# nreHieW/Eagle

Measured on AMD Instinct MI355X. Metric: frames/sec end-to-end (detect+keypoint+homography) @1280x720, higher is better.
Workload: dtype f32 (split: hi/lo binary16 pairs, 3 x fp16 MFMA per product, fp32 accumulate); detector (1.4 % of the FLOP): f32, exact v_mfma_f32_16x16x4_f32 chains

## Files before the change

### eagle_amd/csrc/clip.hip

```cpp
#include "runtime.h"

namespace eagle {

struct ProfOff { EagleHandle* h; bool was; explicit ProfOff(EagleHandle* h_) : h(h_), was(h_->prof) { h->prof = false; } ~ProfOff() { h->prof = was; } };

static void clip_sync(EagleHandle* h)
{
    HIP_CHECK(hipStreamSynchronize(h->s_det));
    HIP_CHECK(hipStreamSynchronize(h->s_main));
    HIP_CHECK(hipStreamSynchronize(h->s_post));
}

void clip_close(EagleHandle* h)
{
    EagleHandle::Clip& c = h->clip;
    if (c.open) { (void)hipStreamSynchronize(h->s_det); (void)hipStreamSynchronize(h->s_main); (void)hipStreamSynchronize(h->s_post); }
    for (auto& p : c.g) { if (p) (void)hipFree(p); p = nullptr; }
    if (c.recs) (void)hipFree(c.recs);
    if (c.mem) (void)hipFree(c.mem);
    if (c.st) (void)hipFree(c.st);
    if (c.st_op) (void)hipFree(c.st_op);
    if (c.h_st) (void)hipHostFree(c.h_st);
    if (c.h_zero) (void)hipHostFree(c.h_zero);
    if (c.h_tail) (void)hipHostFree(c.h_tail);
    if (c.h_mem) (void)hipHostFree(c.h_mem);
    if (c.ecc_small) (void)hipFree(c.ecc_small);
    if (c.ecc_pairs) (void)hipFree(c.ecc_pairs);
    if (c.ecc_out) (void)hipFree(c.ecc_out);
    for (hipEvent_t e : {c.ev_gray, c.ev_det, c.ev_kp, c.ev_loop}) if (e) (void)hipEventDestroy(e);
    c = EagleHandle::Clip();
}

static void clip_open(EagleHandle* h, const uint8_t* d_bgr, int n)
{
    clip_close(h);
    const EagleConfig& cf = h->cfg;
    EagleHandle::Clip& c = h->clip;
    c.cv.bgr = d_bgr; c.cv.n = n; c.cv.h = cf.frame_h; c.cv.w = cf.frame_w;
    c.cv.lh[0] = cf.frame_h; c.cv.lw[0] = cf.frame_w; c.cv.levels = 0;
    for (int l = 1; l <= 2; ++l) {
        c.cv.lh[l] = (c.cv.lh[l - 1] + 1) / 2; c.cv.lw[l] = (c.cv.lw[l - 1] + 1) / 2;
        if (c.cv.lw[l] <= 15 || c.cv.lh[l] <= 15) break;
        c.cv.levels = l;
    }
    c.open = true;
    for (int l = 0; l < 3; ++l) {
        HIP_CHECK(hipMalloc((void**)&c.g[l], std::max<size_t>((size_t)n * c.cv.lh[l] * c.cv.lw[l], 16)));
        c.cv.g[l] = c.g[l];
    }
    const size_t nn = (size_t)std::max(n, 1);
    HIP_CHECK(hipMalloc((void**)&c.recs, sizeof(EagleFrameResult) * nn));
    HIP_CHECK(hipMalloc((void**)&c.mem, sizeof(MemList) * nn));
    HIP_CHECK(hipMalloc((void**)&c.st, sizeof(ChainState)));
    HIP_CHECK(hipMalloc((void**)&c.st_op, sizeof(ChainState)));
    HIP_CHECK(hipHostMalloc((void**)&c.h_st, sizeof(ChainState), hipHostMallocDefault));
    HIP_CHECK(hipHostMalloc((void**)&c.h_zero, sizeof(ChainState), hipHostMallocDefault));
    HIP_CHECK(hipHostMalloc((void**)&c.h_tail, sizeof(int) * 4, hipHostMallocDefault));
    HIP_CHECK(hipHostMalloc((void**)&c.h_mem, sizeof(MemList), hipHostMallocDefault));
    memset(c.h_zero, 0, sizeof(ChainState));
    c.h_zero->stalled = -1;
    c.h_tail[0] = -1; c.h_tail[1] = 0; c.h_tail[2] = -1;
    for (hipEvent_t* e : {&c.ev_gray, &c.ev_det, &c.ev_kp, &c.ev_loop}) HIP_CHECK(hipEventCreateWithFlags(e, hipEventDisableTiming));
    HIP_CHECK(hipMemsetAsync(c.mem, 0xFF, sizeof(MemList) * nn, h->s_main));
    HIP_CHECK(hipMemsetAsync(c.recs, 0, sizeof(EagleFrameResult) * nn, h->s_main));
    HIP_CHECK(hipMemsetAsync(h->clip_sat, 0, sat_pad_bytes(cf.batch), h->s_main));
    HIP_CHECK(hipMemcpyAsync(c.st, c.h_zero, sizeof(ChainState), hipMemcpyHostToDevice, h->s_main));
    if (n > 0) gray_pyramid_launch(d_bgr, n, c.cv.h, c.cv.w, c.g[0], c.g[1], c.g[2], h->s_main);
    HIP_CHECK(hipEventRecord(c.ev_gray, h->s_main));
    HIP_CHECK(hipStreamWaitEvent(h->s_det, c.ev_gray, 0));
    HIP_CHECK(hipEventRecord(c.ev_det, h->s_det));
    HIP_CHECK(hipEventRecord(c.ev_kp, h->s_main));
    HIP_CHECK(hipEventRecord(c.ev_loop, h->s_post));
}

static void clip_detect_objects(EagleHandle* h, int first, int count)
{
    const EagleConfig& cf = h->cfg;
    EagleHandle::Clip& c = h->clip;
    const int B = cf.batch;
    const size_t fb = (size_t)cf.frame_h * cf.frame_w * 3;
    size_t ev_i = 0;
    EagleHandle::StepBuf& sb = h->sb[0];
    ProfOff prof_off(h);
    h->cur_sat = h->clip_sat;
    for (int i = first; i < first + count; i += B) {
        const int na = std::min(B, first + count - i);
        HIP_CHECK(hipMemsetAsync(sb.d_out, 0, sizeof(EagleFrameResult) * B, h->s_det));
        preprocess_launch(h->det_prec, c.cv.bgr + (size_t)i * fb, na, cf.frame_h, cf.frame_w, h->kp_in, h->det_in, h->lb, h->s_det, 2);
        run_net(h, h->yo.get(), h->s_det, ev_i);
        yolo_decode_launch(h->levels, 3, B, 5, cf.detector_floor, h->ds, h->s_det);
        nms_launch(h->ds, B, h->pp, sb.d_out, h->s_det);
        HIP_CHECK(hipMemcpyAsync(c.recs + i, sb.d_out, sizeof(EagleFrameResult) * na, hipMemcpyDeviceToDevice, h->s_det));
    }
    HIP_CHECK(hipEventRecord(c.ev_det, h->s_det));
}

static void clip_detect_keypoints(EagleHandle* h, int first, int stride, int count)
{
    const EagleConfig& cf = h->cfg;
    EagleHandle::Clip& c = h->clip;
    const int B = cf.batch;
    const size_t fb = (size_t)cf.frame_h * cf.frame_w * 3;
    size_t ev_i = 0;
    EagleHandle::StepBuf& sb = h->sb[0];
    ProfOff prof_off(h);
    h->cur_sat = h->clip_sat;
    for (int k0 = 0; k0 < count; k0 += B) {
        const int na = std::min(B, count - k0);
        const uint8_t* src;
        if (stride == 1) src = c.cv.bgr + (size_t)(first + k0) * fb;
        else {
            for (int k = 0; k < na; ++k)
                HIP_CHECK(hipMemcpyAsync(sb.d_frames + (size_t)k * fb, c.cv.bgr + (size_t)(first + (k0 + k) * stride) * fb, fb, hipMemcpyDeviceToDevice, h->s_main));
            src = sb.d_frames;
        }
        preprocess_launch(h->prec, src, na, cf.frame_h, cf.frame_w, h->kp_in, h->det_in, h->lb, h->s_main, 1);
        h->cur_parts = sb.parts;
        run_net(h, h->hr.get(), h->s_main, ev_i);
        if (!h->fused_argmax) heat_argmax_launch(h->logits, sb.parts, h->hm_chunks, h->s_main);
        decode_mem_launch(sb.parts, na, h->pp, c.mem, first + k0 * stride, stride, h->s_main);
    }
    HIP_CHECK(hipEventRecord(c.ev_kp, h->s_main));
}

}

extern "C" {

int eagle_reproject(EagleHandle* h, EagleFrameResult* recs, int n, const double* Hs, const uint8_t* flags)
{
    API_BEGIN_H(h)
    if (!recs || !Hs || !flags || n < 0) fail(EAGLE_E_INVALID, "bad argument");
    if (n == 0) return EAGLE_OK;
    HIP_CHECK(hipSetDevice(h->cfg.device));
    Net scratch;
    EagleFrameResult* d_r = (EagleFrameResult*)scratch.get(sizeof(EagleFrameResult) * (size_t)n);
    double* d_H = (double*)scratch.get(sizeof(double) * 9 * (size_t)n);
    unsigned char* d_f = (unsigned char*)scratch.get((size_t)n);
    HIP_CHECK(hipMemcpyAsync(d_r, recs, sizeof(EagleFrameResult) * (size_t)n, hipMemcpyHostToDevice, h->s_main));
    HIP_CHECK(hipMemcpyAsync(d_H, Hs, sizeof(double) * 9 * (size_t)n, hipMemcpyHostToDevice, h->s_main));
    HIP_CHECK(hipMemcpyAsync(d_f, flags, (size_t)n, hipMemcpyHostToDevice, h->s_main));
    reproject_launch(d_r, d_H, d_f, n, h->cfg.frame_h, h->cfg.frame_w, h->s_main);
    HIP_CHECK(hipMemcpyAsync(recs, d_r, sizeof(EagleFrameResult) * (size_t)n, hipMemcpyDeviceToHost, h->s_main));
    HIP_CHECK(hipStreamSynchronize(h->s_main));
    API_END(h)
}

int eagle_team_colors(EagleHandle* h, const void* d_bgr, int n_frames, const EagleCrop* crops, int n_crops, int32_t* counts)
{
    API_BEGIN_H(h)
    if (!d_bgr || n_frames < 0 || n_crops < 0 || (n_crops > 0 && (!crops || !counts))) fail(EAGLE_E_INVALID, "bad argument");
    if (n_crops == 0) return EAGLE_OK;
    HIP_CHECK(hipSetDevice(h->cfg.device));
    Net scratch;
    EagleCrop* d_c = (EagleCrop*)scratch.get(sizeof(EagleCrop) * (size_t)n_crops);
    int* d_n = (int*)scratch.get(sizeof(int) * 12 * (size_t)n_crops);
    HIP_CHECK(hipMemcpyAsync(d_c, crops, sizeof(EagleCrop) * (size_t)n_crops, hipMemcpyHostToDevice, h->s_main));
    eagle::team_colors_launch((const uint8_t*)d_bgr, n_frames, h->cfg.frame_h, h->cfg.frame_w, d_c, n_crops, d_n, h->s_main);
    HIP_CHECK(hipMemcpyAsync(counts, d_n, sizeof(int) * 12 * (size_t)n_crops, hipMemcpyDeviceToHost, h->s_main));
    HIP_CHECK(hipStreamSynchronize(h->s_main));
    API_END(h)
}

int eagle_reid_features(EagleHandle* h, const void* d_bgr, int n_frames, const EagleCrop* crops, int n_crops, float* feats)
{
    API_BEGIN_H(h)
    if (!h->finalized || !h->reid) fail(EAGLE_E_STATE, "no appearance network: load the reid.* tensors (OSNet-x0.25, torchreid names) before eagle_finalize_weights");
    if (n_frames < 0 || n_crops < 0 || (n_crops > 0 && (!d_bgr || !crops || !feats))) fail(EAGLE_E_INVALID, "bad argument");
    if (n_crops == 0) return EAGLE_OK;
    HIP_CHECK(hipSetDevice(h->cfg.device));
    eagle::ProfOff prof_off(h);
    for (int i0 = 0; i0 < n_crops; i0 += eagle::REID_NB) {
        const int nb = std::min(eagle::REID_NB, n_crops - i0);
        for (int k = 0; k < eagle::REID_NB; ++k) {
            EagleCrop c = {-1, 0, 0, 0, 0};
            if (k < nb) c = crops[i0 + k];
            h->reid_crops_h[k] = c;
        }
        HIP_CHECK(hipMemcpyAsync(h->reid_crops, h->reid_crops_h, sizeof(EagleCrop) * eagle::REID_NB, hipMemcpyHostToDevice, h->s_main));
        eagle::reid_crop_launch((const uint8_t*)d_bgr, n_frames, h->cfg.frame_h, h->cfg.frame_w, h->reid_crops, eagle::REID_NB, h->reid_in, h->s_main);
        size_t ev_i = 0;
        eagle::run_net(h, h->reid.get(), h->s_main, ev_i);
        HIP_CHECK(hipMemcpyAsync(h->reid_feats_h, h->reid_feats, sizeof(float) * EAGLE_REID_DIM * (size_t)nb, hipMemcpyDeviceToHost, h->s_main));
        HIP_CHECK(hipStreamSynchronize(h->s_main));
        memcpy(feats + (size_t)i0 * EAGLE_REID_DIM, h->reid_feats_h, sizeof(float) * EAGLE_REID_DIM * (size_t)nb);
    }
    API_END(h)
}

int eagle_track_open(EagleHandle* h, const EagleTrackParams* params)
{
    API_BEGIN_H(h)
    if (h->tracker) eagle::tracker_destroy(h->tracker);
    h->tracker = eagle::tracker_create(params);
    h->ecc_has_prev = false;
    API_END(h)
}

int eagle_track_frames(EagleHandle* h, EagleFrameResult* recs, int n) { return eagle_track_frames_cmc(h, recs, n, nullptr); }

int eagle_track_frames_cmc(EagleHandle* h, EagleFrameResult* recs, int n, const double* warps) { return eagle_track_frames_reid(h, recs, n, warps, nullptr, nullptr, nullptr); }

int eagle_track_frames_reid(EagleHandle* h, EagleFrameResult* recs, int n, const double* warps, const float* feats, const int32_t* feat_det, const int32_t* feat_count)
{
    API_BEGIN_H(h)
    if (!recs || n < 0 || (feats && (!feat_det || !feat_count))) fail(EAGLE_E_INVALID, "bad argument");
    if (!h->tracker) fail(EAGLE_E_STATE, "eagle_track_open has not been called");
    if (n == 0) return EAGLE_OK;
    if (feats)
        for (int i = 0; i < n; ++i) {
            if (feat_count[i] < 0 || feat_count[i] > EAGLE_MAX_DET) fail(EAGLE_E_INVALID, "eagle_track_frames_reid: feat_count[%d] = %d", i, feat_count[i]);
            if (recs[i].n_det < 0 || recs[i].n_det > EAGLE_MAX_DET) fail(EAGLE_E_INVALID, "eagle_track_frames_reid: record %d has n_det = %d", i, recs[i].n_det);
        }
    if (feats) {
        size_t o = 0;
        for (int i = 0; i < n; ++i)
            for (int k = 0; k < feat_count[i]; ++k, ++o)
                if (feat_det[o] < 0 || feat_det[o] >= recs[i].n_det)
                    fail(EAGLE_E_INVALID, "eagle_track_frames_reid: feat_det[%zu] = %d is not a detection of record %d (n_det %d)", o, feat_det[o], i, recs[i].n_det);
    }
    std::vector<double> Hs((size_t)n * 9, 0.0);
    std::vector<uint8_t> flags((size_t)n, 0);
    bool any = false;
    size_t fo = 0;
    for (int i = 0; i < n; ++i) {
        const int nf = feats ? feat_count[i] : 0;
        const bool applied = eagle::tracker_apply(h->tracker, recs + i, h->cfg.frame_h, h->cfg.frame_w, h->cfg.detector_conf, warps ? warps + (size_t)i * 6 : nullptr,
                                                  feats ? feats + fo * EAGLE_REID_DIM : nullptr, feats ? feat_det + fo : nullptr, nf);
        fo += (size_t)nf;
        if (!applied) continue;
        any = true;
        flags[i] = recs[i].H_valid ? 1 : 2;
        memcpy(&Hs[(size_t)i * 9], recs[i].H, sizeof(double) * 9);
    }
    if (any) {
        const int rc = eagle_reproject(h, recs, n, Hs.data(), flags.data());
        if (rc) return rc;
    }
    API_END(h)
}

#define CLIP_CHECK(h, cond, msg) if (!(h) || !(h)->finalized) return EAGLE_E_STATE; if (!(cond)) { (h)->err = msg; return EAGLE_E_INVALID; }
int eagle_clip_open(EagleHandle* h, const void* d_bgr, int n)
{
    CLIP_CHECK(h, n >= 0 && (d_bgr || n == 0), "eagle_clip_open: bad arguments")
    API_BEGIN
    HIP_CHECK(hipSetDevice(h->cfg.device));
    eagle::clip_open(h, (const uint8_t*)d_bgr, n);
    API_END(h)
}

int eagle_clip_close(EagleHandle* h)
{
    API_BEGIN_H(h)
    HIP_CHECK(hipSetDevice(h->cfg.device));
    eagle::clip_close(h);
    API_END(h)
}

int eagle_clip_detect_objects(EagleHandle* h, int first, int count)
{
    CLIP_CHECK(h, h->clip.open && first >= 0 && count >= 0 && first + (int64_t)count <= h->clip.cv.n, "eagle_clip_detect_objects: no open clip or frames out of range")
    API_BEGIN
    HIP_CHECK(hipSetDevice(h->cfg.device));
    eagle::clip_detect_objects(h, first, count);
    API_END(h)
}

int eagle_clip_detect_keypoints(EagleHandle* h, int first, int stride, int count)
// ... 217 lines not shown
```

### eagle_amd/csrc/common.h

```cpp
#pragma once
#include <hip/hip_runtime.h>
#include <hip/hip_fp16.h>
#include <cstdint>
#include <cstdio>
#include <string>
#include <vector>

#include "../../include/eagle.h"

namespace eagle {

enum Act : int { ACT_NONE = 0, ACT_RELU = 1, ACT_SILU = 2 };

struct Err {
    int code;
    std::string msg;
};
[[noreturn]] void fail(int code, const char* fmt, ...);

#define HIP_CHECK(expr)                                                                                \
    do {                                                                                               \
        hipError_t _e = (expr);                                                                        \
        if (_e != hipSuccess) ::eagle::fail(EAGLE_E_HIP, "%s failed: %s (%s:%d)", #expr, hipGetErrorString(_e), \
                                            __FILE__, __LINE__);                                       \
    } while (0)

void ensure_max_dynamic_lds(const void* fn, int bytes);

struct TView {
    void* p = nullptr;
    int n = 0, h = 0, w = 0;
    int c = 0;
    int cs = 0;
    int off = 0;
    int f32 = 0;
    size_t esize() const { return f32 ? 4 : 2; }
    TView slice(int o, int cc) const { TView v = *this; v.off = off + o; v.c = cc; return v; }
};

struct ConvConfig {
    int ks = 3, stride = 1;
    int kc = 0;
    int nt = 0;
    int wx = 2;
    int cin = 0, cout_pad = 0;
    int variant = 0;
};
struct ArgmaxPart { float score; int idx; };
struct ConvLaunch {
    ConvConfig cfg;
    TView x, y, r1, r2;
    const void* w = nullptr;
    const float* bias = nullptr;
    int pre_act = 0, post_act = 0;
    int out_f32 = 0;
    double flop = 0;
    float descale = 1.0f;
    ArgmaxPart* const* am_slot = nullptr;
    unsigned* const* sat_slot = nullptr;
};
int conv_tiles_per_frame(int precision, const ConvConfig& cfg, int ho, int wo);
bool conv_supported(int precision, const ConvConfig& cfg);
void conv_launch(int precision, const ConvLaunch& L, hipStream_t s);
size_t conv_weight_elems(int precision, const ConvConfig& cfg);
size_t conv_lds_bytes(int precision, const ConvConfig& cfg);
void conv_tile_weights(int precision, const ConvConfig& cfg, const float* w_hwio, int cin_real, int cout_real, void* dst, float* descale = nullptr);
inline int prec_tensor_fmt(int precision) { return precision == EAGLE_PREC_F32 ? 1 : precision == EAGLE_PREC_F32S ? 2 : 0; }
inline bool prec_is_f16_kernels(int precision) { return precision == EAGLE_PREC_F16 || precision == EAGLE_PREC_F32S; }
ConvConfig conv_choose(int precision, int ks, int stride, int cin_pad, int cout_pad, int wo, bool plain_epilogue = false, bool second_residual = false);

struct BneckLaunch {
    TView x, res, y;
    const void *w1 = nullptr, *w2 = nullptr, *w3 = nullptr;
    const float *b1 = nullptr, *b2 = nullptr, *b3 = nullptr;
    float ds1 = 1.f, ds2 = 1.f, ds3 = 1.f;
    unsigned* const* sat_slot = nullptr;
    unsigned long long* dbg = nullptr;
    bool ds_fused = false;
};
bool bneck_supported(const TView& x, int cmid, int cout);
void bneck_tile_weights(const float* w, int taps, int cin, int cout, std::vector<_Float16>& out, float* descale);
void bneck_scale_bias(std::vector<float>& b, float descale);
void bneck_launch(const BneckLaunch& L, hipStream_t s);

struct LetterBox { int new_h, new_w, top, left, out_h, out_w; };
LetterBox letterbox_geometry(int h, int w, int imgsz, int square = 0);
void preprocess_launch(int precision, const uint8_t* d_bgr, int n, int h, int w, const TView& kp, const TView& det,
                       const LetterBox& lb, hipStream_t s, int which = 3, int det_precision = -1);
struct FuseUp { TView z; };
void fuse_sum_launch(const TView& base, const FuseUp* ups, int n_up, int relu, const TView& y, hipStream_t s, unsigned* sat = nullptr);
void maxpool5_launch(const TView& x, const TView& y, hipStream_t s);
void upsample2_launch(const TView& x, const TView& y, hipStream_t s);
void split_to_f32_launch(const TView& x, const TView& y, hipStream_t s);

void heat_argmax_launch(const TView& logits, ArgmaxPart* parts, int chunks, hipStream_t s);

struct DetLevel { TView box, cls; int gh, gw; float stride; int a0; };
struct DetScratch {
    int A = 0;
    float* boxes = nullptr;
    float* conf = nullptr;
    int* cls = nullptr;
    unsigned long long* keys = nullptr;
    int* count = nullptr;
};
void yolo_decode_launch(const DetLevel* lv, int n_lv, int n, int nc, float conf_floor, const DetScratch& sc, hipStream_t s);

struct PostParams {
    int frame_h, frame_w, in_h, in_w;
    int hm_h, hm_w, hm_chunks;
    double keypoint_conf, detector_conf, ransac_thresh;
    float nms_iou;
    int ransac_max_iters, lm_iters;
};
void nms_launch(const DetScratch& sc, int n, const PostParams& pp, EagleFrameResult* d_out, hipStream_t s);
void post_launch(const ArgmaxPart* parts, int n, const PostParams& pp, EagleFrameResult* d_out, hipStream_t s);
void reproject_launch(EagleFrameResult* d_recs, const double* d_Hs, const unsigned char* d_flags, int n, int frame_h, int frame_w, hipStream_t s);
void homography_only_launch(const float* d_img, const float* d_world, int npts, double thresh, int max_iters, int lm_iters,
                            double* d_H, uint8_t* d_mask, int* d_ok, hipStream_t s);


struct ClipView {
    const uint8_t* bgr = nullptr;
    const uint8_t* g[3] = {nullptr, nullptr, nullptr};
    int lh[3] = {0, 0, 0}, lw[3] = {0, 0, 0};
    int levels = 0;
    int n = 0, h = 0, w = 0;
};
struct MemList { int n; EagleFlowKp kp[EAGLE_N_LANDMARKS]; };
struct ChainState {
    int n_prev; EagleFlowKp prev[EAGLE_N_LANDMARKS];
    int has_H, compute_h; double H[9];
    int stalled;
    int error;
    int lk_valid, lk_n;
    float lk_prev[2 * EAGLE_N_LANDMARKS], lk_next[2 * EAGLE_N_LANDMARKS];
    unsigned char lk_status[EAGLE_N_LANDMARKS];
    int flow_n; EagleFlowKp flow[EAGLE_N_LANDMARKS];
};
void gray_pyramid_launch(const uint8_t* d_bgr, int n, int h, int w, uint8_t* g0, uint8_t* g1, uint8_t* g2, hipStream_t s);
void lk_launch(const ClipView& cv, int src_frame, int dst_frame, ChainState* st, const MemList* mem, int kint, hipStream_t s);
struct EccResult { int ok, iters; double rho; float M[6]; };
void ecc_small_launch(const uint8_t* gray, uint8_t* small, int n, int h, int w, int dh, int dw, double inv_scale , hipStream_t s);
void ecc_launch(const uint8_t* small, const uint8_t* carry, const int2* pairs, int n_pairs, EccResult* out, int h, int w, int max_iter, double eps, hipStream_t s);
struct YuvArgs {
    const uint8_t* src;
    uint8_t* dst;
    int h, w;
    int64_t frame_stride, y_pitch, c_offset, c_pitch, v_offset;
    int c_step;
    int vec;
};
void yuv_to_bgr_launch(const YuvArgs& a, int n, hipStream_t s);
void team_colors_launch(const uint8_t* d_bgr, int n_frames, int fh, int fw, const EagleCrop* d_crops, int n_crops, int* d_counts, hipStream_t s);

void reid_crop_launch(const uint8_t* d_bgr, int n_frames, int fh, int fw, const EagleCrop* d_crops, int n, const TView& out, hipStream_t s);
void reid_conv7_launch(const TView& x, const float* w, const float* b, const TView& y, int n, hipStream_t s);
void reid_maxpool3s2_launch(const TView& x, const TView& y, int n, hipStream_t s);
void reid_avgpool2_launch(const TView& x, const TView& y, int n, hipStream_t s);
void reid_dw3_launch(const TView& x, const float* w, const float* b, const TView& y, int n, hipStream_t s);
void reid_gate_launch(const TView* streams, const float* w1, const float* b1, const float* w2, const float* b2, int c_real, int r, float* g, const TView& y, int n, hipStream_t s);
void reid_head_launch(const TView& x, const float* w, const float* b, float* feats, int dim, int n, hipStream_t s);

struct Tracker;
Tracker* tracker_create(const EagleTrackParams* p);
void tracker_destroy(Tracker* t);
bool tracker_apply(Tracker* t, EagleFrameResult* rec, int frame_h, int frame_w, double detector_conf, const double* warp = nullptr,
                   const float* feats = nullptr, const int* feat_det = nullptr, int n_feat = 0);
void similarity_ransac(const double* p0, const double* p1, int n, double* W6);
int lk_debug(const char* key, long long value, void* out, long long out_bytes);
void decode_mem_launch(const ArgmaxPart* parts, int n, const PostParams& pp, MemList* mem, int first, int stride, hipStream_t s);
void chain_launch(const ClipView& cv, ChainState* st, const MemList* mem, EagleFrameResult* recs, const PostParams& pp, int frame,
                  int kint, int hint, int calib, hipStream_t s);
void flow_filter_launch(const ClipView& cv, ChainState* st, int hue_frame, hipStream_t s);

}
```

### eagle_amd/csrc/elementwise.hip

```cpp
#include <type_traits>
#include "common.h"
#include "dmath.h"

namespace eagle {

using half8 = __attribute__((ext_vector_type(8))) _Float16;

struct ResizeAxis { int s0, s1; int a0, a1; };

__device__ __forceinline__ ResizeAxis lin_coef(int d, int dsize, int ssize)
{
    const double scale = (double)ssize / (double)dsize;
    float f = (float)(((double)d + 0.5) * scale - 0.5);
    int s = (int)floorf(f);
    f -= (float)s;
    if (s < 0) { s = 0; f = 0.f; }
    if (s >= ssize - 1) { s = ssize - 1; f = 0.f; }
    ResizeAxis r;
    r.s0 = s; r.s1 = (s + 1 < ssize) ? s + 1 : s;
    r.a0 = (int)(short)lrintf((1.f - f) * 2048.f);
    r.a1 = (int)(short)lrintf(f * 2048.f);
    return r;
}

__device__ __forceinline__ void resize_px(const uint8_t* src, int sh, int sw, int dh, int dw, int dy, int dx, int rgb[3])
{
    const size_t rs = (size_t)sw * 3;
    if (sh == dh && sw == dw) {
        const uint8_t* p = src + dy * rs + dx * 3;
        rgb[0] = p[2]; rgb[1] = p[1]; rgb[2] = p[0];
    } else if (sh == 2 * dh && sw == 2 * dw) {
        const uint8_t* p = src + (size_t)(2 * dy) * rs + (size_t)(2 * dx) * 3;
#pragma unroll
        for (int c = 0; c < 3; ++c) rgb[2 - c] = (p[c] + p[3 + c] + p[rs + c] + p[rs + 3 + c] + 2) >> 2;
    } else {
        const ResizeAxis ax = lin_coef(dx, dw, sw), ay = lin_coef(dy, dh, sh);
        const uint8_t* r0 = src + ay.s0 * rs; const uint8_t* r1 = src + ay.s1 * rs;
#pragma unroll
        for (int c = 0; c < 3; ++c) {
            const int t0 = r0[ax.s0 * 3 + c] * ax.a0 + r0[ax.s1 * 3 + c] * ax.a1;
            const int t1 = r1[ax.s0 * 3 + c] * ax.a0 + r1[ax.s1 * 3 + c] * ax.a1;
            rgb[2 - c] = (((ay.a0 * (t0 >> 4)) >> 16) + ((ay.a1 * (t1 >> 4)) >> 16) + 2) >> 2;
        }
    }
}

struct SplitT { char b[4]; };
__device__ __forceinline__ void split8_store(void* dst, const float* v)
{
    half8 hi, lo;
#pragma unroll
    for (int i = 0; i < 8; ++i) { const float s = __builtin_amdgcn_fmed3f(v[i] * 16.0f, -65504.0f, 65504.0f); hi[i] = (_Float16)s; lo[i] = (_Float16)(s - (float)hi[i]); }
    *(half8*)dst = hi; *((half8*)dst + 1) = lo;
}

template <typename T>
__device__ __forceinline__ void store_px(const TView& v, size_t pix, float r, float g, float b)
{
    if constexpr (sizeof(T) == 4 && !__is_same(T, float)) {
        const float o[8] = {r, g, b, 0.f, 0.f, 0.f, 0.f, 0.f};
        split8_store((char*)v.p + (pix * v.cs + v.off) * 4, o);
    } else if constexpr (sizeof(T) == 2) {
        half8 o = {(_Float16)r, (_Float16)g, (_Float16)b, 0, 0, 0, 0, 0};
        *(half8*)((_Float16*)v.p + pix * v.cs + v.off) = o;
    } else {
        *(float4*)((float*)v.p + pix * v.cs + v.off) = make_float4(r, g, b, 0.f);
    }
}

template <typename T, typename TD = T>
__global__ __launch_bounds__(256) void preprocess_kernel(const uint8_t* bgr, int n, int h, int w, TView kp, TView det, LetterBox lb, int which)
{
    const size_t fsz = (size_t)h * w * 3;
    const int kp_px = kp.h * kp.w, det_px = det.h * det.w;
    const int lo = (which & 1) ? 0 : kp_px, hi = (which & 2) ? kp_px + det_px : kp_px;
    const int per = hi - lo;
    for (size_t i = (size_t)blockIdx.x * blockDim.x + threadIdx.x; i < (size_t)n * per; i += (size_t)gridDim.x * blockDim.x) {
        const int f = (int)(i / per);
        int r = lo + (int)(i - (size_t)f * per);
        const uint8_t* src = bgr + f * fsz;
        int rgb[3];
        if (r < kp_px) {
            const int dy = r / kp.w, dx = r - dy * kp.w;
            resize_px(src, h, w, kp.h, kp.w, dy, dx, rgb);
            const float m0 = 0x1.eeb334p+6f, m1 = 0x1.d11eb8p+6f, m2 = 0x1.9e1eb8p+6f;
            const float s0 = 0x1.18926cp-6f, s1 = 0x1.1ed5bp-6f, s2 = 0x1.1d8f56p-6f;
            store_px<T>(kp, (size_t)f * kp_px + r, ((float)rgb[0] - m0) * s0, ((float)rgb[1] - m1) * s1, ((float)rgb[2] - m2) * s2);
        } else {
            r -= kp_px;
            const int dy = r / det.w, dx = r - dy * det.w;
            const int yy = dy - lb.top, xx = dx - lb.left;
            if (yy >= 0 && yy < lb.new_h && xx >= 0 && xx < lb.new_w) resize_px(src, h, w, lb.new_h, lb.new_w, yy, xx, rgb);
            else rgb[0] = rgb[1] = rgb[2] = 114;
            store_px<TD>(det, (size_t)f * det_px + r, (float)rgb[0] / 255.0f, (float)rgb[1] / 255.0f, (float)rgb[2] / 255.0f);
        }
    }
}

LetterBox letterbox_geometry(int h, int w, int imgsz, int square)
{
    const double r = std::min((double)imgsz / h, (double)imgsz / w);
    LetterBox lb;
    lb.new_w = (int)nearbyint(w * r); lb.new_h = (int)nearbyint(h * r);
    double dw = square ? (imgsz - lb.new_w) : (imgsz - lb.new_w) % 32, dh = square ? (imgsz - lb.new_h) : (imgsz - lb.new_h) % 32;
    dw /= 2; dh /= 2;
    lb.top = (int)nearbyint(dh - 0.1); lb.left = (int)nearbyint(dw - 0.1);
    const int bottom = (int)nearbyint(dh + 0.1), right = (int)nearbyint(dw + 0.1);
    lb.out_h = lb.new_h + lb.top + bottom; lb.out_w = lb.new_w + lb.left + right;
    return lb;
}

template <typename T>
static void preprocess_launch_det(int det_precision, dim3 grid, hipStream_t s, const uint8_t* d_bgr, int n, int h, int w, const TView& kp, const TView& det, const LetterBox& lb, int which)
{
    if (det_precision == EAGLE_PREC_F16) hipLaunchKernelGGL((preprocess_kernel<T, _Float16>), grid, dim3(256), 0, s, d_bgr, n, h, w, kp, det, lb, which);
    else if (det_precision == EAGLE_PREC_F32S) hipLaunchKernelGGL((preprocess_kernel<T, SplitT>), grid, dim3(256), 0, s, d_bgr, n, h, w, kp, det, lb, which);
    else hipLaunchKernelGGL((preprocess_kernel<T, float>), grid, dim3(256), 0, s, d_bgr, n, h, w, kp, det, lb, which);
}

void preprocess_launch(int precision, const uint8_t* d_bgr, int n, int h, int w, const TView& kp, const TView& det,
                       const LetterBox& lb, hipStream_t s, int which, int det_precision)
{
    const size_t total = (size_t)n * (((which & 1) ? kp.h * kp.w : 0) + ((which & 2) ? det.h * det.w : 0));
    if (total == 0) return;
    const int blocks = (int)std::min<size_t>((total + 255) / 256, 256 * 16);
    if (det_precision >= 0 && det_precision != precision) {
        if (precision == EAGLE_PREC_F16) preprocess_launch_det<_Float16>(det_precision, dim3(blocks), s, d_bgr, n, h, w, kp, det, lb, which);
        else if (precision == EAGLE_PREC_F32S) preprocess_launch_det<SplitT>(det_precision, dim3(blocks), s, d_bgr, n, h, w, kp, det, lb, which);
        else preprocess_launch_det<float>(det_precision, dim3(blocks), s, d_bgr, n, h, w, kp, det, lb, which);
        HIP_CHECK(hipGetLastError());
        return;
    }
    if (precision == EAGLE_PREC_F16) hipLaunchKernelGGL(preprocess_kernel<_Float16>, dim3(blocks), dim3(256), 0, s, d_bgr, n, h, w, kp, det, lb, which);
    else if (precision == EAGLE_PREC_F32S) hipLaunchKernelGGL(preprocess_kernel<SplitT>, dim3(blocks), dim3(256), 0, s, d_bgr, n, h, w, kp, det, lb, which);
    else hipLaunchKernelGGL(preprocess_kernel<float>, dim3(blocks), dim3(256), 0, s, d_bgr, n, h, w, kp, det, lb, which);
    HIP_CHECK(hipGetLastError());
}

#ifndef EAGLE_FUSE_NT
#define EAGLE_FUSE_NT 0
#endif
template <typename T> struct Vec;
template <> struct Vec<_Float16> {
    static constexpr int N = 8;
    float v[8];
    __device__ __forceinline__ void load(const void* p, size_t e) { half8 h = *(const half8*)((const _Float16*)p + e); for (int i = 0; i < 8; ++i) v[i] = (float)h[i]; }
    __device__ __forceinline__ void store(void* p, size_t e) const { half8 h; for (int i = 0; i < 8; ++i) h[i] = (_Float16)v[i]; *(half8*)((_Float16*)p + e) = h; }
};
template <> struct Vec<SplitT> {
    static constexpr int N = 8;
    float v[8];
    __device__ __forceinline__ void load(const void* p, size_t e)
    {
        const half8 hi = *(const half8*)((const char*)p + e * 4), lo = *(const half8*)((const char*)p + e * 4 + 16);
        for (int i = 0; i < 8; ++i) v[i] = (float)hi[i] + (float)lo[i];
    }
    __device__ __forceinline__ void store(void* p, size_t e) const
    {
        half8 hi, lo;
#pragma unroll
        for (int i = 0; i < 8; ++i) { const float s = __builtin_amdgcn_fmed3f(v[i], -65504.0f, 65504.0f); hi[i] = (_Float16)s; lo[i] = (_Float16)(s - (float)hi[i]); }
        *(half8*)((char*)p + e * 4) = hi; *((half8*)((char*)p + e * 4) + 1) = lo;
    }
    __device__ __forceinline__ void store_nt(void* p, size_t e) const
    {
        half8 hi, lo;
#pragma unroll
        for (int i = 0; i < 8; ++i) { const float s = __builtin_amdgcn_fmed3f(v[i], -65504.0f, 65504.0f); hi[i] = (_Float16)s; lo[i] = (_Float16)(s - (float)hi[i]); }
        __builtin_nontemporal_store(hi, (half8*)((char*)p + e * 4)); __builtin_nontemporal_store(lo, (half8*)((char*)p + e * 4) + 1);
    }
};
template <> struct Vec<float> {
    static constexpr int N = 4;
    float v[4];
    __device__ __forceinline__ void load(const void* p, size_t e) { float4 f = *(const float4*)((const float*)p + e); v[0] = f.x; v[1] = f.y; v[2] = f.z; v[3] = f.w; }
    __device__ __forceinline__ void store(void* p, size_t e) const { *(float4*)((float*)p + e) = make_float4(v[0], v[1], v[2], v[3]); }
};

struct FuseArgs { TView base, y; TView z[3]; float sh[3], sw[3]; int n_up; int relu; unsigned* sat; };

constexpr int FUSE_ROWS = 8;
template <typename T, int NUP>
__global__ __launch_bounds__(256) void fuse_sum_kernel(FuseArgs a)
{
    constexpr int VN = Vec<T>::N;
    const int H = a.y.h, W = a.y.w, groups = a.y.c / VN;
    const unsigned col = blockIdx.y * 256u + threadIdx.x;
    if (col >= (unsigned)(W * groups)) return;
    const int hb = (H + FUSE_ROWS - 1) / FUSE_ROWS;
    const int band = gridDim.x >> 3, rb = (int)(blockIdx.x & 7) * band + (int)(blockIdx.x >> 3);
    if (rb >= a.y.n * hb) return;
    const int n = rb / hb, oy0 = (rb - n * hb) * FUSE_ROWS;
    const int ox = (int)(col / (unsigned)groups), g = (int)(col - (unsigned)ox * (unsigned)groups);
    constexpr int NU = NUP > 0 ? NUP : 1;
    Vec<T> p00[NU], p01[NU], p10[NU], p11[NU];
    float lx1[NU];
    int cy0[NU], cy1[NU];
    unsigned zc0[NU], zc1[NU];
#pragma unroll
    for (int j = 0; j < NUP; ++j) {
        const TView& z = a.z[j];
        const float fx = a.sw[j] * (float)ox;
        const int x0 = (int)fx, x1 = x0 + (x0 < z.w - 1 ? 1 : 0);
        lx1[j] = fx - (float)x0;
        const unsigned co = (unsigned)(z.off + g * VN);
        zc0[j] = (unsigned)x0 * (unsigned)z.cs + co; zc1[j] = (unsigned)x1 * (unsigned)z.cs + co;
        cy0[j] = -1; cy1[j] = -1;
    }
    for (int r = 0; r < FUSE_ROWS; ++r) {
        const int oy = oy0 + r;
        if (oy >= H) break;
        const unsigned pix = ((unsigned)n * H + (unsigned)oy) * (unsigned)W + (unsigned)ox;
        Vec<T> acc; acc.load(a.base.p, (size_t)pix * a.base.cs + a.base.off + g * VN);
        float ly1[NU];
#pragma unroll
        for (int j = 0; j < NUP; ++j) {
            const TView& z = a.z[j];
            const float fy = a.sh[j] * (float)oy;
            const int y0 = __builtin_amdgcn_readfirstlane((int)fy);
            const int y1 = y0 + (y0 < z.h - 1 ? 1 : 0);
            ly1[j] = fy - (float)y0;
            const unsigned b = (unsigned)n * z.h;
            if (y0 != cy0[j]) {
                if (y0 == cy1[j]) { p00[j] = p10[j]; p01[j] = p11[j]; }
                else {
                    const unsigned ro = (b + (unsigned)y0) * (unsigned)z.w * (unsigned)z.cs;
                    p00[j].load(z.p, (size_t)(ro + zc0[j])); p01[j].load(z.p, (size_t)(ro + zc1[j]));
                }
                cy0[j] = y0;
            }
            if (y1 != cy1[j]) {
                if (y1 == y0) { p10[j] = p00[j]; p11[j] = p01[j]; }
                else {
                    const unsigned ro = (b + (unsigned)y1) * (unsigned)z.w * (unsigned)z.cs;
                    p10[j].load(z.p, (size_t)(ro + zc0[j])); p11[j].load(z.p, (size_t)(ro + zc1[j]));
                }
                cy1[j] = y1;
            }
        }
#pragma unroll
        for (int j = 0; j < NUP; ++j) {
            const float ly0 = 1.0f - ly1[j], lx0 = 1.0f - lx1[j];
#pragma unroll
            for (int k = 0; k < VN; ++k) {
                const float top = fmaf(lx1[j], p01[j].v[k], lx0 * p00[j].v[k]);
// ... 163 lines not shown
```

### eagle_amd/csrc/nets.hip

```cpp
#include "runtime.h"

namespace eagle {

struct Builder {
    EagleHandle* H;
    Net* net;
    int prec;
    double bn_eps;
    int N;
    const char* label_suffix = "";
    int cur_stream = 0;
    void set_stream(int k) { cur_stream = k; net->pool = k; }
    void fork_join(Op::Kind kind, int nbranch) { Op op; op.kind = kind; op.nbranch = nbranch; op.tag = kind == Op::FORK ? "fork" : "join"; net->ops.push_back(op); }

    int gran() const { return prec == EAGLE_PREC_F32 ? 4 : 8; }

    TView act(int h, int w, int c, bool f32 = false)
    {
        TView v; v.n = N; v.h = h; v.w = w; v.c = c; v.cs = c; v.off = 0;
        v.f32 = (f32 || prec == EAGLE_PREC_F32) ? 1 : prec_tensor_fmt(prec);
        v.p = net->get((size_t)N * h * w * c * v.esize());
        return v;
    }
    void release(const TView& v) { net->put(v.p); }

    const HostTensor& W(const std::string& name)
    {
        auto it = H->weights.find(name);
        if (it == H->weights.end()) fail(EAGLE_E_MISSING, "weight tensor '%s' was not loaded", name.c_str());
        return it->second;
    }

    TView conv(const TView& x, const std::string& cname, const std::string& bn, int stride, int pre, const TView* r1,
               const TView* r2, int post, const TView* out = nullptr, bool out_f32 = false, ArgmaxPart* const* am_slot = nullptr)
    {
        std::vector<float> hwio, bias; int cin, cout, ks;
        fold(cname, bn, hwio, bias, cin, cout, ks);
        if (cin > x.c) fail(EAGLE_E_INVALID, "%s: input has %d channels, weight expects %d", cname.c_str(), x.c, cin);
        const int cout_pad = (cout + 15) / 16 * 16;
        bias.resize(cout_pad, 0.f);
        const int ho = (x.h + 2 * (ks / 2) - ks) / stride + 1, wo = (x.w + 2 * (ks / 2) - ks) / stride + 1;
        if (const char* dump = getenv("EAGLE_DUMP_LAYERS")) {
            if (FILE* f = fopen(dump, "a")) { fprintf(f, "%d,%d,%d,%d,%d,%d,%d\n", ks, stride, x.c, cout_pad, x.h, x.w, N); fclose(f); }
        }
        ConvLaunch L;
        L.cfg = conv_choose(prec, ks, stride, x.c, cout_pad, wo, pre == ACT_NONE && post <= ACT_RELU && !out_f32, r1 && r2);
        if (!conv_supported(prec, L.cfg))
            fail(EAGLE_E_NOKERNEL, "%s: no kernel instance (ks=%d s=%d kc=%d nt=%d)", cname.c_str(), ks, stride, L.cfg.kc, L.cfg.nt);
        const size_t ne = conv_weight_elems(prec, L.cfg);
        std::vector<char> tiled(ne * (prec == EAGLE_PREC_F32 ? 4 : 2));
        conv_tile_weights(prec, L.cfg, hwio.data(), cin, cout, tiled.data(), &L.descale);
        L.w = net->upload(tiled.data(), tiled.size());
        L.bias = (const float*)net->upload(bias.data(), bias.size() * 4);
        L.x = x;
        if (out) {
            L.y = *out;
            if (out->c != cout_pad || out->h != ho || out->w != wo) fail(EAGLE_E_INVALID, "%s: output slice mismatch", cname.c_str());
        } else {
            L.y = act(ho, wo, cout_pad, out_f32);
        }
        if (r1) L.r1 = *r1;
        if (r2) L.r2 = *r2;
        L.pre_act = pre; L.post_act = post; L.out_f32 = out_f32 ? 1 : 0;
        refuse_2gib(cname, "layer", {&L.x, &L.y, r1 ? &L.r1 : nullptr, r2 ? &L.r2 : nullptr});
        L.am_slot = am_slot;
        if (prec == EAGLE_PREC_F32S && !out_f32 && !am_slot) L.sat_slot = &H->cur_sat;
        if (am_slot) { H->hm_chunks = conv_tiles_per_frame(prec, L.cfg, ho, wo); H->fused_argmax = true; }
        L.flop = 2.0 * N * ho * wo * (double)cout * cin * ks * ks;
        const int pr = prec;
        char label[64];
        snprintf(label, sizeof(label), "conv %dx%d/%d %d->%d @%dx%d v%d%s", ks, ks, stride, cin, cout, ho, wo, L.cfg.variant, label_suffix);
        const double es = prec == EAGLE_PREC_F16 ? 2 : 4;
        emit_conv(label, L.flop, (double)N * x.h * x.w * cin * es + (double)N * ho * wo * cout * ((out_f32 || prec != EAGLE_PREC_F16) ? 4 : 2) * (am_slot ? 0 : 1) +
                                 (r1 ? (double)N * ho * wo * cout * es : 0) + (r2 ? (double)N * ho * wo * cout * es : 0) + (double)ks * ks * cin * cout * es,
                  [L, pr](hipStream_t s) { conv_launch(pr, L, s); });
        return L.y;
    }
    void fold(const std::string& cname, const std::string& bn, std::vector<float>& hwio, std::vector<float>& bias, int& cin, int& cout, int& ks)
    {
        const HostTensor& w = W(cname + ".weight");
        if (w.shape.size() != 4) fail(EAGLE_E_INVALID, "%s.weight: expected 4-d", cname.c_str());
        cout = (int)w.shape[0]; cin = (int)w.shape[1]; ks = (int)w.shape[2];
        hwio.assign((size_t)ks * ks * cin * cout, 0.f); bias.assign(cout, 0.f);
        std::vector<double> scale(cout, 1.0);
        if (!bn.empty()) {
            const HostTensor &g = W(bn + ".weight"), &b = W(bn + ".bias"), &m = W(bn + ".running_mean"), &v = W(bn + ".running_var");
            for (int o = 0; o < cout; ++o) {
                scale[o] = (double)g.data[o] / std::sqrt((double)v.data[o] + bn_eps);
                bias[o] = (float)((double)b.data[o] - (double)m.data[o] * scale[o]);
            }
        } else if (H->weights.count(cname + ".bias")) {
            const HostTensor& b = W(cname + ".bias");
            for (int o = 0; o < cout; ++o) bias[o] = b.data[o];
        }
        for (int o = 0; o < cout; ++o)
            for (int i = 0; i < cin; ++i)
                for (int t = 0; t < ks * ks; ++t) {
                    const float wv = w.data[((size_t)o * cin + i) * ks * ks + t];
                    hwio[((size_t)t * cin + i) * cout + o] = bn.empty() ? wv : (float)((double)wv * scale[o]);
                }
    }
    void refuse_2gib(const std::string& name, const char* what, std::initializer_list<const TView*> ts)
    {
        for (const TView* t : ts)
            if (t && (size_t)t->n * t->h * t->w * t->cs * t->esize() >= ((size_t)1 << 31))
                fail(EAGLE_E_INVALID, "%s: a %d x %d x %d x %d-channel tensor of this %s reaches 2 GiB at a device batch of %d frames (32-bit tensor offsets); use a smaller EagleConfig.batch",
                     name.c_str(), t->n, t->h, t->w, t->cs, what, N);
    }
    void emit_conv(const char* label, double flop, double bytes, std::function<void(hipStream_t)> run)
    {
        net->names.emplace_back(new std::string(label));
        Op op; op.kind = Op::CONV; op.flop = flop; op.bytes = bytes; op.tag = net->names.back()->c_str(); op.stream = cur_stream; op.run = std::move(run);
        net->ops.push_back(op);
    }
    TView bottleneck(const TView& x, const std::string& q, const TView& res, const std::string& ds_conv = "", const std::string& ds_bn = "")
    {
        BneckLaunch L;
        const bool dsf = !ds_conv.empty();
        std::vector<float> hw, bs; int ci, co, ks;
        std::vector<_Float16> img;
        double flop = 0;
        const char* cn[3] = {"conv1", "conv2", "conv3"}; const char* bnn[3] = {"bn1", "bn2", "bn3"};
        const int want_ks[3] = {1, 3, 1}, want_ci[3] = {x.c, 64, 64}, want_co[3] = {64, 64, 256};
        for (int k = 0; k < 3; ++k) {
            fold(q + cn[k], q + bnn[k], hw, bs, ci, co, ks);
            if (ks != want_ks[k] || ci != want_ci[k] || co != want_co[k]) fail(EAGLE_E_INVALID, "%s%s: not the Bottleneck shape of the fused kernel", q.c_str(), cn[k]);
            if (k == 2 && dsf) {
                std::vector<float> hwd, bd; int cid, cod, ksd;
                fold(ds_conv, ds_bn, hwd, bd, cid, cod, ksd);
                if (ksd != 1 || cid != 64 || cod != 256 || x.c != 64) fail(EAGLE_E_INVALID, "%s: not the 1x1 64->256 downsample of the fused kernel", ds_conv.c_str());
                hw.insert(hw.end(), hwd.begin(), hwd.end());
                for (int o = 0; o < 256; ++o) bs[o] = bs[o] + bd[o];
                ci = 128;
                flop += 2.0 * N * x.h * x.w * 256.0 * 64;
            }
            float ds = 1.f;
            bneck_tile_weights(hw.data(), ks * ks, ci, co, img, &ds);
            bneck_scale_bias(bs, ds);
            const void* dw = net->upload(img.data(), img.size() * 2);
            const float* db = (const float*)net->upload(bs.data(), bs.size() * 4);
            if (k == 0) { L.w1 = dw; L.b1 = db; L.ds1 = ds; } else if (k == 1) { L.w2 = dw; L.b2 = db; L.ds2 = ds; } else { L.w3 = dw; L.b3 = db; L.ds3 = ds; }
            flop += 2.0 * N * x.h * x.w * (double)co * (k == 2 ? 64 : ci) * ks * ks;
        }
        L.x = x; L.y = act(x.h, x.w, 256); L.res = dsf ? L.y : res; L.ds_fused = dsf;
        L.sat_slot = &H->cur_sat;
        refuse_2gib(q, "block", {&L.x, &L.y, &L.res});
        char label[64];
        snprintf(label, sizeof(label), "bneck %d->64->256%s @%dx%d%s", x.c, dsf ? "+ds" : "", x.h, x.w, label_suffix);
        emit_conv(label, flop, (double)N * x.h * x.w * 4.0 * (x.c + 256 + ((dsf || res.p == x.p) ? 0 : 256)) + 4.0 * (x.c * 64 + 9 * 64 * 64 + 64 * 256 + (dsf ? 64 * 256 : 0)),
                  [L](hipStream_t s) { bneck_launch(L, s); });
        return L.y;
    }
    static double vbytes(const TView& v) { return (double)v.n * v.h * v.w * v.c * (v.f32 ? 4 : 2); }
    void other(std::function<void(hipStream_t)> fn, const char* tag, double bytes = 0)
    {
        Op op; op.kind = Op::OTHER; op.run = std::move(fn); op.tag = tag; op.stream = cur_stream; op.bytes = bytes;
        net->ops.push_back(op);
    }
};

static const char* HRP = "unnormalized_model.0.";

static std::vector<TView> hr_stage(Builder& B, std::vector<TView> xs, int stage_idx, int n_modules, int nb, bool last_single)
{
    const int R = ACT_RELU;
    for (int m = 0; m < n_modules; ++m) {
        const std::string q = std::string(HRP) + "stage" + std::to_string(stage_idx) + "." + std::to_string(m) + ".";
        B.fork_join(Op::FORK, nb - 1);
        const bool interleave = !(getenv("EAGLE_HR_INTERLEAVE") && atoi(getenv("EAGLE_HR_INTERLEAVE")) == 0);
        for (int step = 0; step < 4 * nb; ++step) {
            const int k = interleave ? step / nb : step % 4, b = interleave ? nb - 1 - step % nb : step / 4;
            B.set_stream(b);
            TView x = xs[b];
            const std::string r = q + "branches." + std::to_string(b) + "." + std::to_string(k) + ".";
            TView o = B.conv(x, r + "conv1", r + "bn1", 1, 0, nullptr, nullptr, R);
            TView y = B.conv(o, r + "conv2", r + "bn2", 1, 0, &x, nullptr, R);
            B.release(o);
            B.release(x);
            xs[b] = y;
        }
        B.set_stream(0);
        B.fork_join(Op::JOIN, nb - 1);
        const int n_out = (last_single && m == n_modules - 1) ? 1 : nb;
        std::vector<TView> out;
        if (n_out > 1) B.fork_join(Op::FORK, n_out - 1);
        for (int i = 0; i < n_out; ++i) {
            B.set_stream(n_out > 1 ? i : 0);
            TView y; bool have_y = false;
            for (int j = 0; j < i; ++j) {
                TView t = xs[j];
                for (int k = 0; k < i - j; ++k) {
                    const std::string r = q + "fuse_layers." + std::to_string(i) + "." + std::to_string(j) + "." + std::to_string(k) + ".";
                    const bool last = k == i - j - 1;
                    TView nt;
                    if (!last) {
                        nt = B.conv(t, r + "0", r + "1", 2, 0, nullptr, nullptr, R);
                    } else {
                        const TView* ident = (j == i - 1) ? &xs[i] : nullptr;
                        const bool relu_now = ident && i == nb - 1;
                        nt = B.conv(t, r + "0", r + "1", 2, 0, have_y ? &y : nullptr, ident, relu_now ? R : 0);
                    }
                    if (k > 0) B.release(t);
                    t = nt;
                }
                if (have_y) B.release(y);
                y = t; have_y = true;
            }
            if (i == 0) y = xs[0];
            FuseUp ups[3]; int nu = 0;
            for (int j = i + 1; j < nb; ++j) {
                const std::string r = q + "fuse_layers." + std::to_string(i) + "." + std::to_string(j) + ".";
                ups[nu++].z = B.conv(xs[j], r + "0", r + "1", 1, 0, nullptr, nullptr, 0);
            }
            if (nu) {
                TView o = B.act(y.h, y.w, y.c);
                const TView base = y; FuseUp u0 = ups[0], u1 = ups[1], u2 = ups[2]; const int n_up = nu;
                EagleHandle* const Hh = B.H;
                B.other([base, u0, u1, u2, n_up, o, Hh](hipStream_t s) { FuseUp u[3] = {u0, u1, u2}; fuse_sum_launch(base, u, n_up, 1, o, s, Hh->cur_sat); }, "fuse_sum",
                        Builder::vbytes(base) + Builder::vbytes(o) + (nu > 0 ? Builder::vbytes(ups[0].z) : 0) + (nu > 1 ? Builder::vbytes(ups[1].z) : 0) + (nu > 2 ? Builder::vbytes(ups[2].z) : 0));
                for (int k = 0; k < nu; ++k) B.release(ups[k].z);
                if (i != 0) B.release(y);
                y = o;
            }
            out.push_back(y);
        }
        B.set_stream(0);
        if (n_out > 1) B.fork_join(Op::JOIN, n_out - 1);
        for (int b = 0; b < nb; ++b) B.release(xs[b]);
        xs = out;
    }
    return xs;
}

static TView build_hrnet(Builder& B, const TView& x_in)
{
    const int R = ACT_RELU;
    const std::string P = HRP;
    TView x = B.conv(x_in, P + "conv1", P + "bn1", 2, 0, nullptr, nullptr, R);
    TView x2 = B.conv(x, P + "conv2", P + "bn2", 2, 0, nullptr, nullptr, R);
    B.release(x); x = x2;
    for (int b = 0; b < 4; ++b) {
        const std::string q = P + "layer1." + std::to_string(b) + ".";
        const char* fe = getenv("EAGLE_BNECK_FUSED");
        const char* de = getenv("EAGLE_BNECK_DS");
        const bool fused = B.prec == EAGLE_PREC_F32S && !(fe && atoi(fe) == 0) && bneck_supported(x, 64, 256);
        const bool dsf = fused && b == 0 && x.c == 64 && !(de && atoi(de) == 0);
        TView res = x;
        if (b == 0 && !dsf) res = B.conv(x, q + "downsample.0", q + "downsample.1", 1, 0, nullptr, nullptr, 0);
        if (fused) {
            TView y = dsf ? B.bottleneck(x, q, x, q + "downsample.0", q + "downsample.1") : B.bottleneck(x, q, res);
            if (b == 0 && !dsf) B.release(res);
            B.release(x);
            x = y;
            continue;
        }
        TView o1 = B.conv(x, q + "conv1", q + "bn1", 1, 0, nullptr, nullptr, R);
        TView o2 = B.conv(o1, q + "conv2", q + "bn2", 1, 0, nullptr, nullptr, R);
        TView y = B.conv(o2, q + "conv3", q + "bn3", 1, 0, &res, nullptr, R);
        B.release(o1); B.release(o2);
        if (b == 0) B.release(res);
        B.release(x);
        x = y;
    }
    std::vector<TView> ys(2);
    B.fork_join(Op::FORK, 1);
    B.set_stream(1);
    ys[1] = B.conv(x, P + "transition1.1.0.0", P + "transition1.1.0.1", 2, 0, nullptr, nullptr, R);
    B.set_stream(0);
    ys[0] = B.conv(x, P + "transition1.0.0", P + "transition1.0.1", 1, 0, nullptr, nullptr, R);
    B.fork_join(Op::JOIN, 1);
    B.release(x);
    ys = hr_stage(B, ys, 2, 1, 2, false);
    ys.push_back(B.conv(ys.back(), P + "transition2.2.0.0", P + "transition2.2.0.1", 2, 0, nullptr, nullptr, R));
    ys = hr_stage(B, ys, 3, 4, 3, false);
    ys.push_back(B.conv(ys.back(), P + "transition3.3.0.0", P + "transition3.3.0.1", 2, 0, nullptr, nullptr, R));
    ys = hr_stage(B, ys, 4, 3, 4, true);
    ArgmaxPart* const* am = (prec_is_f16_kernels(B.prec) && !getenv("EAGLE_NO_FUSED_ARGMAX")) ? &B.H->cur_parts : nullptr;
    TView logits = B.conv(ys[0], "unnormalized_model.1", "", 1, 0, nullptr, nullptr, 0, nullptr, true, am);
    B.release(ys[0]);
    return logits;
}

struct YoloDims { int c[5]; int n[4]; };
static YoloDims yolo_dims(int variant)
{
    static const double D[5] = {0.33, 0.33, 0.67, 1.0, 1.0}, Wd[5] = {0.25, 0.5, 0.75, 1.0, 1.25};
    static const int MC[5] = {1024, 1024, 768, 512, 512};
    YoloDims y;
    const int base[5] = {64, 128, 256, 512, 1024};
    for (int i = 0; i < 5; ++i) y.c[i] = (int)std::ceil(std::min(base[i], MC[variant]) * Wd[variant] / 8.0) * 8;
    const int rep[4] = {3, 6, 6, 3};
    for (int i = 0; i < 4; ++i) y.n[i] = std::max((int)std::nearbyint(rep[i] * D[variant]), 1);
    return y;
}

struct YoloBuilder {
    Builder& B;
    int S = ACT_SILU;
    TView cv(const TView& x, const std::string& name, int stride = 1, const TView* r1 = nullptr, const TView* out = nullptr)
    {
        return B.conv(x, name + ".conv", name + ".bn", stride, S, r1, nullptr, 0, out);
    }
    TView c2f(const TView& x, int idx, int cout, int n, bool shortcut, const TView* out = nullptr)
    {
        const std::string p = "model." + std::to_string(idx);
        const int c = cout / 2;
        TView cat = B.act(x.h, x.w, (2 + n) * c);
        TView first = cat.slice(0, 2 * c);
        cv(x, p + ".cv1", 1, nullptr, &first);
        for (int k = 0; k < n; ++k) {
            TView in = cat.slice((1 + k) * c, c);
            TView t = cv(in, p + ".m." + std::to_string(k) + ".cv1");
            TView o = cat.slice((2 + k) * c, c);
            cv(t, p + ".m." + std::to_string(k) + ".cv2", 1, shortcut ? &in : nullptr, &o);
            B.release(t);
        }
        TView y = cv(cat, p + ".cv2", 1, nullptr, out);
        B.release(cat);
        return y;
    }
};

static void build_yolo(Builder& B, const TView& x_in, int variant, DetLevel lv[3], int nc, bool mixed = false)
{
    YoloBuilder Y{B};
    const YoloDims d = yolo_dims(variant);
    const int c1 = d.c[0], c2 = d.c[1], c3 = d.c[2], c4 = d.c[3], c5 = d.c[4];
    TView x0 = Y.cv(x_in, "model.0", 2);
    TView x1 = Y.cv(x0, "model.1", 2); B.release(x0);
    TView x2 = Y.c2f(x1, 2, c2, d.n[0], true); B.release(x1);
    TView x3 = Y.cv(x2, "model.3", 2); B.release(x2);
    const int h3 = x3.h, w3 = x3.w;
    const int h4 = (h3 - 1) / 2 + 1, w4 = (w3 - 1) / 2 + 1, h5 = (h4 - 1) / 2 + 1, w5 = (w4 - 1) / 2 + 1;
    TView cat15 = B.act(h3, w3, c4 + c3);
    TView cat12 = B.act(h4, w4, c5 + c4);
    TView cat18 = B.act(h4, w4, c3 + c4);
    TView cat21 = B.act(h5, w5, c4 + c5);
    TView p3 = cat15.slice(c4, c3), p4 = cat12.slice(c5, c4), p5 = cat21.slice(c4, c5), h12 = cat18.slice(c3, c4);
    Y.c2f(x3, 4, c3, d.n[1], true, &p3); B.release(x3);
    TView x5 = Y.cv(p3, "model.5", 2);
    Y.c2f(x5, 6, c4, d.n[2], true, &p4); B.release(x5);
    TView x7 = Y.cv(p4, "model.7", 2);
    TView x8 = Y.c2f(x7, 8, c5, d.n[3], true); B.release(x7);
    {
        const int ch = c5 / 2;
        TView cat = B.act(h5, w5, 4 * ch);
        TView s0 = cat.slice(0, ch), s1 = cat.slice(ch, ch), s2 = cat.slice(2 * ch, ch), s3 = cat.slice(3 * ch, ch);
        Y.cv(x8, "model.9.cv1", 1, nullptr, &s0); B.release(x8);
        B.other([s0, s1](hipStream_t s) { maxpool5_launch(s0, s1, s); }, "maxpool5", 2 * Builder::vbytes(s0));
        B.other([s1, s2](hipStream_t s) { maxpool5_launch(s1, s2, s); }, "maxpool5", 2 * Builder::vbytes(s0));
        B.other([s2, s3](hipStream_t s) { maxpool5_launch(s2, s3, s); }, "maxpool5", 2 * Builder::vbytes(s0));
        Y.cv(cat, "model.9.cv2", 1, nullptr, &p5);
        B.release(cat);
    }
    {
        TView u = cat12.slice(0, c5);
        B.other([p5, u](hipStream_t s) { upsample2_launch(p5, u, s); }, "upsample2", Builder::vbytes(p5) + Builder::vbytes(u));
        Y.c2f(cat12, 12, c4, d.n[0], false, &h12);
    }
    TView h15, h18, h21;
    {
        TView u = cat15.slice(0, c4);
        B.other([h12, u](hipStream_t s) { upsample2_launch(h12, u, s); }, "upsample2", Builder::vbytes(h12) + Builder::vbytes(u));
    }
    if (!mixed) {
        h15 = Y.c2f(cat15, 15, c3, d.n[0], false);
        {
            TView o = cat18.slice(0, c3);
            Y.cv(h15, "model.16", 2, nullptr, &o);
        }
        h18 = Y.c2f(cat18, 18, c4, d.n[0], false);
        {
            TView o = cat21.slice(0, c4);
            Y.cv(h18, "model.19", 2, nullptr, &o);
        }
        h21 = Y.c2f(cat21, 21, c5, d.n[0], false);
    } else {
        B.prec = EAGLE_PREC_F32;
        auto to_f32 = [&B](const TView& x, const TView& y) {
            B.other([x, y](hipStream_t s) { split_to_f32_launch(x, y, s); }, "split_to_f32", Builder::vbytes(x) + Builder::vbytes(y));
        };
        TView cat15f = B.act(h3, w3, c4 + c3), cat18f = B.act(h4, w4, c3 + c4), cat21f = B.act(h5, w5, c4 + c5);
        to_f32(cat15, cat15f);
        h15 = Y.c2f(cat15f, 15, c3, d.n[0], false);
        {
            TView o = cat18f.slice(0, c3);
            Y.cv(h15, "model.16", 2, nullptr, &o);
            to_f32(h12, cat18f.slice(c3, c4));
        }
        h18 = Y.c2f(cat18f, 18, c4, d.n[0], false);
        {
// ... 9 lines not shown
    for (int l = 0; l < 3; ++l) {
        const std::string pb = "model.22.cv2." + std::to_string(l), pc = "model.22.cv3." + std::to_string(l);
        TView b0 = Y.cv(feats[l], pb + ".0");
        TView b1 = Y.cv(b0, pb + ".1"); B.release(b0);
        TView box = B.conv(b1, pb + ".2", "", 1, 0, nullptr, nullptr, 0, nullptr, true); B.release(b1);
        TView k0 = Y.cv(feats[l], pc + ".0");
        TView k1 = Y.cv(k0, pc + ".1"); B.release(k0);
        TView cls = B.conv(k1, pc + ".2", "", 1, 0, nullptr, nullptr, 0, nullptr, true); B.release(k1);
        lv[l].box = box; lv[l].cls = cls; lv[l].gh = box.h; lv[l].gw = box.w; lv[l].stride = strides[l]; lv[l].a0 = a0;
        a0 += box.h * box.w;
    }
    (void)c1; (void)nc;
}

static const char* RP = "reid.";

struct ReidFold { std::vector<float> scale, shift; };
static ReidFold reid_bn(Builder& B, const std::string& bn, int c)
{
    const HostTensor &g = B.W(bn + ".weight"), &b = B.W(bn + ".bias"), &m = B.W(bn + ".running_mean"), &v = B.W(bn + ".running_var");
    ReidFold f; f.scale.resize(c); f.shift.resize(c);
    for (int o = 0; o < c; ++o) {
        const double sc = (double)g.data[o] / std::sqrt((double)v.data[o] + 1e-5);
        f.scale[o] = (float)sc; f.shift[o] = (float)((double)b.data[o] - (double)m.data[o] * sc);
    }
    return f;
}

static TView reid_light(Builder& B, const TView& x, const std::string& lc, int mid)
{
    TView t = B.conv(x, lc + ".conv1", "", 1, 0, nullptr, nullptr, 0);
    const HostTensor& w = B.W(lc + ".conv2.weight");
    const ReidFold f = reid_bn(B, lc + ".bn", mid);
    const int C = t.c;
    std::vector<float> wk((size_t)9 * C, 0.f), bk(C, 0.f);
    for (int c = 0; c < mid; ++c) {
        for (int k = 0; k < 9; ++k) wk[(size_t)k * C + c] = (float)((double)w.data[(size_t)c * 9 + k] * (double)f.scale[c]);
        bk[c] = f.shift[c];
    }
    const float* dw = (const float*)B.net->upload(wk.data(), wk.size() * 4);
    const float* db = (const float*)B.net->upload(bk.data(), bk.size() * 4);
    TView y = B.act(t.h, t.w, C);
    const int n = B.N;
    B.other([t, dw, db, y, n](hipStream_t s) { reid_dw3_launch(t, dw, db, y, n, s); }, "reid dw3x3", 2 * Builder::vbytes(y));
    B.release(t);
    return y;
}

static TView reid_osblock(Builder& B, const TView& x, const std::string& b, int cin, int cout)
{
    const int mid = cout / 4, R = ACT_RELU;
    TView x1 = B.conv(x, b + ".conv1.conv", b + ".conv1.bn", 1, 0, nullptr, nullptr, R);
    TView st[4];
    st[0] = reid_light(B, x1, b + ".conv2a", mid);
    const char* names[3] = {"b", "c", "d"};
    for (int k = 0; k < 3; ++k) {
        TView y = x1;
        for (int d = 0; d < k + 2; ++d) {
            TView nx = reid_light(B, y, b + ".conv2" + names[k] + "." + std::to_string(d), mid);
            if (d > 0) B.release(y);
            y = nx;
        }
        st[k + 1] = y;
    }
    B.release(x1);
    const HostTensor &w1 = B.W(b + ".gate.fc1.weight"), &b1 = B.W(b + ".gate.fc1.bias"), &w2 = B.W(b + ".gate.fc2.weight"), &b2 = B.W(b + ".gate.fc2.bias");
    const int r = (int)w1.shape[0];
    const float* d1 = (const float*)B.net->upload(w1.data.data(), w1.data.size() * 4);
    const float* e1 = (const float*)B.net->upload(b1.data.data(), b1.data.size() * 4);
    const float* d2 = (const float*)B.net->upload(w2.data.data(), w2.data.size() * 4);
    const float* e2 = (const float*)B.net->upload(b2.data.data(), b2.data.size() * 4);
    const int C = st[0].c, n = B.N;
    float* g = (float*)B.net->get((size_t)n * 4 * C * 4);
    TView x2 = B.act(st[0].h, st[0].w, C);
    const TView s0 = st[0], s1 = st[1], s2 = st[2], s3 = st[3];
    B.other([s0, s1, s2, s3, d1, e1, d2, e2, mid, r, g, x2, n](hipStream_t s) { const TView ss[4] = {s0, s1, s2, s3}; reid_gate_launch(ss, d1, e1, d2, e2, mid, r, g, x2, n, s); },
            "reid gate", 5 * Builder::vbytes(x2));
    for (auto& t : st) B.release(t);
    TView ident = x;
    if (cin != cout) ident = B.conv(x, b + ".downsample.conv", b + ".downsample.bn", 1, 0, nullptr, nullptr, 0);
    TView y = B.conv(x2, b + ".conv3.conv", b + ".conv3.bn", 1, 0, &ident, nullptr, R);
    B.release(x2);
    if (cin != cout) B.release(ident);
    return y;
}

static void build_reid(Builder& B, EagleHandle* h)
{
    const std::string P = RP;
    const int n = B.N;
    h->reid_in = B.act(256, 128, 4);
    const HostTensor& w1 = B.W(P + "conv1.conv.weight");
    const ReidFold f1 = reid_bn(B, P + "conv1.bn", 16);
    std::vector<float> wk(7 * 7 * 3 * 16), bk(16);
    for (int o = 0; o < 16; ++o) {
        for (int c = 0; c < 3; ++c)
            for (int k = 0; k < 49; ++k) wk[(size_t)(k * 3 + c) * 16 + o] = (float)((double)w1.data[((size_t)o * 3 + c) * 49 + k] * (double)f1.scale[o]);
        bk[o] = f1.shift[o];
    }
    const float* dw = (const float*)B.net->upload(wk.data(), wk.size() * 4);
    const float* db = (const float*)B.net->upload(bk.data(), bk.size() * 4);
    TView c1 = B.act(128, 64, 16);
    const TView in = h->reid_in;
    B.other([in, dw, db, c1, n](hipStream_t s) { reid_conv7_launch(in, dw, db, c1, n, s); }, "reid conv7x7", Builder::vbytes(in) + Builder::vbytes(c1));
    TView x = B.act(64, 32, 16);
    B.other([c1, x, n](hipStream_t s) { reid_maxpool3s2_launch(c1, x, n, s); }, "reid maxpool", Builder::vbytes(c1) + Builder::vbytes(x));
    B.release(c1);
    static const int CH[4] = {16, 64, 96, 128};
    const char* stage[3] = {"conv2", "conv3", "conv4"};
    for (int sI = 0; sI < 3; ++sI) {
        const int cin = CH[sI], cout = CH[sI + 1];
        const std::string sp = P + stage[sI];
        TView y = reid_osblock(B, x, sp + ".0", cin, cout); B.release(x); x = y;
        y = reid_osblock(B, x, sp + ".1", cout, cout); B.release(x); x = y;
        if (sI < 2) {
            TView t = B.conv(x, sp + ".2.0.conv", sp + ".2.0.bn", 1, 0, nullptr, nullptr, ACT_RELU); B.release(x);
            TView p = B.act(t.h / 2, t.w / 2, t.c);
            B.other([t, p, n](hipStream_t s) { reid_avgpool2_launch(t, p, n, s); }, "reid avgpool", Builder::vbytes(t) + Builder::vbytes(p));
            B.release(t);
            x = p;
        }
    }
    TView c5 = B.conv(x, P + "conv5.conv", P + "conv5.bn", 1, 0, nullptr, nullptr, ACT_RELU); B.release(x);
    const HostTensor &fw = B.W(P + "fc.0.weight"), &fb = B.W(P + "fc.0.bias");
    const ReidFold ff = reid_bn(B, P + "fc.1", EAGLE_REID_DIM);
    std::vector<float> hw((size_t)EAGLE_REID_DIM * c5.c, 0.f), hb(EAGLE_REID_DIM);
    for (int o = 0; o < EAGLE_REID_DIM; ++o) {
        for (int c = 0; c < 128; ++c) hw[(size_t)o * c5.c + c] = (float)((double)fw.data[(size_t)o * 128 + c] * (double)ff.scale[o]);
        hb[o] = (float)((double)fb.data[o] * (double)ff.scale[o] + (double)ff.shift[o]);
    }
    const float* dhw = (const float*)B.net->upload(hw.data(), hw.size() * 4);
    const float* dhb = (const float*)B.net->upload(hb.data(), hb.size() * 4);
    h->reid_feats = (float*)B.net->get((size_t)n * EAGLE_REID_DIM * 4);
    float* feats = h->reid_feats;
    B.other([c5, dhw, dhb, feats, n](hipStream_t s) { reid_head_launch(c5, dhw, dhb, feats, EAGLE_REID_DIM, n, s); }, "reid head", Builder::vbytes(c5));
    h->reid_crops = (EagleCrop*)B.net->get(sizeof(EagleCrop) * (size_t)n);
    HIP_CHECK(hipHostMalloc((void**)&h->reid_crops_h, sizeof(EagleCrop) * (size_t)n, hipHostMallocDefault));
    HIP_CHECK(hipHostMalloc((void**)&h->reid_feats_h, sizeof(float) * EAGLE_REID_DIM * (size_t)n, hipHostMallocDefault));
}

void finalize(EagleHandle* h)
{
    const EagleConfig& c = h->cfg;
    const int B = c.batch;
    h->prec = c.precision;
    const bool det_mixed = c.det_precision == EAGLE_DET_PREC_MIXED;
    h->det_prec = det_mixed ? EAGLE_PREC_F32S : c.det_precision ? c.det_precision - 1 : c.precision;
    h->hr.reset(new Net); h->yo.reset(new Net); h->misc.reset(new Net);
    const int cin_pad = h->prec == EAGLE_PREC_F32 ? 4 : 8, det_cin_pad = h->det_prec == EAGLE_PREC_F32 ? 4 : 8;
    h->lb = letterbox_geometry(c.frame_h, c.frame_w, c.det_imgsz, c.letterbox);
    Builder Bh{h, h->hr.get(), h->prec, 1e-5, B};
    Builder By{h, h->yo.get(), h->det_prec, 1e-3, B};
    By.label_suffix = " d";
    h->kp_in = Bh.act(540, 960, cin_pad);
    h->det_in = By.act(h->lb.out_h, h->lb.out_w, det_cin_pad);
    h->logits = build_hrnet(Bh, h->kp_in);
    build_yolo(By, h->det_in, c.det_variant, h->levels, 5, det_mixed);
    if (h->weights.count(std::string(RP) + "conv1.conv.weight")) {
        h->reid.reset(new Net);
        Builder Br{h, h->reid.get(), EAGLE_PREC_F32, 1e-5, REID_NB};
        build_reid(Br, h);
    }
    Net* m = h->misc.get();
    for (auto& sb : h->sb) {
        sb.d_frames = (uint8_t*)m->get((size_t)B * c.frame_h * c.frame_w * 3);
        sb.parts = (ArgmaxPart*)m->get(sizeof(ArgmaxPart) * (size_t)B * h->hm_chunks * 64);
        const size_t sat_pad = sat_pad_bytes(B);
        sb.d_sat = (unsigned*)m->get(sat_pad + sizeof(EagleFrameResult) * (size_t)B);
        sb.d_out = (EagleFrameResult*)((char*)sb.d_sat + sat_pad);
        HIP_CHECK(hipHostMalloc((void**)&sb.h_sat, sat_pad + sizeof(EagleFrameResult) * (size_t)B, hipHostMallocDefault));
        sb.h_out = (EagleFrameResult*)((char*)sb.h_sat + sat_pad);
        HIP_CHECK(hipEventCreateWithFlags(&sb.ev_compute, hipEventDisableTiming));
        HIP_CHECK(hipEventCreateWithFlags(&sb.ev_done, hipEventDisableTiming));
        HIP_CHECK(hipEventCreateWithFlags(&sb.ev_copy, hipEventDisableTiming));
    }
    h->clip_sat = (unsigned*)m->get(sat_pad_bytes(B));
    HIP_CHECK(hipHostMalloc((void**)&h->clip_sat_h, sat_pad_bytes(B), hipHostMallocDefault));
    int A = 0;
    for (int l = 0; l < 3; ++l) A += h->levels[l].gh * h->levels[l].gw;
    h->ds.A = A;
    h->ds.boxes = (float*)m->get(sizeof(float) * 4 * (size_t)B * A);
    h->ds.conf = (float*)m->get(sizeof(float) * (size_t)B * A);
    h->ds.cls = (int*)m->get(sizeof(int) * (size_t)B * A);
    h->ds.keys = (unsigned long long*)m->get(sizeof(unsigned long long) * (size_t)B * A);
    h->ds.count = (int*)m->get(sizeof(int) * (size_t)B);
    PostParams& pp = h->pp;
    pp.frame_h = c.frame_h; pp.frame_w = c.frame_w; pp.in_h = h->lb.out_h; pp.in_w = h->lb.out_w;
    pp.hm_h = h->logits.h; pp.hm_w = h->logits.w; pp.hm_chunks = h->hm_chunks;
    pp.keypoint_conf = c.keypoint_conf; pp.detector_conf = c.detector_conf; pp.nms_iou = c.nms_iou;
    pp.ransac_thresh = c.ransac_thresh; pp.ransac_max_iters = c.ransac_max_iters; pp.lm_iters = c.lm_iters;
    h->n_conv = 0; h->conv_flop_step = 0; h->n_launch = 6;
    for (Net* n : {h->hr.get(), h->yo.get()})
        for (Op& op : n->ops) { ++h->n_launch; if (op.kind == Op::CONV) { ++h->n_conv; h->conv_flop_step += op.flop; } }
    h->conv_ev.resize((size_t)h->n_conv * 2);
    for (auto& e : h->conv_ev) HIP_CHECK(hipEventCreate(&e));
    h->weights.clear();
    h->finalized = true;
}

}
```

### eagle_amd/csrc/ops_api.hip

```cpp
#include "runtime.h"

extern "C" {

static void to_dev(Net& net, int prec, const float* src, int n, int h, int w, int c, int cpad, TView& v)
{
    v.n = n; v.h = h; v.w = w; v.c = cpad; v.cs = cpad; v.off = 0; v.f32 = prec_tensor_fmt(prec);
    const size_t px = (size_t)n * h * w;
    if (v.f32 == 2) {
        std::vector<_Float16> t(px * cpad * 2, (_Float16)0.f);
        for (size_t p = 0; p < px; ++p)
            for (int k = 0; k < c; ++k) {
                const float sv = src[p * c + k] * 16.0f;
                const _Float16 hi = (_Float16)sv;
                t[p * cpad * 2 + (k / 8) * 16 + (k % 8)] = hi;
                t[p * cpad * 2 + (k / 8) * 16 + 8 + (k % 8)] = (_Float16)(sv - (float)hi);
            }
        v.p = net.upload(t.data(), t.size() * 2);
    } else if (v.f32) {
        std::vector<float> t(px * cpad, 0.f);
        for (size_t p = 0; p < px; ++p) for (int k = 0; k < c; ++k) t[p * cpad + k] = src[p * c + k];
        v.p = net.upload(t.data(), t.size() * 4);
    } else {
        std::vector<_Float16> t(px * cpad, (_Float16)0.f);
        for (size_t p = 0; p < px; ++p) for (int k = 0; k < c; ++k) t[p * cpad + k] = (_Float16)src[p * c + k];
        v.p = net.upload(t.data(), t.size() * 2);
    }
}
static void from_dev(const TView& v, int c, float* dst)
{
    const size_t px = (size_t)v.n * v.h * v.w;
    if (v.f32 == 2) {
        std::vector<_Float16> t(px * v.cs * 2);
        HIP_CHECK(hipMemcpy(t.data(), v.p, t.size() * 2, hipMemcpyDeviceToHost));
        for (size_t p = 0; p < px; ++p)
            for (int k = 0; k < c; ++k) {
                const size_t e = p * v.cs * 2 + (size_t)((v.off + k) / 8) * 16 + (v.off + k) % 8;
                dst[p * c + k] = ((float)t[e] + (float)t[e + 8]) * 0.0625f;
            }
    } else if (v.f32) {
        std::vector<float> t(px * v.cs);
        HIP_CHECK(hipMemcpy(t.data(), v.p, t.size() * 4, hipMemcpyDeviceToHost));
        for (size_t p = 0; p < px; ++p) for (int k = 0; k < c; ++k) dst[p * c + k] = t[p * v.cs + v.off + k];
    } else {
        std::vector<_Float16> t(px * v.cs);
        HIP_CHECK(hipMemcpy(t.data(), v.p, t.size() * 2, hipMemcpyDeviceToHost));
        for (size_t p = 0; p < px; ++p) for (int k = 0; k < c; ++k) dst[p * c + k] = (float)t[p * v.cs + v.off + k];
    }
}

int eagle_op_conv2d(int device, int precision, const float* x, int n, int h, int w, int cin, const float* w_hwio,
                    const float* bias, int cout, int ks, int stride, int pre_act, const float* r1, const float* r2,
                    int post_act, float* y)
{
    EagleHandle* hh = nullptr;
    API_BEGIN
    HIP_CHECK(hipSetDevice(device));
    Net net;
    const int g = precision == EAGLE_PREC_F32 ? 4 : 8;
    const int cin_pad = cin <= g ? g : (cin + 15) / 16 * 16, cout_pad = (cout + 15) / 16 * 16;
    const int ho = (h + 2 * (ks / 2) - ks) / stride + 1, wo = (w + 2 * (ks / 2) - ks) / stride + 1;
    ConvLaunch L;
    to_dev(net, precision, x, n, h, w, cin, cin_pad, L.x);
    L.cfg = conv_choose(precision, ks, stride, cin_pad, cout_pad, wo, pre_act == ACT_NONE && post_act <= ACT_RELU, r1 && r2);
    if (!conv_supported(precision, L.cfg)) fail(EAGLE_E_NOKERNEL, "no kernel instance ks=%d s=%d kc=%d nt=%d", ks, stride, L.cfg.kc, L.cfg.nt);
    std::vector<char> tiled(conv_weight_elems(precision, L.cfg) * (precision == EAGLE_PREC_F32 ? 4 : 2));
    conv_tile_weights(precision, L.cfg, w_hwio, cin, cout, tiled.data(), &L.descale);
    L.w = net.upload(tiled.data(), tiled.size());
    std::vector<float> b(cout_pad, 0.f);
    for (int i = 0; i < cout; ++i) b[i] = bias[i];
    L.bias = (const float*)net.upload(b.data(), b.size() * 4);
    L.y.n = n; L.y.h = ho; L.y.w = wo; L.y.c = cout_pad; L.y.cs = cout_pad; L.y.f32 = prec_tensor_fmt(precision);
    L.y.p = net.get((size_t)n * ho * wo * cout_pad * L.y.esize());
    if (r1) to_dev(net, precision, r1, n, ho, wo, cout, cout_pad, L.r1);
    if (r2) to_dev(net, precision, r2, n, ho, wo, cout, cout_pad, L.r2);
    L.pre_act = pre_act; L.post_act = post_act;
    conv_launch(precision, L, nullptr);
    HIP_CHECK(hipDeviceSynchronize());
    from_dev(L.y, cout, y);
    API_END(hh)
}

int eagle_op_bottleneck(int device, const float* x, int n, int h, int w, int cin, const float* w1, const float* b1, const float* w2, const float* b2,
                        const float* w3, const float* b3, const float* res, float* y, int reps, float* ms, const float* wd, const float* bd)
{
    EagleHandle* hh = nullptr;
    API_BEGIN
    HIP_CHECK(hipSetDevice(device));
    if (!x || !w1 || !b1 || !w2 || !b2 || !w3 || !b3 || !y || n < 1 || h < 1 || w < 1 || cin % 16 || cin < 16) fail(EAGLE_E_INVALID, "eagle_op_bottleneck: bad argument (Cin must be a multiple of 16)");
    if ((wd != nullptr) != (bd != nullptr) || (wd && (res || cin != 64))) fail(EAGLE_E_INVALID, "eagle_op_bottleneck: the in-kernel downsample branch takes (wd, bd) together, Cin = 64 and no residual tensor");
    if (!res && !wd && cin != 256) fail(EAGLE_E_INVALID, "eagle_op_bottleneck: an identity shortcut needs Cin = 256");
    Net net;
    BneckLaunch L;
    to_dev(net, EAGLE_PREC_F32S, x, n, h, w, cin, cin, L.x);
    if (res) to_dev(net, EAGLE_PREC_F32S, res, n, h, w, 256, 256, L.res); else L.res = L.x;
    L.y = L.x; L.y.c = L.y.cs = 256; L.y.off = 0; L.y.p = net.get((size_t)n * h * w * 256 * 4);
    if (wd) L.res = L.y;
    std::vector<_Float16> img;
    bneck_tile_weights(w1, 1, cin, 64, img, &L.ds1); L.w1 = net.upload(img.data(), img.size() * 2);
    bneck_tile_weights(w2, 9, 64, 64, img, &L.ds2); L.w2 = net.upload(img.data(), img.size() * 2);
    std::vector<float> w3x(w3, w3 + 64 * 256), sb3(b3, b3 + 256);
    if (wd) {
        w3x.insert(w3x.end(), wd, wd + 64 * 256);
        for (int o = 0; o < 256; ++o) sb3[o] = sb3[o] + bd[o];
        L.ds_fused = true;
    }
    bneck_tile_weights(w3x.data(), 1, wd ? 128 : 64, 256, img, &L.ds3); L.w3 = net.upload(img.data(), img.size() * 2);
    std::vector<float> sb1(b1, b1 + 64), sb2(b2, b2 + 64);
    bneck_scale_bias(sb1, L.ds1); bneck_scale_bias(sb2, L.ds2); bneck_scale_bias(sb3, L.ds3);
    L.b1 = (const float*)net.upload(sb1.data(), 64 * 4); L.b2 = (const float*)net.upload(sb2.data(), 64 * 4); L.b3 = (const float*)net.upload(sb3.data(), 256 * 4);
    if (getenv("EAGLE_BNECK_TIMING")) L.dbg = (unsigned long long*)net.get(8192 * 8 * 8);
    unsigned* op_sat = nullptr; unsigned* const* op_sat_slot = &op_sat;
    if (getenv("EAGLE_BNECK_OPSAT")) { op_sat = (unsigned*)net.get(sizeof(unsigned) * (size_t)n); L.sat_slot = op_sat_slot; }
    bneck_launch(L, nullptr);
    HIP_CHECK(hipDeviceSynchronize());
    if (L.dbg) {
        std::vector<unsigned long long> t(8192 * 8);
        HIP_CHECK(hipMemcpy(t.data(), L.dbg, t.size() * 8, hipMemcpyDeviceToHost));
        double sum[8] = {0}; int nw = 0;
        for (int b = 0; b < 8192; ++b) { bool any = false; for (int k = 0; k < 8; ++k) { sum[k] += (double)t[b * 8 + k]; any |= t[b * 8 + k] != 0; } nw += any; }
        if (nw) fprintf(stderr, "[bneck timing] %d workgroups, mean us per workgroup: phase1 %.1f  wait %.1f  epi1 %.1f  phase2 %.1f  epi2 %.1f  phase3 %.1f\n", nw,
                        sum[0] / nw / 100, sum[1] / nw / 100, sum[2] / nw / 100, sum[3] / nw / 100, sum[4] / nw / 100, sum[5] / nw / 100);
    }
    if (reps > 0 && ms) {
        hipEvent_t e0, e1;
        HIP_CHECK(hipEventCreate(&e0)); HIP_CHECK(hipEventCreate(&e1));
        HIP_CHECK(hipEventRecord(e0, nullptr));
        for (int i = 0; i < reps; ++i) bneck_launch(L, nullptr);
        HIP_CHECK(hipEventRecord(e1, nullptr));
        HIP_CHECK(hipEventSynchronize(e1));
        HIP_CHECK(hipEventElapsedTime(ms, e0, e1));
        *ms /= (float)reps;
        (void)hipEventDestroy(e0); (void)hipEventDestroy(e1);
    }
    from_dev(L.y, 256, y);
    API_END(hh)
}

int eagle_op_fuse_sum(int device, int precision, const float* base, int n, int H, int W, int c, int n_up,
                      const float* const* ups, const int* up_h, const int* up_w, int relu, float* y)
{
    EagleHandle* hh = nullptr;
    API_BEGIN
    HIP_CHECK(hipSetDevice(device));
    if (n_up > 3 || c % 8) fail(EAGLE_E_INVALID, "fuse_sum: n_up <= 3 and c %% 8 == 0 required");
    Net net;
    TView b, o;
    to_dev(net, precision, base, n, H, W, c, c, b);
    FuseUp u[3];
    for (int i = 0; i < n_up; ++i) to_dev(net, precision, ups[i], n, up_h[i], up_w[i], c, c, u[i].z);
    o = b; o.p = net.get((size_t)n * H * W * c * b.esize());
    fuse_sum_launch(b, u, n_up, relu, o, nullptr);
    HIP_CHECK(hipDeviceSynchronize());
    from_dev(o, c, y);
    API_END(hh)
}

int eagle_op_preprocess(int device, int precision, const uint8_t* bgr, int n, int h, int w, int det_imgsz,
                        float* kp_out, float* det_out, int* det_hw)
{
    return eagle_op_preprocess_lb(device, precision, bgr, n, h, w, det_imgsz, EAGLE_LETTERBOX_RECT, kp_out, det_out, det_hw);
}

int eagle_op_preprocess_lb(int device, int precision, const uint8_t* bgr, int n, int h, int w, int det_imgsz, int letterbox,
                           float* kp_out, float* det_out, int* det_hw)
{
    EagleHandle* hh = nullptr;
    API_BEGIN
    HIP_CHECK(hipSetDevice(device));
    Net net;
    const int cp = precision == EAGLE_PREC_F32 ? 4 : 8;
    const LetterBox lb = letterbox_geometry(h, w, det_imgsz, letterbox);
    det_hw[0] = lb.out_h; det_hw[1] = lb.out_w;
    if (!kp_out || !det_out) return EAGLE_OK;
    uint8_t* d = (uint8_t*)net.upload(bgr, (size_t)n * h * w * 3);
    TView kp, det;
    kp.n = n; kp.h = 540; kp.w = 960; kp.c = kp.cs = cp; kp.f32 = prec_tensor_fmt(precision);
    det = kp; det.h = lb.out_h; det.w = lb.out_w;
    kp.p = net.get((size_t)n * 540 * 960 * cp * kp.esize());
    det.p = net.get((size_t)n * lb.out_h * lb.out_w * cp * det.esize());
    preprocess_launch(precision, d, n, h, w, kp, det, lb, nullptr);
    HIP_CHECK(hipDeviceSynchronize());
    from_dev(kp, 3, kp_out);
    from_dev(det, 3, det_out);
    API_END(hh)
}

int eagle_op_find_homography(int device, const float* img_pts, const float* world_pts, int n, double thresh,
                             int max_iters, int lm_iters, double* H9, uint8_t* mask, int* ok)
{
    EagleHandle* hh = nullptr;
    API_BEGIN
    HIP_CHECK(hipSetDevice(device));
    if (n < 0 || n > EAGLE_MAX_KP) fail(EAGLE_E_INVALID, "0 <= n <= %d required", EAGLE_MAX_KP);
    Net net;
    float* di = (float*)net.upload(img_pts, sizeof(float) * 2 * std::max(n, 1));
    float* dw = (float*)net.upload(world_pts, sizeof(float) * 2 * std::max(n, 1));
    double* dH = (double*)net.get(72);
    uint8_t* dm = (uint8_t*)net.get(256);
    int* dok = (int*)net.get(16);
    homography_only_launch(di, dw, n, thresh, max_iters, lm_iters, dH, dm, dok, nullptr);
    HIP_CHECK(hipDeviceSynchronize());
    HIP_CHECK(hipMemcpy(H9, dH, 72, hipMemcpyDeviceToHost));
    if (n > 0) HIP_CHECK(hipMemcpy(mask, dm, n, hipMemcpyDeviceToHost));
    HIP_CHECK(hipMemcpy(ok, dok, sizeof(int), hipMemcpyDeviceToHost));
    API_END(hh)
}

}
```

### eagle_amd/csrc/resize.h

```cpp
#pragma once
#include <hip/hip_runtime.h>
#include <cstdint>

namespace eagle {

struct ResizeTap { int s0, s1; int a0, a1; };

__device__ __forceinline__ ResizeTap resize_tap_scaled(int d, double scale, int ssize)
{
    float f = (float)(((double)d + 0.5) * scale - 0.5);
    int s = (int)floorf(f);
    f -= (float)s;
    if (s < 0) { s = 0; f = 0.f; }
    if (s >= ssize - 1) { s = ssize - 1; f = 0.f; }
    ResizeTap r;
    r.s0 = s; r.s1 = (s + 1 < ssize) ? s + 1 : s;
    r.a0 = (int)(short)lrintf((1.f - f) * 2048.f);
    r.a1 = (int)(short)lrintf(f * 2048.f);
    return r;
}
__device__ __forceinline__ ResizeTap resize_tap(int d, int dsize, int ssize) { return resize_tap_scaled(d, (double)ssize / (double)dsize, ssize); }

__device__ __forceinline__ void resize_px_strided(const uint8_t* src, size_t rs, int sh, int sw, int dh, int dw, int dy, int dx, int rgb[3])
{
    if (sh == dh && sw == dw) {
        const uint8_t* p = src + dy * rs + dx * 3;
        rgb[0] = p[2]; rgb[1] = p[1]; rgb[2] = p[0];
    } else if (sh == 2 * dh && sw == 2 * dw) {
        const uint8_t* p = src + (size_t)(2 * dy) * rs + (size_t)(2 * dx) * 3;
#pragma unroll
        for (int c = 0; c < 3; ++c) rgb[2 - c] = (p[c] + p[3 + c] + p[rs + c] + p[rs + 3 + c] + 2) >> 2;
    } else {
        const ResizeTap ax = resize_tap(dx, dw, sw), ay = resize_tap(dy, dh, sh);
        const uint8_t* r0 = src + ay.s0 * rs; const uint8_t* r1 = src + ay.s1 * rs;
#pragma unroll
        for (int c = 0; c < 3; ++c) {
            const int t0 = r0[ax.s0 * 3 + c] * ax.a0 + r0[ax.s1 * 3 + c] * ax.a1;
            const int t1 = r1[ax.s0 * 3 + c] * ax.a0 + r1[ax.s1 * 3 + c] * ax.a1;
            rgb[2 - c] = (((ay.a0 * (t0 >> 4)) >> 16) + ((ay.a1 * (t1 >> 4)) >> 16) + 2) >> 2;
        }
    }
}

}
```

### eagle_amd/csrc/runtime.h

```cpp
#pragma once
#include <algorithm>
#include <atomic>
#include <chrono>
#include <cmath>
#include <condition_variable>
#include <mutex>
#include <shared_mutex>
#include <thread>
#include <cstdarg>
#include <cstring>
#include <functional>
#include <map>
#include <memory>
#include <string>
#include <vector>
#include <cstddef>
#include "common.h"

namespace eagle {

extern thread_local std::string g_create_error;
extern std::shared_timed_mutex g_capture_mutex;
extern std::mutex g_gate_m;
extern std::condition_variable g_gate_cv;
// ... 2 lines not shown
extern thread_local std::shared_lock<std::shared_timed_mutex>* t_api_lock;
struct ApiGuard {
    std::shared_lock<std::shared_timed_mutex> lk;
    bool outer;
    ApiGuard() : lk(g_capture_mutex, std::defer_lock), outer(t_api_lock == nullptr)
    {
        if (!outer) return;
        {
            std::unique_lock<std::mutex> g(g_gate_m);
            g_gate_cv.wait_for(g, std::chrono::milliseconds(GATE_WAIT_MS), [] { return g_capture_waiting == 0; });
        }
        lk.lock(); t_api_lock = &lk;
    }
    ~ApiGuard() { if (outer) t_api_lock = nullptr; }
};
struct CaptureExclusive {
    std::shared_lock<std::shared_timed_mutex>* al;
    std::unique_lock<std::shared_timed_mutex> ex;
    bool ok = false;
    CaptureExclusive() : al(t_api_lock), ex(g_capture_mutex, std::defer_lock)
    {
        if (al && al->owns_lock()) al->unlock();
        { std::lock_guard<std::mutex> g(g_gate_m); ++g_capture_waiting; }
        ok = ex.try_lock_for(std::chrono::milliseconds(CAPTURE_TRY_MS));
        { std::lock_guard<std::mutex> g(g_gate_m); --g_capture_waiting; }
        g_gate_cv.notify_all();
        if (!ok && al) al->lock();
    }
    ~CaptureExclusive() { if (ok) { ex.unlock(); if (al) al->lock(); } }
};
extern int g_dbg_skip;

struct HostTensor { std::vector<int64_t> shape; std::vector<float> data; };

class CopyPool {
public:
    explicit CopyPool(int n) { for (int i = 0; i < n; ++i) th_.emplace_back([this] { work(); }); }
    ~CopyPool()
    {
        { std::lock_guard<std::mutex> g(m_); quit_ = true; }
        cv_.notify_all();
        for (auto& t : th_) t.join();
    }
    void run(int n, const std::function<void(int)>& fn)
    {
        if (n <= 0) return;
        std::unique_lock<std::mutex> g(m_);
        fn_ = &fn; next_ = 0; n_ = n; left_ = n;
        cv_.notify_all();
        done_.wait(g, [this] { return left_ == 0; });
        fn_ = nullptr;
    }
private:
    void work()
    {
        std::unique_lock<std::mutex> g(m_);
        for (;;) {
            cv_.wait(g, [this] { return quit_ || (fn_ && next_ < n_); });
            if (quit_) return;
            const int k = next_++;
            const std::function<void(int)>* f = fn_;
            g.unlock();
            (*f)(k);
            g.lock();
            if (--left_ == 0) done_.notify_all();
        }
    }
    std::vector<std::thread> th_;
    std::mutex m_;
    std::condition_variable cv_, done_;
    const std::function<void(int)>* fn_ = nullptr;
    int next_ = 0, n_ = 0, left_ = 0;
    bool quit_ = false;
};

struct Op {
    enum Kind { CONV, OTHER, FORK, JOIN } kind = OTHER;
    std::function<void(hipStream_t)> run;
    double flop = 0;
    double bytes = 0;
    const char* tag = "";
    int stream = 0;
    int nbranch = 0;
};

struct Net {
    std::vector<Op> ops;
    std::vector<std::unique_ptr<std::string>> names;
    std::vector<void*> owned;
    std::multimap<size_t, void*> free_list[4];
    int pool = 0;
    std::map<void*, size_t> sizes;
    size_t bytes = 0;
    ~Net() { for (void* p : owned) (void)hipFree(p); }
    void* get(size_t b)
    {
        b = (b + 255) & ~(size_t)255;
        auto it = free_list[pool].find(b);
        if (it != free_list[pool].end()) { void* p = it->second; free_list[pool].erase(it); return p; }
        void* p = nullptr;
        HIP_CHECK(hipMalloc(&p, b));
        HIP_CHECK(hipMemset(p, 0, b));
        owned.push_back(p); sizes[p] = b; bytes += b;
        return p;
    }
    void put(void* p) { if (p) free_list[pool].insert({sizes.at(p), p}); }
    void* upload(const void* src, size_t b)
    {
        void* p = nullptr;
        HIP_CHECK(hipMalloc(&p, std::max<size_t>(b, 16)));
        HIP_CHECK(hipMemcpy(p, src, b, hipMemcpyHostToDevice));
        owned.push_back(p); bytes += b;
        return p;
    }
};

}

using namespace eagle;

struct EagleHandle {
    EagleConfig cfg;
    std::string err;
    std::map<std::string, HostTensor> weights;
    bool finalized = false;
    int prec = 0, det_prec = 0;
    hipStream_t s_main = nullptr, s_det = nullptr, s_post = nullptr, s_copy = nullptr;
    hipStream_t s_br[3] = {nullptr, nullptr, nullptr};
    hipEvent_t ev_fork = nullptr, ev_join[3] = {nullptr, nullptr, nullptr};
    bool multi_stream = true;
    hipEvent_t ev_pre = nullptr, ev_det = nullptr, ev_t0 = nullptr, ev_t1 = nullptr;
    struct StepBuf {
        ArgmaxPart* parts = nullptr;
        EagleFrameResult* d_out = nullptr;
        EagleFrameResult* h_out = nullptr;
        unsigned* d_sat = nullptr;
        unsigned* h_sat = nullptr;
        uint8_t* d_frames = nullptr;
        uint8_t* h_frames = nullptr;
        uint8_t* d_yuv = nullptr;
        uint8_t* h_yuv = nullptr;
        bool copy_pending = false;
        hipEvent_t ev_compute = nullptr, ev_done = nullptr, ev_copy = nullptr;
        std::map<int, hipGraphExec_t> graphs;
        int capture_backoff = 0, capture_skip = 0;
    } sb[2];
    bool graph_broken = false;
    int graph_captures = 0, graph_skipped = 0;
    std::unique_ptr<Net> hr, yo, misc, reid;
    TView reid_in; float* reid_feats = nullptr; EagleCrop* reid_crops = nullptr; EagleCrop* reid_crops_h = nullptr; float* reid_feats_h = nullptr;
    eagle::Tracker* tracker = nullptr;
    std::unique_ptr<CopyPool> pool;
    TView kp_in, det_in, logits;
    LetterBox lb;
    int hm_chunks = 64;
    ArgmaxPart* cur_parts = nullptr;
    unsigned* cur_sat = nullptr;
    unsigned* clip_sat = nullptr;
    unsigned* clip_sat_h = nullptr;
    long long sat_events = 0; int sat_frames = 0;
    bool fused_argmax = false;
    DetScratch ds;
    DetLevel levels[3];
    PostParams pp;
    bool warmed = false;
    int call_steps = 0;
    bool prof = false;
    std::vector<hipEvent_t> conv_ev;
    struct Span { int k; double bytes; hipEvent_t a, b; };
    std::vector<hipEvent_t> span_pool; size_t span_used = 0;
    std::vector<Span> spans;
    std::vector<EagleKernelTime> ktab;
    std::vector<const Op*> conv_ops;
    EagleTimings timings{};
    double conv_flop_step = 0; int n_conv = 0, n_launch = 0;
    struct Clip {
        bool open = false;
        ClipView cv;
        uint8_t* g[3] = {nullptr, nullptr, nullptr};
        EagleFrameResult* recs = nullptr;
        MemList* mem = nullptr;
        ChainState* st = nullptr;
        ChainState* st_op = nullptr;
        ChainState* h_st = nullptr;
        ChainState* h_zero = nullptr;
        int* h_tail = nullptr;
        MemList* h_mem = nullptr;
        hipEvent_t ev_gray = nullptr, ev_det = nullptr, ev_kp = nullptr, ev_loop = nullptr;
        uint8_t* ecc_small = nullptr;
        int ecc_h = 0, ecc_w = 0;
        int2* ecc_pairs = nullptr; eagle::EccResult* ecc_out = nullptr;
        int ecc_next = -1, ecc_tmpl = -2;
    } clip;
    uint8_t* ecc_prev = nullptr; int ecc_prev_h = 0, ecc_prev_w = 0; bool ecc_has_prev = false;
    void* rccl = nullptr; void* comm = nullptr; int rank = 0, world = 1;
    void* gather_buf = nullptr; size_t gather_cap = 0;
};

namespace eagle {
constexpr int REID_NB = 64;
void finalize(EagleHandle* h);
size_t sat_pad_bytes(int B);
void run_net(EagleHandle* h, Net* net, hipStream_t s, size_t& ev_i);
void check_saturation(EagleHandle* h, const char* what);
void clip_close(EagleHandle* h);
}

#define API_BEGIN try { eagle::ApiGuard api_guard_;
#define API_BEGIN_H(h) if (!(h)) return EAGLE_E_INVALID; API_BEGIN
#define API_END(h)                                                       \
    }                                                                    \
    catch (const eagle::Err& e) { if (h) (h)->err = e.msg; else eagle::g_create_error = e.msg; return e.code; } \
    catch (const std::exception& e) { if (h) (h)->err = e.what(); else eagle::g_create_error = e.what(); return EAGLE_E_INVALID; } \
    return EAGLE_OK;
```

### eagle_amd/csrc/step.hip

```cpp
#include "runtime.h"

namespace eagle {

static int ktab_index(EagleHandle* h, const char* name)
{
    for (size_t i = 0; i < h->ktab.size(); ++i) if (!strcmp(h->ktab[i].name, name)) return (int)i;
    EagleKernelTime e; memset(&e, 0, sizeof(e)); strncpy(e.name, name, sizeof(e.name) - 1);
    h->ktab.push_back(e);
    return (int)h->ktab.size() - 1;
}
template <class F>
static void timed(EagleHandle* h, const char* name, double bytes, hipStream_t st, F&& fn)
{
    if (!h->prof) { fn(); return; }
    while (h->span_pool.size() < h->span_used + 2) { hipEvent_t e; HIP_CHECK(hipEventCreate(&e)); h->span_pool.push_back(e); }
    EagleHandle::Span sp{ktab_index(h, name), bytes, h->span_pool[h->span_used], h->span_pool[h->span_used + 1]};
    h->span_used += 2;
    HIP_CHECK(hipEventRecord(sp.a, st));
    fn();
    HIP_CHECK(hipEventRecord(sp.b, st));
    h->spans.push_back(sp);
}

size_t sat_pad_bytes(int B) { return ((size_t)B * sizeof(unsigned) + 255) & ~(size_t)255; }

void run_net(EagleHandle* h, Net* net, hipStream_t s, size_t& ev_i)
{
    const bool multi = h->multi_stream && !h->prof;
    for (Op& op : net->ops) {
        if (op.kind == Op::FORK) {
            if (multi) {
                HIP_CHECK(hipEventRecord(h->ev_fork, s));
                for (int k = 0; k < op.nbranch; ++k) HIP_CHECK(hipStreamWaitEvent(h->s_br[k], h->ev_fork, 0));
            }
            continue;
        }
        if (op.kind == Op::JOIN) {
            if (multi)
                for (int k = 0; k < op.nbranch; ++k) {
                    HIP_CHECK(hipEventRecord(h->ev_join[k], h->s_br[k]));
                    HIP_CHECK(hipStreamWaitEvent(s, h->ev_join[k], 0));
                }
            continue;
        }
        hipStream_t st = (multi && op.stream > 0) ? h->s_br[op.stream - 1] : s;
        if ((g_dbg_skip & 64) && op.kind == Op::OTHER) continue;
        if ((g_dbg_skip & 128) && op.kind == Op::CONV) continue;
        if (h->prof && op.kind == Op::CONV) {
            HIP_CHECK(hipEventRecord(h->conv_ev[ev_i++], st));
            op.run(st);
            HIP_CHECK(hipEventRecord(h->conv_ev[ev_i++], st));
            h->conv_ops.push_back(&op);
        } else {
            timed(h, op.tag, op.bytes, st, [&] { op.run(st); });
        }
    }
}

static void enqueue_compute(EagleHandle* h, int p, const uint8_t* d_src, int n_active)
{
    const EagleConfig& c = h->cfg;
    const int B = c.batch;
    EagleHandle::StepBuf& sb = h->sb[p];
    size_t ev_i = 0;
    HIP_CHECK(hipMemsetAsync(sb.d_sat, 0, sat_pad_bytes(B) + sizeof(EagleFrameResult) * B, h->s_main));
    h->cur_sat = sb.d_sat;
    const double esz = h->prec == EAGLE_PREC_F16 ? 2 : 4;
    if (!(g_dbg_skip & 16))
        timed(h, "preprocess", (double)n_active * ((double)c.frame_h * c.frame_w * 3 + (540.0 * 960 + (double)h->lb.out_h * h->lb.out_w) * h->kp_in.c * esz), h->s_main,
              [&] {
                  preprocess_launch(h->prec, d_src, n_active, c.frame_h, c.frame_w, h->kp_in, h->det_in, h->lb, h->s_main, 3, h->det_prec);
              });
    const bool two = !h->prof;
    hipStream_t sd = two ? h->s_det : h->s_main;
    if (two) {
        HIP_CHECK(hipEventRecord(h->ev_pre, h->s_main));
        HIP_CHECK(hipStreamWaitEvent(sd, h->ev_pre, 0));
    }
    if (!(g_dbg_skip & 2)) run_net(h, h->yo.get(), sd, ev_i);
    if (!(g_dbg_skip & 4)) {
        timed(h, "yolo_decode", (double)B * h->ds.A * ((64 + 16) * 4.0 + 4 * 4 + 4 + 4 + 8), sd, [&] { yolo_decode_launch(h->levels, 3, B, 5, c.detector_floor, h->ds, sd); });
        timed(h, "nms", (double)B * h->ds.A * 8.0, sd, [&] { nms_launch(h->ds, B, h->pp, sb.d_out, sd); });
    }
    if (two) HIP_CHECK(hipEventRecord(h->ev_det, sd));
    h->cur_parts = sb.parts;
    if (!(g_dbg_skip & 1)) run_net(h, h->hr.get(), h->s_main, ev_i);
    if (!(g_dbg_skip & 32) && !h->fused_argmax)
        timed(h, "heat_argmax", (double)h->logits.n * h->logits.h * h->logits.w * h->logits.cs * 4.0, h->s_main, [&] { heat_argmax_launch(h->logits, sb.parts, h->hm_chunks, h->s_main); });
    if (two) HIP_CHECK(hipStreamWaitEvent(h->s_main, h->ev_det, 0));
}

static bool graph_on(const EagleHandle* h) { return !h->graph_broken && (h->cfg.use_graph == 1 || (h->cfg.use_graph == 2 && h->call_steps >= 3)); }

static void launch_step(EagleHandle* h, int p, const uint8_t* d_src, int n_active)
{
    const EagleConfig& c = h->cfg;
    EagleHandle::StepBuf& sb = h->sb[p];
    bool replayed = false;
    if (graph_on(h) && !h->prof) {
        if (!h->warmed) {
            enqueue_compute(h, p, d_src, n_active);
            HIP_CHECK(hipStreamSynchronize(h->s_main));
            h->warmed = true;
        }
        if (d_src != sb.d_frames) fail(EAGLE_E_STATE, "graph replay needs the slot's staging buffer as the source");
        auto it = sb.graphs.find(n_active);
        if (it == sb.graphs.end() && sb.capture_skip > 0) --sb.capture_skip;
        else if (it == sb.graphs.end()) {
            CaptureExclusive only_this_thread_talks_to_hip;
            if (only_this_thread_talks_to_hip.ok) {
                struct CaptureScope {
                    EagleHandle* h; bool open = false; hipGraph_t g = nullptr;
                    ~CaptureScope()
                    {
                        if (open) { (void)hipStreamEndCapture(h->s_main, &g); (void)hipGetLastError(); h->graph_broken = true; }
                        if (g) (void)hipGraphDestroy(g);
                    }
                } cs{h};
                HIP_CHECK(hipStreamBeginCapture(h->s_main, hipStreamCaptureModeThreadLocal));
                cs.open = true;
                enqueue_compute(h, p, d_src, n_active);
                cs.open = false;
                HIP_CHECK(hipStreamEndCapture(h->s_main, &cs.g));
                hipGraphExec_t ge = nullptr;
                if (hipGraphInstantiate(&ge, cs.g, nullptr, nullptr, 0) != hipSuccess) { (void)hipGetLastError(); h->graph_broken = true; fail(EAGLE_E_HIP, "hipGraphInstantiate failed"); }
                if (sb.graphs.size() >= 16) { (void)hipGraphExecDestroy(sb.graphs.begin()->second); sb.graphs.erase(sb.graphs.begin()); }
                it = sb.graphs.emplace(n_active, ge).first;
                sb.capture_backoff = 0;
                ++h->graph_captures;
            } else {
                sb.capture_backoff = std::min(64, std::max(1, sb.capture_backoff * 2));
                sb.capture_skip = sb.capture_backoff;
                ++h->graph_skipped;
            }
        }
        if (it != sb.graphs.end()) { HIP_CHECK(hipGraphLaunch(it->second, h->s_main)); replayed = true; }
    }
    if (!replayed) enqueue_compute(h, p, d_src, n_active);
    hipStream_t sp = h->prof ? h->s_main : h->s_post;
    if (!h->prof) {
        HIP_CHECK(hipEventRecord(sb.ev_compute, h->s_main));
        HIP_CHECK(hipStreamWaitEvent(sp, sb.ev_compute, 0));
    }
    if (!(g_dbg_skip & 8)) timed(h, "post (geometry)", 0, sp, [&] { post_launch(sb.parts, c.batch, h->pp, sb.d_out, sp); });
    HIP_CHECK(hipMemcpyAsync(sb.h_sat, sb.d_sat, sat_pad_bytes(c.batch) + sizeof(EagleFrameResult) * n_active, hipMemcpyDeviceToHost, sp));
    HIP_CHECK(hipEventRecord(sb.ev_done, sp));
}

static void collect_step(EagleHandle* h, int p, int n_active, EagleFrameResult* out)
{
    HIP_CHECK(hipEventSynchronize(h->sb[p].ev_done));
    memcpy(out, h->sb[p].h_out, sizeof(EagleFrameResult) * n_active);
    for (int i = 0; i < n_active; ++i)
        if (h->sb[p].h_sat[i]) { out[i].pad[1] = 1; h->sat_events += h->sb[p].h_sat[i]; ++h->sat_frames; }
    h->timings.n_launches += h->n_launch;
    h->timings.n_conv_launches += h->n_conv;
    h->timings.conv_flop += h->conv_flop_step;
    if (h->prof) {
        for (size_t i = 0; i + 1 < h->conv_ev.size(); i += 2) {
            float t = 0.f;
            HIP_CHECK(hipEventElapsedTime(&t, h->conv_ev[i], h->conv_ev[i + 1]));
            h->timings.conv_ms += t;
            if (i / 2 < h->conv_ops.size()) {
                const Op* op = h->conv_ops[i / 2];
                EagleKernelTime& e = h->ktab[ktab_index(h, op->tag)];
                e.ms += t; e.launches += 1; e.bytes += op->bytes; e.flop += op->flop;
            }
        }
        h->conv_ops.clear();
        for (const EagleHandle::Span& sp : h->spans) {
            float t = 0.f;
            HIP_CHECK(hipEventElapsedTime(&t, sp.a, sp.b));
            EagleKernelTime& e = h->ktab[sp.k];
            e.ms += t; e.launches += 1; e.bytes += sp.bytes;
        }
        h->spans.clear(); h->span_used = 0;
    }
}

template <class Stage>
static void run_pipeline(EagleHandle* h, const char* what, int n, EagleFrameResult* out, Stage stage)
{
    const int B = h->cfg.batch;
    memset(&h->timings, 0, sizeof(h->timings));
    h->sat_events = 0; h->sat_frames = 0;
    if (n == 0) return;
    h->call_steps = (n + B - 1) / B;
    HIP_CHECK(hipEventRecord(h->ev_t0, h->s_main));
    int prev_n = 0, prev_i = 0, k = 0;
    for (int i = 0; i < n; i += B, ++k) {
        const int p = k & 1, na = std::min(B, n - i);
        const uint8_t* src = stage(p, i, na);
        launch_step(h, p, src, na);
        if (k > 0) collect_step(h, p ^ 1, prev_n, out + prev_i);
        prev_n = na; prev_i = i;
        if (h->prof) { collect_step(h, p, na, out + i); prev_n = 0; }
    }
    if (prev_n > 0) collect_step(h, (k - 1) & 1, prev_n, out + prev_i);
    hipStream_t sp = h->prof ? h->s_main : h->s_post;
    HIP_CHECK(hipEventRecord(h->ev_t1, sp));
    HIP_CHECK(hipEventSynchronize(h->ev_t1));
    HIP_CHECK(hipEventSynchronize(h->ev_t0));
    float ms = 0.f;
    HIP_CHECK(hipEventElapsedTime(&ms, h->ev_t0, h->ev_t1));
    h->timings.total_ms = ms;
    h->timings.sat_events = (int32_t)std::min<long long>(h->sat_events, 0x7fffffff);
    h->timings.sat_frames = h->sat_frames;
    check_saturation(h, what);
}

void check_saturation(EagleHandle* h, const char* what)
{
    if (h->sat_events > 0 && !h->cfg.allow_saturation)
        fail(EAGLE_E_RANGE, "%s: %lld activation stores in %d frame(s) left the range of the f32s tensor format (|v| > 4094) and were clipped; the records are "
             "written (EagleFrameResult.pad[1] marks the frames) but are not fp32-grade.  Use EAGLE_PREC_F32 for these weights, or set EagleConfig.allow_saturation",
             what, h->sat_events, h->sat_frames);
}

struct HostPlane { int64_t off, pitch, rows, row_bytes, dense_off; };

struct YuvGeom {
    int fmt, h, w, nplanes;
    int64_t frame_stride, y_pitch, c_offset, c_pitch, v_offset;
    int64_t extent;
// ... 230 lines not shown
```

### eagle_amd/lib.py

```python
import ctypes as C
import os

import numpy as np

_HERE = os.path.dirname(os.path.abspath(__file__))
LIB_PATH = os.environ.get("EAGLE_HIP_LIB") or os.path.join(_HERE, "libeagle_hip.so")

MAX_DET, N_LANDMARKS, MAX_KP = 300, 57, 87
PREC_F16, PREC_F32, PREC_F32S = 0, 1, 2
PRECISIONS = {"f16": PREC_F16, "f32": PREC_F32, "f32s": PREC_F32S}
DET_VARIANTS = {"n": 0, "s": 1, "m": 2, "l": 3, "x": 4}
AUTO, SMALL_BATCH = -1, 32
LETTERBOX = {"rect": 0, "square": 1}
DET_PREC_AUTO = -1
DET_PREC_MIXED = 4


class EagleError(RuntimeError):
    pass


class EagleRangeError(EagleError):
    records = None


class EagleConfig(C.Structure):
    _fields_ = [("device", C.c_int32), ("frame_h", C.c_int32), ("frame_w", C.c_int32), ("det_variant", C.c_int32),
                ("det_imgsz", C.c_int32), ("batch", C.c_int32), ("precision", C.c_int32),
                ("keypoint_conf", C.c_double), ("detector_conf", C.c_double), ("ransac_thresh", C.c_double),
                ("detector_floor", C.c_float), ("nms_iou", C.c_float),
                ("ransac_max_iters", C.c_int32), ("lm_iters", C.c_int32), ("use_graph", C.c_int32), ("det_precision", C.c_int32),
                ("allow_saturation", C.c_int32), ("multi_stream", C.c_int32), ("letterbox", C.c_int32), ("reserved", C.c_int32 * 3)]


class EagleTimings(C.Structure):
    _fields_ = [("total_ms", C.c_float), ("conv_ms", C.c_float), ("n_launches", C.c_int32),
                ("n_conv_launches", C.c_int32), ("conv_flop", C.c_double), ("sat_events", C.c_int32), ("sat_frames", C.c_int32),
                ("graph_captures", C.c_int32), ("graph_skipped", C.c_int32), ("reserved", C.c_int32 * 4)]


class EagleTrackParams(C.Structure):
    _fields_ = [("track_high_thresh", C.c_float), ("track_low_thresh", C.c_float), ("new_track_thresh", C.c_float), ("match_thresh", C.c_float),
                ("track_buffer", C.c_int32), ("frame_rate", C.c_int32)]


class EagleYuvLayout(C.Structure):
    _fields_ = [("frame_stride", C.c_int64), ("y_pitch", C.c_int64), ("c_offset", C.c_int64), ("c_pitch", C.c_int64), ("v_offset", C.c_int64)]


PIX_FORMATS = {"nv12": 1, "i420": 2}


class EagleKernelTime(C.Structure):
    _fields_ = [("name", C.c_char * 40), ("ms", C.c_float), ("launches", C.c_int32), ("bytes", C.c_double), ("flop", C.c_double)]


DET_DTYPE = np.dtype([("x1", "<f4"), ("y1", "<f4"), ("x2", "<f4"), ("y2", "<f4"), ("conf", "<f4"), ("cls", "<i4"),
                      ("id", "<i4"), ("bx1", "<i4"), ("by1", "<i4"), ("bx2", "<i4"), ("by2", "<i4"),
                      ("foot_x", "<i4"), ("foot_y", "<i4"), ("pitch_xf", "<f4"), ("pitch_yf", "<f4"),
                      ("pitch_x", "<i4"), ("pitch_y", "<i4"), ("reported", "u1"), ("in_bounds", "u1"), ("pad", "u1", 2)],
                     align=True)
KP_DTYPE = np.dtype([("label", "<i4"), ("x", "<i4"), ("y", "<i4"), ("score", "<f4"), ("synthesized", "u1"),
                     ("on_plane", "u1"), ("inlier", "u1"), ("pad", "u1")], align=True)
RESULT_DTYPE = np.dtype([("n_det", "<i4"), ("n_kp", "<i4"), ("n_candidates", "<i4"), ("H_valid", "u1"),
                         ("bounds_valid", "u1"), ("pad", "u1", 2), ("H", "<f8", 9), ("bounds", "<f8", 4),
                         ("hm_idx", "<i4", N_LANDMARKS), ("hm_score", "<f4", N_LANDMARKS),
                         ("kp", KP_DTYPE, MAX_KP), ("det", DET_DTYPE, MAX_DET)], align=True)

_lib = None


def require_torch_first():
    import sys
    if "torch" not in sys.modules and _lib is not None:
        raise EagleError("torch must be imported before eagle_amd.lib loads libeagle_hip.so in a process that uses both "
                         "(two ROCm runtimes would be mapped: torch's bundled one and /opt/rocm's); import torch first, or keep the process torch-free")


def load():
    global _lib
    if _lib is not None:
        return _lib
    if not os.path.exists(LIB_PATH):
        raise EagleError(f"{LIB_PATH} not found: run `python -c 'import __graft_entry__ as g; g.build()'` "
                         "(there is no CPU fallback for the product path)")
    L = C.CDLL(LIB_PATH)
    vp, i32, i64 = C.c_void_p, C.c_int, C.c_int64
    fp, dp, u8p = C.POINTER(C.c_float), C.POINTER(C.c_double), C.POINTER(C.c_uint8)
    L.eagle_abi_sizes.argtypes = [C.POINTER(C.c_int32)]
    L.eagle_default_config.argtypes = [C.POINTER(EagleConfig)]
    L.eagle_create.argtypes = [C.POINTER(EagleConfig), C.POINTER(vp)]
    L.eagle_destroy.argtypes = [vp]
    L.eagle_destroy.restype = None
    L.eagle_last_error.argtypes = [vp]
    L.eagle_last_error.restype = C.c_char_p
    L.eagle_get_config.argtypes = [vp, C.POINTER(EagleConfig)]
    L.eagle_resolve_config.argtypes = [C.POINTER(EagleConfig)]
    L.eagle_load_weights.argtypes = [vp, C.c_char_p, fp, C.POINTER(i64), i32]
    L.eagle_finalize_weights.argtypes = [vp]
    L.eagle_process_frames.argtypes = [vp, u8p, i32, i64, i64, vp]
    L.eagle_process_device_frames.argtypes = [vp, vp, i32, vp]
    L.eagle_host_alloc.argtypes = [vp, i64, C.POINTER(vp)]
    L.eagle_host_free.argtypes = [vp, vp]
    L.eagle_device_alloc.argtypes = [vp, i64, C.POINTER(vp)]
    L.eagle_device_free.argtypes = [vp, vp]
    L.eagle_device_upload.argtypes = [vp, vp, vp, i64]
    L.eagle_reproject.argtypes = [vp, vp, i32, dp, u8p]
    L.eagle_clip_open.argtypes = [vp, vp, i32]
    L.eagle_clip_close.argtypes = [vp]
    L.eagle_clip_detect_keypoints.argtypes = [vp, i32, i32, i32]
    L.eagle_clip_get_keypoints.argtypes = [vp, i32, vp, C.POINTER(i32)]
    L.eagle_clip_set_keypoints.argtypes = [vp, i32, vp, i32]
    L.eagle_clip_flow.argtypes = [vp, i32, i32, i32, vp, i32, vp, C.POINTER(i32), fp, u8p]
    L.eagle_clip_run.argtypes = [vp, i32, i32, i32, i32, i32, i32, C.POINTER(i32)]
    L.eagle_clip_detect_objects.argtypes = [vp, i32, i32]
    L.eagle_clip_fetch.argtypes = [vp, vp]
    L.eagle_comm_id.argtypes = [vp]
    L.eagle_comm_init.argtypes = [vp, i32, i32, vp]
    L.eagle_gather.argtypes = [vp, vp, i32, vp]
    L.eagle_set_profiling.argtypes = [vp, i32]
    L.eagle_get_timings.argtypes = [vp, C.POINTER(EagleTimings)]
    L.eagle_get_kernel_times.argtypes = [vp, C.POINTER(EagleKernelTime), i32, C.POINTER(i32)]
    L.eagle_op_conv2d.argtypes = [i32, i32, fp, i32, i32, i32, i32, fp, fp, i32, i32, i32, i32, fp, fp, i32, fp]
    L.eagle_op_bottleneck.argtypes = [i32, fp, i32, i32, i32, i32, fp, fp, fp, fp, fp, fp, fp, fp, i32, fp, fp, fp]
    L.eagle_op_fuse_sum.argtypes = [i32, i32, fp, i32, i32, i32, i32, i32, C.POINTER(fp), C.POINTER(i32), C.POINTER(i32), i32, fp]
    L.eagle_op_preprocess.argtypes = [i32, i32, u8p, i32, i32, i32, i32, fp, fp, C.POINTER(i32)]
    L.eagle_op_preprocess_lb.argtypes = [i32, i32, u8p, i32, i32, i32, i32, i32, fp, fp, C.POINTER(i32)]
    L.eagle_op_find_homography.argtypes = [i32, fp, fp, i32, C.c_double, i32, i32, dp, u8p, C.POINTER(i32)]
    L.eagle_debug.argtypes = [C.c_char_p, i64, vp, i64]
    L.eagle_team_colors.argtypes = [vp, vp, i32, vp, i32, vp]
    L.eagle_track_open.argtypes = [vp, C.POINTER(EagleTrackParams)]
    L.eagle_track_frames.argtypes = [vp, vp, i32]
    L.eagle_track_frames_cmc.argtypes = [vp, vp, i32, C.POINTER(C.c_double)]
    L.eagle_clip_motion.argtypes = [vp, i32, i32, C.POINTER(C.c_double)]
    L.eagle_clip_motion_ecc.argtypes = [vp, i32, i32, i32, C.POINTER(C.c_double), C.POINTER(i32)]
    L.eagle_reid_features.argtypes = [vp, vp, i32, vp, i32, fp]
    yl = C.POINTER(EagleYuvLayout)
    L.eagle_process_frames_yuv.argtypes = [vp, i32, u8p, i32, yl, vp]
    L.eagle_process_device_frames_yuv.argtypes = [vp, i32, vp, i32, yl, vp]
    L.eagle_yuv_to_bgr.argtypes = [vp, i32, vp, i32, yl, vp]
    L.eagle_op_yuv_to_bgr.argtypes = [i32, i32, u8p, i32, i32, i32, yl, u8p]
    L.eagle_track_frames_reid.argtypes = [vp, vp, i32, C.POINTER(C.c_double), fp, C.POINTER(i32), C.POINTER(i32)]
    _lib = L
    return L


EXPORTS = ["eagle_abi_sizes", "eagle_default_config", "eagle_create", "eagle_destroy", "eagle_last_error", "eagle_get_config", "eagle_resolve_config", "eagle_load_weights",
           "eagle_finalize_weights", "eagle_process_frames", "eagle_process_device_frames", "eagle_device_alloc",
           "eagle_device_free", "eagle_device_upload", "eagle_host_alloc", "eagle_host_free", "eagle_reproject", "eagle_comm_id", "eagle_comm_init", "eagle_gather",
           "eagle_set_profiling", "eagle_get_timings", "eagle_get_kernel_times", "eagle_op_conv2d", "eagle_op_bottleneck", "eagle_op_fuse_sum", "eagle_op_preprocess", "eagle_op_preprocess_lb",
           "eagle_op_find_homography", "eagle_clip_open", "eagle_clip_close", "eagle_clip_detect_objects", "eagle_clip_detect_keypoints", "eagle_clip_get_keypoints",
           "eagle_clip_set_keypoints", "eagle_clip_flow", "eagle_clip_run", "eagle_clip_fetch", "eagle_debug", "eagle_track_open", "eagle_track_frames", "eagle_track_frames_cmc", "eagle_clip_motion_ecc", "eagle_clip_motion", "eagle_team_colors",
           "eagle_reid_features", "eagle_track_frames_reid", "eagle_process_frames_yuv", "eagle_process_device_frames_yuv", "eagle_yuv_to_bgr",
           "eagle_op_yuv_to_bgr"]

FLOWKP_DTYPE = np.dtype([("label", "<i4"), ("x", "<i4"), ("y", "<i4"), ("score", "<f4")], align=True)
E_REFERENCE_RAISES = -7
E_RANGE = -8


def debug(key, value=0, out=None):
    rc = load().eagle_debug(key.encode(), int(value), None if out is None else out.ctypes.data_as(C.c_void_p), 0 if out is None else out.nbytes)
    if rc:
        raise EagleError(f"eagle_debug({key}) failed ({rc})")
    return out


def resolve_config(cfg):
    out = EagleConfig.from_buffer_copy(cfg)
    if load().eagle_resolve_config(C.byref(out)):
        raise EagleError("eagle_resolve_config failed")
    return out


def abi_sizes():
    o = (C.c_int32 * 4)()
    load().eagle_abi_sizes(o)
    return list(o)


def _fp(a):
    return a.ctypes.data_as(C.POINTER(C.c_float)) if a is not None else None


def default_config(**kw):
    cfg = EagleConfig()
    load().eagle_default_config(C.byref(cfg))
    for k, v in kw.items():
        if k == "det_variant" and isinstance(v, str):
            v = DET_VARIANTS[v]
        if k == "letterbox" and isinstance(v, str):
            v = LETTERBOX[v]
        if not hasattr(cfg, k):
            raise TypeError(f"unknown config field {k}")
        setattr(cfg, k, v)
    return cfg


class Handle:

    def __init__(self, cfg=None, **kw):
        self.L = load()
        self.cfg = cfg or default_config(**kw)
        self._h = C.c_void_p()
        rc = self.L.eagle_create(C.byref(self.cfg), C.byref(self._h))
        if rc:
            raise EagleError(f"eagle_create failed ({rc}): {self.L.eagle_last_error(None).decode()}")
        resolved = EagleConfig()
        self._check(self.L.eagle_get_config(self._h, C.byref(resolved)), "get_config")
        self.cfg = resolved

    def _check(self, rc, what):
        if rc == E_RANGE:
            raise EagleRangeError(f"{what}: {self.L.eagle_last_error(self._h).decode()}")
        if rc:
            raise EagleError(f"{what} failed ({rc}): {self.L.eagle_last_error(self._h).decode()}")

    def _check_records(self, rc, what, out):
        try:
            self._check(rc, what)
        except EagleRangeError as e:
            e.records = out
            raise

    def close(self):
        if self._h:
            self.L.eagle_destroy(self._h)
            self._h = C.c_void_p()

    def __del__(self):
        try:
            self.close()
        except Exception:
            pass

    def load_weight(self, name, arr):
        arr = np.ascontiguousarray(arr, np.float32)
        shape = (C.c_int64 * max(arr.ndim, 1))(*arr.shape)
        self._check(self.L.eagle_load_weights(self._h, name.encode(), _fp(arr), shape, arr.ndim), f"load_weights({name})")

    def finalize_weights(self):
        self._check(self.L.eagle_finalize_weights(self._h), "finalize_weights")

    def process(self, frames, out=None, strides=None):
        frames = np.asarray(frames)
        if frames.dtype != np.uint8:
            frames = frames.astype(np.uint8)
        if frames.ndim == 3:
            frames = frames[None]
        n, h, w, c = frames.shape
        if (h, w, c) != (self.cfg.frame_h, self.cfg.frame_w, 3):
            raise EagleError(f"frame shape {(h, w, c)} does not match the handle ({self.cfg.frame_h}, {self.cfg.frame_w}, 3)")
        fs, rs, ps, cs = frames.strides
        if n == 1:
            fs = max(fs, rs * (h - 1) + 3 * w)
        if not (cs == 1 and ps == 3 and rs >= 3 * w and fs >= rs * (h - 1) + 3 * w):
            frames = np.ascontiguousarray(frames)
            fs, rs = h * w * 3, w * 3
        if strides is not None:
            fs, rs = strides
        if out is None:
            out = np.zeros(n, RESULT_DTYPE)
        assert out.dtype == RESULT_DTYPE and len(out) >= n and out.flags.c_contiguous
        self._check_records(self.L.eagle_process_frames(self._h, C.cast(frames.ctypes.data, C.POINTER(C.c_uint8)), n, int(fs), int(rs),
                                                        out.ctypes.data_as(C.c_void_p)), "process_frames", out)
        return out

    def host_frames(self, n):
        shape = (n, self.cfg.frame_h, self.cfg.frame_w, 3)
        nbytes = int(np.prod(shape))
        p = C.c_void_p()
        self._check(self.L.eagle_host_alloc(self._h, nbytes, C.byref(p)), "host_alloc")
        buf = (C.c_uint8 * max(nbytes, 1)).from_address(p.value)
        a = np.frombuffer(buf, np.uint8, nbytes).reshape(shape)
        self._pinned = getattr(self, "_pinned", {})
        self._pinned[a.ctypes.data] = p
        return a

    def host_buffer(self, nbytes):
        p = C.c_void_p()
        self._check(self.L.eagle_host_alloc(self._h, int(nbytes), C.byref(p)), "host_alloc")
        a = np.frombuffer((C.c_uint8 * max(int(nbytes), 1)).from_address(p.value), np.uint8, int(nbytes))
        self._pinned = getattr(self, "_pinned", {})
        self._pinned[a.ctypes.data] = p
        return a

    def host_free(self, a):
        p = self._pinned.pop(a.ctypes.data)
        self._check(self.L.eagle_host_free(self._h, p), "host_free")

    def upload(self, frames):
        frames = np.ascontiguousarray(frames, np.uint8)
        d = C.c_void_p()
        self._check(self.L.eagle_device_alloc(self._h, frames.nbytes, C.byref(d)), "device_alloc")
        self._check(self.L.eagle_device_upload(self._h, d, frames.ctypes.data_as(C.c_void_p), frames.nbytes), "device_upload")
        return d

    def free(self, d):
        self._check(self.L.eagle_device_free(self._h, d), "device_free")

    def process_device(self, dptr, n, out=None):
        if out is None:
            out = np.zeros(n, RESULT_DTYPE)
# ... 82 lines not shown

    def clip_detect_keypoints(self, first, stride=1, count=1):
        self._check(self.L.eagle_clip_detect_keypoints(self._h, first, stride, count), "clip_detect_keypoints")

    def clip_get_keypoints(self, frame):
        buf = np.zeros(N_LANDMARKS, FLOWKP_DTYPE); n = C.c_int(0)
        self._check(self.L.eagle_clip_get_keypoints(self._h, frame, buf.ctypes.data_as(C.c_void_p), C.byref(n)), "clip_get_keypoints")
        return None if n.value < 0 else buf[: n.value].copy()

    def clip_set_keypoints(self, frame, kps):
        kps = np.ascontiguousarray(kps, FLOWKP_DTYPE)
        self._check(self.L.eagle_clip_set_keypoints(self._h, frame, kps.ctypes.data_as(C.c_void_p), len(kps)), "clip_set_keypoints")

    def clip_flow(self, src_frame, dst_frame, hue_frame, kps, raw=False):
        kps = np.ascontiguousarray(kps, FLOWKP_DTYPE)
        out = np.zeros(N_LANDMARKS, FLOWKP_DTYPE); n = C.c_int(0)
        nxt = np.zeros((max(len(kps), 1), 2), np.float32); st = np.zeros(max(len(kps), 1), np.uint8)
        self._check(self.L.eagle_clip_flow(self._h, src_frame, dst_frame, hue_frame, kps.ctypes.data_as(C.c_void_p), len(kps),
                                           out.ctypes.data_as(C.c_void_p), C.byref(n), _fp(nxt), st.ctypes.data_as(C.POINTER(C.c_uint8))), "clip_flow")
        return (out[: n.value].copy(), nxt[: len(kps)], st[: len(kps)]) if raw else out[: n.value].copy()

    def clip_run(self, first, last, keypoint_interval, homography_interval, calibration=False, wait=True):
        stalled = C.c_int(-1)
        rc = self.L.eagle_clip_run(self._h, first, last, keypoint_interval, homography_interval, int(calibration), int(wait), C.byref(stalled))
        if rc == E_REFERENCE_RAISES:
            raise IndexError(self.L.eagle_last_error(self._h).decode())
        self._check(rc, "clip_run")
        return stalled.value

    def clip_fetch(self, n):
        out = np.zeros(n, RESULT_DTYPE)
        self._check(self.L.eagle_clip_fetch(self._h, out.ctypes.data_as(C.c_void_p)), "clip_fetch")
        return out

    def team_colors(self, dptr, n_frames, crops):
        crops = np.ascontiguousarray(crops, np.int32).reshape(-1, 5)
        out = np.zeros((len(crops), 12), np.int32)
        self._check(self.L.eagle_team_colors(self._h, dptr, n_frames, crops.ctypes.data_as(C.c_void_p), len(crops), out.ctypes.data_as(C.c_void_p)), "team_colors")
        return out

    def track_open(self, **params):
        p = None
        if params:
            d = dict(track_high_thresh=0.5, track_low_thresh=0.1, new_track_thresh=0.6, match_thresh=0.8, track_buffer=30, frame_rate=30)
            d.update(params)
            p = C.byref(EagleTrackParams(**d))
        self._check(self.L.eagle_track_open(self._h, p), "track_open")

    def reid_features(self, dptr, n_frames, crops):
        crops = np.ascontiguousarray(crops, np.int32).reshape(-1, 5)
        out = np.zeros((len(crops), 512), np.float32)
        self._check(self.L.eagle_reid_features(self._h, dptr, n_frames, crops.ctypes.data_as(C.c_void_p), len(crops), out.ctypes.data_as(C.POINTER(C.c_float))), "reid_features")
        return out

    def track_frames_reid(self, recs, feats, feat_det, feat_count, warps=None):
        assert recs.dtype == RESULT_DTYPE and recs.flags.c_contiguous
        feats = np.ascontiguousarray(feats, np.float32).reshape(-1, 512)
        feat_det = np.ascontiguousarray(feat_det, np.int32); feat_count = np.ascontiguousarray(feat_count, np.int32)
        assert len(feat_count) == len(recs) and int(feat_count.sum()) == len(feats) == len(feat_det)
        w = None if warps is None else np.ascontiguousarray(warps, np.float64).reshape(len(recs), 6)
        self._check(self.L.eagle_track_frames_reid(self._h, recs.ctypes.data_as(C.c_void_p), len(recs), None if w is None else w.ctypes.data_as(C.POINTER(C.c_double)),
                                                   feats.ctypes.data_as(C.POINTER(C.c_float)), feat_det.ctypes.data_as(C.POINTER(C.c_int32)),
                                                   feat_count.ctypes.data_as(C.POINTER(C.c_int32))), "track_frames_reid")
        return recs

    def track_frames(self, recs, warps=None):
        assert recs.dtype == RESULT_DTYPE and recs.flags.c_contiguous
        w = None
        if warps is not None:
            w = np.ascontiguousarray(warps, np.float64).reshape(len(recs), 6)
        self._check(self.L.eagle_track_frames_cmc(self._h, recs.ctypes.data_as(C.c_void_p), len(recs),
                                                  w.ctypes.data_as(C.POINTER(C.c_double)) if w is not None else None), "track_frames")
        return recs

    def clip_motion(self, first, count):
        w = np.zeros((max(count, 0), 6), np.float64)
        self._check(self.L.eagle_clip_motion(self._h, first, count, w.ctypes.data_as(C.POINTER(C.c_double))), "clip_motion")
        return w

    def clip_motion_ecc(self, first, count, carry=False, return_ok=False):
        w = np.zeros((max(count, 0), 6), np.float64)
        ok = np.zeros(max(count, 0), np.int32)
        self._check(self.L.eagle_clip_motion_ecc(self._h, first, count, int(bool(carry)), w.ctypes.data_as(C.POINTER(C.c_double)),
                                                 ok.ctypes.data_as(C.POINTER(C.c_int32))), "clip_motion_ecc")
        return (w, ok) if return_ok else w

    def set_profiling(self, on):
        self._check(self.L.eagle_set_profiling(self._h, int(on)), "set_profiling")

    def timings(self):
        t = EagleTimings()
        self._check(self.L.eagle_get_timings(self._h, C.byref(t)), "get_timings")
        return t

    def kernel_times(self):
        buf = (EagleKernelTime * 256)(); n = C.c_int(0)
        self._check(self.L.eagle_get_kernel_times(self._h, buf, 256, C.byref(n)), "get_kernel_times")
        return [(buf[i].name.decode(), float(buf[i].ms), int(buf[i].launches), float(buf[i].bytes), float(buf[i].flop)) for i in range(min(n.value, 256))]

    def comm_init(self, rank, world, uid_bytes):
        buf = C.create_string_buffer(bytes(uid_bytes), 128)
        self._check(self.L.eagle_comm_init(self._h, rank, world, buf), "comm_init")

    def gather(self, local, world, out=None):
        local = np.ascontiguousarray(local)
        if out is None:
            out = np.zeros(len(local) * world, RESULT_DTYPE)
        assert out.dtype == RESULT_DTYPE and len(out) == len(local) * world and out.flags.c_contiguous
        self._check(self.L.eagle_gather(self._h, local.ctypes.data_as(C.c_void_p), len(local), out.ctypes.data_as(C.c_void_p)), "gather")
        return out


def comm_unique_id():
    buf = C.create_string_buffer(128)
    rc = load().eagle_comm_id(buf)
    if rc:
        raise EagleError(f"eagle_comm_id failed ({rc}): {load().eagle_last_error(None).decode()}")
    return buf.raw


def op_conv2d(x, w_hwio, bias, stride=1, pre=0, r1=None, r2=None, post=0, precision=PREC_F32, device=0):
    L = load()
    x = np.ascontiguousarray(x, np.float32); w = np.ascontiguousarray(w_hwio, np.float32); b = np.ascontiguousarray(bias, np.float32)
    n, h, wd, cin = x.shape
    ks, _, _, cout = w.shape
    ho = (h + 2 * (ks // 2) - ks) // stride + 1
    wo = (wd + 2 * (ks // 2) - ks) // stride + 1
    y = np.empty((n, ho, wo, cout), np.float32)
    r1 = None if r1 is None else np.ascontiguousarray(r1, np.float32)
    r2 = None if r2 is None else np.ascontiguousarray(r2, np.float32)
    rc = L.eagle_op_conv2d(device, precision, _fp(x), n, h, wd, cin, _fp(w), _fp(b), cout, ks, stride, pre, _fp(r1), _fp(r2), post, _fp(y))
    if rc:
        raise EagleError(f"eagle_op_conv2d failed ({rc}): {L.eagle_last_error(None).decode()}")
    return y


def op_bottleneck(x, w1, b1, w2, b2, w3, b3, res=None, reps=0, device=0, wd=None, bd=None):
    L = load()
    x = np.ascontiguousarray(x, np.float32)
    n, h, w, cin = x.shape
    arrs = [np.ascontiguousarray(a, np.float32) for a in (w1, b1, w2, b2, w3, b3)]
    assert arrs[0].shape == (1, 1, cin, 64) and arrs[2].shape == (3, 3, 64, 64) and arrs[4].shape == (1, 1, 64, 256), "HWIO weights of a 64-wide Bottleneck"
    res = None if res is None else np.ascontiguousarray(res, np.float32)
    y = np.empty((n, h, w, 256), np.float32)
    ms = C.c_float(0)
    wd = None if wd is None else np.ascontiguousarray(wd, np.float32)
    bd = None if bd is None else np.ascontiguousarray(bd, np.float32)
    rc = L.eagle_op_bottleneck(device, _fp(x), n, h, w, cin, *[_fp(a) for a in arrs], _fp(res), _fp(y), int(reps), C.byref(ms), _fp(wd), _fp(bd))
    if rc:
        raise EagleError(f"eagle_op_bottleneck failed ({rc}): {L.eagle_last_error(None).decode()}")
    return (y, ms.value) if reps > 0 else y


def op_fuse_sum(base, ups, relu=True, precision=PREC_F32, device=0):
    L = load()
    base = np.ascontiguousarray(base, np.float32)
    n, H, W, c = base.shape
    ups = [np.ascontiguousarray(u, np.float32) for u in ups]
    arr = (C.POINTER(C.c_float) * max(len(ups), 1))(*[_fp(u) for u in ups])
    uh = (C.c_int * max(len(ups), 1))(*[u.shape[1] for u in ups])
    uw = (C.c_int * max(len(ups), 1))(*[u.shape[2] for u in ups])
    y = np.empty_like(base)
    rc = L.eagle_op_fuse_sum(device, precision, _fp(base), n, H, W, c, len(ups), arr, uh, uw, int(relu), _fp(y))
    if rc:
        raise EagleError(f"eagle_op_fuse_sum failed ({rc}): {L.eagle_last_error(None).decode()}")
    return y


def op_preprocess(frames, det_imgsz=640, precision=PREC_F32, device=0, letterbox=0):
    L = load()
    frames = np.ascontiguousarray(frames, np.uint8)
    n, h, w, _ = frames.shape
    hw = (C.c_int * 2)()
    rc = L.eagle_op_preprocess_lb(device, precision, frames.ctypes.data_as(C.POINTER(C.c_uint8)), n, h, w, det_imgsz, int(letterbox), None, None, hw)
    if rc:
        raise EagleError(f"eagle_op_preprocess failed ({rc}): {L.eagle_last_error(None).decode()}")
    kp = np.empty((n, 540, 960, 3), np.float32)
    det = np.empty((n, hw[0], hw[1], 3), np.float32)
    rc = L.eagle_op_preprocess_lb(device, precision, frames.ctypes.data_as(C.POINTER(C.c_uint8)), n, h, w, det_imgsz, int(letterbox), _fp(kp), _fp(det), hw)
    if rc:
        raise EagleError(f"eagle_op_preprocess failed ({rc}): {L.eagle_last_error(None).decode()}")
    return kp, det


def op_find_homography(img_pts, world_pts, thresh=5.0, max_iters=2000, lm_iters=10, device=0):
    L = load()
    a = np.ascontiguousarray(img_pts, np.float32).reshape(-1, 2)
    b = np.ascontiguousarray(world_pts, np.float32).reshape(-1, 2)
    n = len(a)
    H = np.zeros(9, np.float64); mask = np.zeros(max(n, 1), np.uint8); ok = C.c_int(0)
    rc = L.eagle_op_find_homography(device, _fp(a), _fp(b), n, thresh, max_iters, lm_iters,
                                    H.ctypes.data_as(C.POINTER(C.c_double)), mask.ctypes.data_as(C.POINTER(C.c_uint8)), C.byref(ok))
    if rc:
        raise EagleError(f"eagle_op_find_homography failed ({rc}): {L.eagle_last_error(None).decode()}")
    return (H.reshape(3, 3), mask[:n]) if ok.value else (None, None)


def _pix(fmt):
    if isinstance(fmt, str):
        if fmt.lower() not in PIX_FORMATS:
            raise EagleError(f"unknown pixel format {fmt!r} (nv12 or i420)")
        return PIX_FORMATS[fmt.lower()]
    return int(fmt)


def _yuv_layout(layout):
    if layout is None or isinstance(layout, EagleYuvLayout):
        return layout
    lay = EagleYuvLayout()
    for k, v in dict(layout).items():
        if k not in dict(EagleYuvLayout._fields_):
            raise TypeError(f"unknown layout field {k}")
        setattr(lay, k, int(v))
    return lay


def yuv_span(fmt, h, w, layout, n):
    lay = _yuv_layout(layout) or EagleYuvLayout()
    nv12 = _pix(fmt) == PIX_FORMATS["nv12"]
    c_row = w if nv12 else w // 2
    yp = lay.y_pitch or w
    co = lay.c_offset or yp * h
    cp = lay.c_pitch or c_row
    planes = [(0, yp, h, w), (co, cp, h // 2, c_row)]
    if not nv12:
        planes.append((lay.v_offset or co + cp * (h // 2), cp, h // 2, c_row))
    extent = max(o + p * (r - 1) + b for o, p, r, b in planes)
    stride = lay.frame_stride or max(o + p * r for o, p, r, _ in planes)
    return 0 if n <= 0 else (n - 1) * stride + extent


def op_yuv_to_bgr(frames, fmt="nv12", layout=None, h=None, w=None, n=None, device=0):
    L = load()
    a = np.asarray(frames)
    if a.ndim in (2, 3):
        if a.ndim == 2:
            a = a[None]
        n, h, w = a.shape[0], a.shape[1] * 2 // 3, a.shape[2]
    elif h is None or w is None or n is None:
        raise EagleError("a flat 4:2:0 buffer needs h, w and n")
    a = np.ascontiguousarray(a, np.uint8)
    lay = _yuv_layout(layout)
    if a.ndim == 1 and a.nbytes < yuv_span(fmt, h, w, lay, n):
        raise EagleError(f"the buffer holds {a.nbytes} bytes, {n} frames of this layout span {yuv_span(fmt, h, w, lay, n)}")
    out = np.empty((n, h, w, 3), np.uint8)
    rc = L.eagle_op_yuv_to_bgr(device, _pix(fmt), a.ctypes.data_as(C.POINTER(C.c_uint8)), n, h, w, None if lay is None else C.byref(lay),
                               out.ctypes.data_as(C.POINTER(C.c_uint8)))
    if rc:
        raise EagleError(f"eagle_op_yuv_to_bgr failed ({rc}): {L.eagle_last_error(None).decode()}")
    return out
```

### include/eagle.h

```cpp
#ifndef EAGLE_H
#define EAGLE_H
#include <stdint.h>

#ifdef __cplusplus
extern "C" {
#endif

#define EAGLE_OK 0
#define EAGLE_E_INVALID (-1)
#define EAGLE_E_HIP (-2)
#define EAGLE_E_STATE (-3)
#define EAGLE_E_MISSING (-4)
#define EAGLE_E_NOKERNEL (-5)
#define EAGLE_E_COMM (-6)
#define EAGLE_E_RANGE (-8)

#define EAGLE_MAX_DET 300
#define EAGLE_N_LANDMARKS 57
#define EAGLE_MAX_KP 87

#define EAGLE_PREC_F16 0
#define EAGLE_PREC_F32 1
#define EAGLE_PREC_F32S 2

// ... 19 lines not shown
    int32_t det_variant;
    int32_t det_imgsz;
    int32_t batch;
    int32_t precision;
    double keypoint_conf;
    double detector_conf;
    double ransac_thresh;
    float detector_floor;
    float nms_iou;
    int32_t ransac_max_iters;
    int32_t lm_iters;
    int32_t use_graph;
    int32_t det_precision;
    int32_t allow_saturation;
    int32_t multi_stream;
    int32_t letterbox;
    int32_t reserved[3];
} EagleConfig;

typedef struct EagleDet {
    float x1, y1, x2, y2;
    float conf;
    int32_t cls;
    int32_t id;
    int32_t bx1, by1, bx2, by2;
    int32_t foot_x, foot_y;
    float pitch_xf, pitch_yf;
    int32_t pitch_x, pitch_y;
    uint8_t reported;
    uint8_t in_bounds;
    uint8_t pad[2];
} EagleDet;

typedef struct EagleKeypoint {
    int32_t label;
    int32_t x, y;
    float score;
    uint8_t synthesized;
    uint8_t on_plane;
    uint8_t inlier;
    uint8_t pad;
} EagleKeypoint;

typedef struct EagleFrameResult {
    int32_t n_det;
    int32_t n_kp;
    int32_t n_candidates;
    uint8_t H_valid;
    uint8_t bounds_valid;
    uint8_t pad[2];
    double H[9];
    double bounds[4];
    int32_t hm_idx[EAGLE_N_LANDMARKS];
    float hm_score[EAGLE_N_LANDMARKS];
    EagleKeypoint kp[EAGLE_MAX_KP];
    EagleDet det[EAGLE_MAX_DET];
} EagleFrameResult;

int eagle_abi_sizes(int32_t* out4);
int eagle_default_config(EagleConfig* cfg);
int eagle_create(const EagleConfig* cfg, EagleHandle** out);
void eagle_destroy(EagleHandle* h);
const char* eagle_last_error(EagleHandle* h);
int eagle_resolve_config(EagleConfig* cfg);
int eagle_get_config(EagleHandle* h, EagleConfig* cfg);

int eagle_load_weights(EagleHandle* h, const char* name, const float* data, const int64_t* shape, int ndim);
int eagle_finalize_weights(EagleHandle* h);

int eagle_process_frames(EagleHandle* h, const uint8_t* bgr, int n, int64_t frame_stride, int64_t row_stride,
                         EagleFrameResult* out);
int eagle_host_alloc(EagleHandle* h, int64_t bytes, void** ptr);
int eagle_host_free(EagleHandle* h, void* ptr);

int eagle_process_device_frames(EagleHandle* h, const void* d_bgr, int n, EagleFrameResult* out);
int eagle_device_alloc(EagleHandle* h, int64_t bytes, void** dptr);
int eagle_device_free(EagleHandle* h, void* dptr);
int eagle_device_upload(EagleHandle* h, void* dptr, const void* src, int64_t bytes);

#define EAGLE_PIX_NV12 1
#define EAGLE_PIX_I420 2
typedef struct EagleYuvLayout {
    int64_t frame_stride;
    int64_t y_pitch;
    int64_t c_offset;
    int64_t c_pitch;
    int64_t v_offset;
} EagleYuvLayout;
int eagle_process_frames_yuv(EagleHandle* h, int format, const uint8_t* src, int n, const EagleYuvLayout* layout, EagleFrameResult* out);
int eagle_process_device_frames_yuv(EagleHandle* h, int format, const void* d_src, int n, const EagleYuvLayout* layout, EagleFrameResult* out);
int eagle_yuv_to_bgr(EagleHandle* h, int format, const void* d_src, int n, const EagleYuvLayout* layout, void* d_bgr);
int eagle_op_yuv_to_bgr(int device, int format, const uint8_t* src, int n, int h, int w, const EagleYuvLayout* layout, uint8_t* bgr);

int eagle_reproject(EagleHandle* h, EagleFrameResult* recs, int n, const double* Hs, const uint8_t* flags);

typedef struct EagleFlowKp { int32_t label; int32_t x, y; float score; } EagleFlowKp;
int eagle_clip_open(EagleHandle* h, const void* d_bgr, int n);
int eagle_clip_detect_objects(EagleHandle* h, int first, int count);
int eagle_clip_detect_keypoints(EagleHandle* h, int first, int stride, int count);
int eagle_clip_get_keypoints(EagleHandle* h, int frame, EagleFlowKp* out , int* n );
int eagle_clip_set_keypoints(EagleHandle* h, int frame, const EagleFlowKp* in, int n);
int eagle_clip_flow(EagleHandle* h, int src_frame, int dst_frame, int hue_frame, const EagleFlowKp* in, int n_in,
                    EagleFlowKp* out , int* n_out, float* next_pts , uint8_t* status );
int eagle_clip_run(EagleHandle* h, int first, int last, int keypoint_interval, int homography_interval, int calibration, int wait,
                   int* stalled_at);
int eagle_clip_fetch(EagleHandle* h, EagleFrameResult* out);
int eagle_clip_close(EagleHandle* h);
#define EAGLE_E_REFERENCE_RAISES (-7)

typedef struct EagleCrop { int32_t frame, x1, y1, x2, y2; } EagleCrop;
typedef struct EagleTrackParams {
    float track_high_thresh, track_low_thresh, new_track_thresh, match_thresh;
    int32_t track_buffer, frame_rate;
} EagleTrackParams;
int eagle_track_open(EagleHandle* h, const EagleTrackParams* params );
int eagle_track_frames(EagleHandle* h, EagleFrameResult* recs, int n);
int eagle_clip_motion(EagleHandle* h, int first, int count, double* warps);
int eagle_clip_motion_ecc(EagleHandle* h, int first, int count, int carry, double* warps, int* ok);
int eagle_track_frames_cmc(EagleHandle* h, EagleFrameResult* recs, int n, const double* warps );
#define EAGLE_REID_DIM 512
int eagle_reid_features(EagleHandle* h, const void* d_bgr, int n_frames, const EagleCrop* crops, int n_crops, float* feats);
int eagle_track_frames_reid(EagleHandle* h, EagleFrameResult* recs, int n, const double* warps , const float* feats,
                            const int32_t* feat_det, const int32_t* feat_count);

int eagle_team_colors(EagleHandle* h, const void* d_bgr, int n_frames, const EagleCrop* crops, int n_crops, int32_t* counts);

int eagle_comm_id(void* id128);
int eagle_comm_init(EagleHandle* h, int rank, int world, const void* id128);
int eagle_gather(EagleHandle* h, const EagleFrameResult* local, int n_local, EagleFrameResult* all );

typedef struct EagleTimings {
    float total_ms;
    float conv_ms;
    int32_t n_launches;
    int32_t n_conv_launches;
    double conv_flop;
    int32_t sat_events;
    int32_t sat_frames;
    int32_t graph_captures;
    int32_t graph_skipped;
    int32_t reserved[4];
} EagleTimings;
int eagle_set_profiling(EagleHandle* h, int per_kernel_events);
int eagle_get_timings(EagleHandle* h, EagleTimings* t);
typedef struct EagleKernelTime { char name[40]; float ms; int32_t launches; double bytes; double flop; } EagleKernelTime;
int eagle_get_kernel_times(EagleHandle* h, EagleKernelTime* out, int cap, int* n);

int eagle_op_conv2d(int device, int precision, const float* x, int n, int h, int w, int cin, const float* w_hwio,
                    const float* bias, int cout, int ks, int stride, int pre_act, const float* r1, const float* r2,
                    int post_act, float* y);
int eagle_op_bottleneck(int device, const float* x, int n, int h, int w, int cin, const float* w1, const float* b1, const float* w2, const float* b2,
                        const float* w3, const float* b3, const float* res, float* y, int reps, float* ms,
                        const float* wd , const float* bd);
int eagle_op_fuse_sum(int device, int precision, const float* base, int n, int H, int W, int c, int n_up,
                      const float* const* ups, const int* up_h, const int* up_w, int relu, float* y);
int eagle_op_preprocess(int device, int precision, const uint8_t* bgr, int n, int h, int w, int det_imgsz,
                        float* kp_out , float* det_out , int* det_hw );
int eagle_op_preprocess_lb(int device, int precision, const uint8_t* bgr, int n, int h, int w, int det_imgsz, int letterbox ,
                           float* kp_out, float* det_out, int* det_hw);
int eagle_op_find_homography(int device, const float* img_pts, const float* world_pts, int n, double thresh,
                             int max_iters, int lm_iters, double* H9, uint8_t* mask, int* ok);

int eagle_debug(const char* key, int64_t value, void* out, int64_t out_bytes);

#ifdef __cplusplus
}
#endif
#endif
```

Measured before the change: 819.7.

## Fuse keypoint resize/normalize preprocessing into the HRNet stem convolution

Adds a fused stem kernel that reads raw BGR frames, bilinearly resizes and normalizes a halo window into LDS, and computes the 3x3/2 3->64 first convolution with split-fp16 MFMA in one pass. When the model's conv1 matches, the keypoint preprocessing output (540x960 split tensor) is no longer written or reread; preprocess only produces the detector input. This removes a full-resolution intermediate round trip through memory and one kernel launch. The cost is recomputing the resize for overlapping halo pixels and a more complex kernel with its own weight layout.

```diff
diff --git a/eagle_amd/csrc/clip.hip b/eagle_amd/csrc/clip.hip
--- a/eagle_amd/csrc/clip.hip
+++ b/eagle_amd/csrc/clip.hip
@@ -114,7 +114,8 @@
                 HIP_CHECK(hipMemcpyAsync(sb.d_frames + (size_t)k * fb, c.cv.bgr + (size_t)(first + (k0 + k) * stride) * fb, fb, hipMemcpyDeviceToDevice, h->s_main));
             src = sb.d_frames;
         }
-        preprocess_launch(h->prec, src, na, cf.frame_h, cf.frame_w, h->kp_in, h->det_in, h->lb, h->s_main, 1);
+        h->cur_src = src; h->cur_n = na;
+        if (!h->stem_on) preprocess_launch(h->prec, src, na, cf.frame_h, cf.frame_w, h->kp_in, h->det_in, h->lb, h->s_main, 1);
         h->cur_parts = sb.parts;
         run_net(h, h->hr.get(), h->s_main, ev_i);
         if (!h->fused_argmax) heat_argmax_launch(h->logits, sb.parts, h->hm_chunks, h->s_main);
diff --git a/eagle_amd/csrc/common.h b/eagle_amd/csrc/common.h
--- a/eagle_amd/csrc/common.h
+++ b/eagle_amd/csrc/common.h
@@ -82,6 +82,20 @@
 void bneck_tile_weights(const float* w, int taps, int cin, int cout, std::vector<_Float16>& out, float* descale);
 void bneck_scale_bias(std::vector<float>& b, float descale);
 void bneck_launch(const BneckLaunch& L, hipStream_t s);
+
+struct StemLaunch {
+    const uint8_t* bgr = nullptr;
+    int n = 0, sh = 0, sw = 0;
+    int dh = 540, dw = 960;
+    const void* w = nullptr;
+    const float* bias = nullptr;
+    float descale = 1.f;
+    TView y;
+    unsigned* const* sat_slot = nullptr;
+};
+bool stem_supported(int precision, int ks, int stride, int cin, int cout);
+void stem_tile_weights(const float* w , std::vector<_Float16>& out, float* descale);
+void stem_launch(const StemLaunch& L, hipStream_t s);
 
 struct LetterBox { int new_h, new_w, top, left, out_h, out_w; };
 LetterBox letterbox_geometry(int h, int w, int imgsz, int square = 0);
diff --git a/eagle_amd/csrc/elementwise.hip b/eagle_amd/csrc/elementwise.hip
--- a/eagle_amd/csrc/elementwise.hip
+++ b/eagle_amd/csrc/elementwise.hip
@@ -1,49 +1,11 @@
 #include <type_traits>
 #include "common.h"
 #include "dmath.h"
+#include "resize.h"
 
 namespace eagle {
 
 using half8 = __attribute__((ext_vector_type(8))) _Float16;
-
-struct ResizeAxis { int s0, s1; int a0, a1; };
-
-__device__ __forceinline__ ResizeAxis lin_coef(int d, int dsize, int ssize)
-{
-    const double scale = (double)ssize / (double)dsize;
-    float f = (float)(((double)d + 0.5) * scale - 0.5);
-    int s = (int)floorf(f);
-    f -= (float)s;
-    if (s < 0) { s = 0; f = 0.f; }
-    if (s >= ssize - 1) { s = ssize - 1; f = 0.f; }
-    ResizeAxis r;
-    r.s0 = s; r.s1 = (s + 1 < ssize) ? s + 1 : s;
-    r.a0 = (int)(short)lrintf((1.f - f) * 2048.f);
-    r.a1 = (int)(short)lrintf(f * 2048.f);
-    return r;
-}
-
-__device__ __forceinline__ void resize_px(const uint8_t* src, int sh, int sw, int dh, int dw, int dy, int dx, int rgb[3])
-{
-    const size_t rs = (size_t)sw * 3;
-    if (sh == dh && sw == dw) {
-        const uint8_t* p = src + dy * rs + dx * 3;
-        rgb[0] = p[2]; rgb[1] = p[1]; rgb[2] = p[0];
-    } else if (sh == 2 * dh && sw == 2 * dw) {
-        const uint8_t* p = src + (size_t)(2 * dy) * rs + (size_t)(2 * dx) * 3;
-#pragma unroll
-        for (int c = 0; c < 3; ++c) rgb[2 - c] = (p[c] + p[3 + c] + p[rs + c] + p[rs + 3 + c] + 2) >> 2;
-    } else {
-        const ResizeAxis ax = lin_coef(dx, dw, sw), ay = lin_coef(dy, dh, sh);
-        const uint8_t* r0 = src + ay.s0 * rs; const uint8_t* r1 = src + ay.s1 * rs;
-#pragma unroll
-        for (int c = 0; c < 3; ++c) {
-            const int t0 = r0[ax.s0 * 3 + c] * ax.a0 + r0[ax.s1 * 3 + c] * ax.a1;
-            const int t1 = r1[ax.s0 * 3 + c] * ax.a0 + r1[ax.s1 * 3 + c] * ax.a1;
-            rgb[2 - c] = (((ay.a0 * (t0 >> 4)) >> 16) + ((ay.a1 * (t1 >> 4)) >> 16) + 2) >> 2;
-        }
-    }
-}
 
 struct SplitT { char b[4]; };
 __device__ __forceinline__ void split8_store(void* dst, const float* v)
@@ -82,15 +44,15 @@
         int rgb[3];
         if (r < kp_px) {
             const int dy = r / kp.w, dx = r - dy * kp.w;
-            resize_px(src, h, w, kp.h, kp.w, dy, dx, rgb);
-            const float m0 = 0x1.eeb334p+6f, m1 = 0x1.d11eb8p+6f, m2 = 0x1.9e1eb8p+6f;
-            const float s0 = 0x1.18926cp-6f, s1 = 0x1.1ed5bp-6f, s2 = 0x1.1d8f56p-6f;
-            store_px<T>(kp, (size_t)f * kp_px + r, ((float)rgb[0] - m0) * s0, ((float)rgb[1] - m1) * s1, ((float)rgb[2] - m2) * s2);
+            resize_px_strided(src, (size_t)w * 3, h, w, kp.h, kp.w, dy, dx, rgb);
+            float v[3];
+            kp_normalize(rgb, v);
+            store_px<T>(kp, (size_t)f * kp_px + r, v[0], v[1], v[2]);
         } else {
             r -= kp_px;
             const int dy = r / det.w, dx = r - dy * det.w;
             const int yy = dy - lb.top, xx = dx - lb.left;
-            if (yy >= 0 && yy < lb.new_h && xx >= 0 && xx < lb.new_w) resize_px(src, h, w, lb.new_h, lb.new_w, yy, xx, rgb);
+            if (yy >= 0 && yy < lb.new_h && xx >= 0 && xx < lb.new_w) resize_px_strided(src, (size_t)w * 3, h, w, lb.new_h, lb.new_w, yy, xx, rgb);
             else rgb[0] = rgb[1] = rgb[2] = 114;
             store_px<TD>(det, (size_t)f * det_px + r, (float)rgb[0] / 255.0f, (float)rgb[1] / 255.0f, (float)rgb[2] / 255.0f);
         }
diff --git a/eagle_amd/csrc/nets.hip b/eagle_amd/csrc/nets.hip
--- a/eagle_amd/csrc/nets.hip
+++ b/eagle_amd/csrc/nets.hip
@@ -149,6 +149,28 @@
         snprintf(label, sizeof(label), "bneck %d->64->256%s @%dx%d%s", x.c, dsf ? "+ds" : "", x.h, x.w, label_suffix);
         emit_conv(label, flop, (double)N * x.h * x.w * 4.0 * (x.c + 256 + ((dsf || res.p == x.p) ? 0 : 256)) + 4.0 * (x.c * 64 + 9 * 64 * 64 + 64 * 256 + (dsf ? 64 * 256 : 0)),
                   [L](hipStream_t s) { bneck_launch(L, s); });
+        return L.y;
+    }
+    TView stem(const TView& x_in, const std::string& cname, const std::string& bn)
+    {
+        std::vector<float> hwio, bias; int cin, cout, ks;
+        fold(cname, bn, hwio, bias, cin, cout, ks);
+        if (!stem_supported(prec, ks, 2, cin, cout)) fail(EAGLE_E_NOKERNEL, "%s: not the 3x3/2 3->64 convolution of the fused stem", cname.c_str());
+        StemLaunch L;
+        std::vector<_Float16> img;
+        stem_tile_weights(hwio.data(), img, &L.descale);
+        L.w = net->upload(img.data(), img.size() * 2);
+        L.bias = (const float*)net->upload(bias.data(), bias.size() * 4);
+        L.sh = H->cfg.frame_h; L.sw = H->cfg.frame_w; L.dh = x_in.h; L.dw = x_in.w;
+        L.y = act((x_in.h - 1) / 2 + 1, (x_in.w - 1) / 2 + 1, 64);
+        L.sat_slot = &H->cur_sat;
+        refuse_2gib(cname, "layer", {&L.y});
+        const double flop = 2.0 * N * L.y.h * L.y.w * 64.0 * 27;
+        char label[64];
+        snprintf(label, sizeof(label), "conv stem 3x3/2 3->64 @%dx%d%s", L.y.h, L.y.w, label_suffix);
+        EagleHandle* const Hh = H;
+        emit_conv(label, flop, (double)N * L.sh * L.sw * 3.0 + (double)N * L.y.h * L.y.w * 64 * 4.0 + 27.0 * 64 * 4,
+                  [L, Hh](hipStream_t s) { StemLaunch l = L; l.bgr = Hh->cur_src; l.n = Hh->cur_n; stem_launch(l, s); });
         return L.y;
     }
     static double vbytes(const TView& v) { return (double)v.n * v.h * v.w * v.c * (v.f32 ? 4 : 2); }
@@ -236,7 +258,7 @@
 {
     const int R = ACT_RELU;
     const std::string P = HRP;
-    TView x = B.conv(x_in, P + "conv1", P + "bn1", 2, 0, nullptr, nullptr, R);
+    TView x = B.H->stem_on ? B.stem(x_in, P + "conv1", P + "bn1") : B.conv(x_in, P + "conv1", P + "bn1", 2, 0, nullptr, nullptr, R);
     TView x2 = B.conv(x, P + "conv2", P + "bn2", 2, 0, nullptr, nullptr, R);
     B.release(x); x = x2;
     for (int b = 0; b < 4; ++b) {
@@ -552,7 +574,10 @@
     Builder Bh{h, h->hr.get(), h->prec, 1e-5, B};
     Builder By{h, h->yo.get(), h->det_prec, 1e-3, B};
     By.label_suffix = " d";
-    h->kp_in = Bh.act(540, 960, cin_pad);
+    const HostTensor& w1 = Bh.W(std::string(HRP) + "conv1.weight");
+    h->stem_on = w1.shape.size() == 4 && stem_supported(h->prec, (int)w1.shape[2], 2, (int)w1.shape[1], (int)w1.shape[0]);
+    if (h->stem_on) { TView v; v.n = B; v.h = 540; v.w = 960; v.c = v.cs = cin_pad; v.f32 = prec_tensor_fmt(h->prec); h->kp_in = v; }
+    else h->kp_in = Bh.act(540, 960, cin_pad);
     h->det_in = By.act(h->lb.out_h, h->lb.out_w, det_cin_pad);
     h->logits = build_hrnet(Bh, h->kp_in);
     build_yolo(By, h->det_in, c.det_variant, h->levels, 5, det_mixed);
diff --git a/eagle_amd/csrc/ops_api.hip b/eagle_amd/csrc/ops_api.hip
--- a/eagle_amd/csrc/ops_api.hip
+++ b/eagle_amd/csrc/ops_api.hip
@@ -136,6 +136,33 @@
     API_END(hh)
 }
 
+int eagle_op_stem(int device, const uint8_t* bgr, int n, int h, int w, int dh, int dw, const float* w1, const float* b1, float* y, uint32_t* sat)
+{
+    EagleHandle* hh = nullptr;
+    API_BEGIN
+    HIP_CHECK(hipSetDevice(device));
+    if (!bgr || !w1 || !b1 || !y || n < 1 || h < 1 || w < 1 || dh < 1 || dw < 1) fail(EAGLE_E_INVALID, "eagle_op_stem: bad argument");
+    if (!stem_supported(EAGLE_PREC_F32S, 3, 2, 3, 64)) fail(EAGLE_E_NOKERNEL, "eagle_op_stem: no kernel");
+    Net net;
+    StemLaunch L;
+    L.bgr = (const uint8_t*)net.upload(bgr, (size_t)n * h * w * 3);
+    L.n = n; L.sh = h; L.sw = w; L.dh = dh; L.dw = dw;
+    std::vector<_Float16> img;
+    stem_tile_weights(w1, img, &L.descale);
+    L.w = net.upload(img.data(), img.size() * 2);
+    L.bias = (const float*)net.upload(b1, 64 * 4);
+    L.y.n = n; L.y.h = (dh - 1) / 2 + 1; L.y.w = (dw - 1) / 2 + 1; L.y.c = L.y.cs = 64; L.y.f32 = 2;
+    L.y.p = net.get((size_t)n * L.y.h * L.y.w * 64 * 4);
+    unsigned* d_sat = (unsigned*)net.get(sizeof(unsigned) * (size_t)n);
+    unsigned* const* slot = &d_sat;
+    L.sat_slot = slot;
+    stem_launch(L, nullptr);
+    HIP_CHECK(hipDeviceSynchronize());
+    from_dev(L.y, 64, y);
+    if (sat) HIP_CHECK(hipMemcpy(sat, d_sat, sizeof(unsigned) * (size_t)n, hipMemcpyDeviceToHost));
+    API_END(hh)
+}
+
 int eagle_op_fuse_sum(int device, int precision, const float* base, int n, int H, int W, int c, int n_up,
                       const float* const* ups, const int* up_h, const int* up_w, int relu, float* y)
 {
diff --git a/eagle_amd/csrc/resize.h b/eagle_amd/csrc/resize.h
--- a/eagle_amd/csrc/resize.h
+++ b/eagle_amd/csrc/resize.h
@@ -21,6 +21,19 @@
 }
 __device__ __forceinline__ ResizeTap resize_tap(int d, int dsize, int ssize) { return resize_tap_scaled(d, (double)ssize / (double)dsize, ssize); }
 
+__device__ __forceinline__ bool resize_uses_taps(int sh, int sw, int dh, int dw) { return !(sh == dh && sw == dw) && !(sh == 2 * dh && sw == 2 * dw); }
+
+__device__ __forceinline__ void resize_px_taps(const uint8_t* src, size_t rs, const ResizeTap& ax, const ResizeTap& ay, int rgb[3])
+{
+    const uint8_t* r0 = src + ay.s0 * rs; const uint8_t* r1 = src + ay.s1 * rs;
+#pragma unroll
+    for (int c = 0; c < 3; ++c) {
+        const int t0 = r0[ax.s0 * 3 + c] * ax.a0 + r0[ax.s1 * 3 + c] * ax.a1;
+        const int t1 = r1[ax.s0 * 3 + c] * ax.a0 + r1[ax.s1 * 3 + c] * ax.a1;
+        rgb[2 - c] = (((ay.a0 * (t0 >> 4)) >> 16) + ((ay.a1 * (t1 >> 4)) >> 16) + 2) >> 2;
+    }
+}
+
 __device__ __forceinline__ void resize_px_strided(const uint8_t* src, size_t rs, int sh, int sw, int dh, int dw, int dy, int dx, int rgb[3])
 {
     if (sh == dh && sw == dw) {
@@ -31,15 +44,15 @@
 #pragma unroll
         for (int c = 0; c < 3; ++c) rgb[2 - c] = (p[c] + p[3 + c] + p[rs + c] + p[rs + 3 + c] + 2) >> 2;
     } else {
-        const ResizeTap ax = resize_tap(dx, dw, sw), ay = resize_tap(dy, dh, sh);
-        const uint8_t* r0 = src + ay.s0 * rs; const uint8_t* r1 = src + ay.s1 * rs;
-#pragma unroll
-        for (int c = 0; c < 3; ++c) {
-            const int t0 = r0[ax.s0 * 3 + c] * ax.a0 + r0[ax.s1 * 3 + c] * ax.a1;
-            const int t1 = r1[ax.s0 * 3 + c] * ax.a0 + r1[ax.s1 * 3 + c] * ax.a1;
-            rgb[2 - c] = (((ay.a0 * (t0 >> 4)) >> 16) + ((ay.a1 * (t1 >> 4)) >> 16) + 2) >> 2;
-        }
+        resize_px_taps(src, rs, resize_tap(dx, dw, sw), resize_tap(dy, dh, sh), rgb);
     }
 }
 
+__device__ __forceinline__ void kp_normalize(const int rgb[3], float v[3])
+{
+    const float m0 = 0x1.eeb334p+6f, m1 = 0x1.d11eb8p+6f, m2 = 0x1.9e1eb8p+6f;
+    const float s0 = 0x1.18926cp-6f, s1 = 0x1.1ed5bp-6f, s2 = 0x1.1d8f56p-6f;
+    v[0] = ((float)rgb[0] - m0) * s0; v[1] = ((float)rgb[1] - m1) * s1; v[2] = ((float)rgb[2] - m2) * s2;
 }
+
+}
diff --git a/eagle_amd/csrc/runtime.h b/eagle_amd/csrc/runtime.h
--- a/eagle_amd/csrc/runtime.h
+++ b/eagle_amd/csrc/runtime.h
@@ -178,6 +178,9 @@
     eagle::Tracker* tracker = nullptr;
     std::unique_ptr<CopyPool> pool;
     TView kp_in, det_in, logits;
+    bool stem_on = false;
+    const uint8_t* cur_src = nullptr;
+    int cur_n = 0;
     LetterBox lb;
     int hm_chunks = 64;
     ArgmaxPart* cur_parts = nullptr;
diff --git a/eagle_amd/csrc/stem.hip b/eagle_amd/csrc/stem.hip
--- /dev/null
+++ b/eagle_amd/csrc/stem.hip
@@ -0,0 +1,240 @@
+#include <algorithm>
+#include <cmath>
+#include <vector>
+
+#include "common.h"
+#include "dmath.h"
+#include "conv_internal.h"
+#include "resize.h"
+
+namespace eagle {
+
+#include "conv_kernels.inc"
+
+using f32x16 = __attribute__((ext_vector_type(16))) float;
+
+constexpr int ST_TH = 8, ST_TW = 32;
+constexpr int ST_WH = 2 * ST_TH + 1, ST_WW = 2 * ST_TW + 1;
+constexpr int ST_HC = ST_TW + 1;
+constexpr int ST_WIN = ST_WH * 2 * ST_HC * 16;
+constexpr int ST_TPS = 272, ST_STRIP = 32 * ST_TPS;
+constexpr int ST_TAPS = (ST_WH + ST_WW) * (int)sizeof(ResizeTap);
+constexpr int ST_REG = ST_WIN > 4 * ST_STRIP ? ST_WIN : 4 * ST_STRIP;
+constexpr int ST_LDS = ST_REG + ST_TAPS;
+constexpr int ST_PI = (ST_WH * ST_WW + 255) / 256;
+static_assert(sizeof(ResizeTap) == 16 && ST_LDS <= 64 * 1024, "stem geometry");
+
+struct StemArgs {
+    const uint8_t* bgr; int n, sh, sw;
+    int dh, dw;
+    const void* w; const float* bias; float descale;
+    void* y; int ycs, yoff; unsigned ybytes;
+    int ho, wo, tiles_x, tiles_y;
+    unsigned* sat;
+};
+
+__device__ __forceinline__ void stem_split4(float v0, float v1, float v2, float v3, half4& hi, half4& lo)
+{
+    const float s0 = __builtin_amdgcn_fmed3f(v0 * SPLIT_SX, -65504.0f, 65504.0f), s1 = __builtin_amdgcn_fmed3f(v1 * SPLIT_SX, -65504.0f, 65504.0f),
+                s2 = __builtin_amdgcn_fmed3f(v2 * SPLIT_SX, -65504.0f, 65504.0f), s3 = __builtin_amdgcn_fmed3f(v3 * SPLIT_SX, -65504.0f, 65504.0f);
+    hi = half4{(_Float16)s0, (_Float16)s1, (_Float16)s2, (_Float16)s3};
+    lo = half4{(_Float16)(s0 - (float)hi[0]), (_Float16)(s1 - (float)hi[1]), (_Float16)(s2 - (float)hi[2]), (_Float16)(s3 - (float)hi[3])};
+}
+
+__device__ __forceinline__ int stem_rec(int wy, int wx) { return ((wy * 2 + (wx & 1)) * ST_HC + (wx >> 1)) * 16; }
+
+__global__ __launch_bounds__(256, 4) void stem_split_kernel(StemArgs a)
+{
+    extern __shared__ __attribute__((aligned(16))) char smem[];
+    char* const win = smem;
+    ResizeTap* const taps = (ResizeTap*)(smem + ST_REG);
+    const int tid = threadIdx.x, lane = tid & 63, wave = __builtin_amdgcn_readfirstlane(tid >> 6);
+    const int kh = lane >> 5, lx = lane & 31;
+    char* const strip = smem + wave * ST_STRIP;
+    int t = blockIdx.x;
+    const int tx = t % a.tiles_x; t /= a.tiles_x;
+    const int ty = t % a.tiles_y, n = t / a.tiles_y;
+    const int oy0 = ty * ST_TH, ox0 = tx * ST_TW;
+    const int iy0 = 2 * oy0 - 1, ix0 = 2 * ox0 - 1;
+
+    u32x4 A[2][2][2];
+#pragma unroll
+    for (int s = 0; s < 2; ++s)
+#pragma unroll
+        for (int pt = 0; pt < 2; ++pt)
+#pragma unroll
+            for (int m = 0; m < 2; ++m) A[s][pt][m] = *(const u32x4*)((const char*)a.w + (((s * 2 + pt) * 2 + m) * 64 + lane) * 16);
+
+    const bool use_taps = resize_uses_taps(a.sh, a.sw, a.dh, a.dw);
+    if (use_taps && tid < ST_WH + ST_WW) {
+        const bool row = tid < ST_WH;
+        const int d = row ? iy0 + tid : ix0 + (tid - ST_WH), ds = row ? a.dh : a.dw, ss = row ? a.sh : a.sw;
+        if (d >= 0 && d < ds) taps[tid] = resize_tap(d, ds, ss);
+    }
+    __syncthreads();
+    {
+        const size_t rs = (size_t)a.sw * 3;
+        const uint8_t* const src = a.bgr + (size_t)n * a.sh * rs;
+        int rgb[ST_PI][3];
+        if (use_taps) {
+            ResizeTap tx[ST_PI], ty[ST_PI];
+#pragma unroll
+            for (int i = 0; i < ST_PI; ++i) {
+                const int p = min(tid + i * 256, ST_WH * ST_WW - 1), wy = p / ST_WW, wx = p - wy * ST_WW;
+                const int cy = min(max(iy0 + wy, 0), a.dh - 1) - iy0, cx = min(max(ix0 + wx, 0), a.dw - 1) - ix0;
+                ty[i] = taps[min(max(cy, 0), ST_WH - 1)]; tx[i] = taps[ST_WH + min(max(cx, 0), ST_WW - 1)];
+            }
+#pragma unroll
+            for (int i = 0; i < ST_PI; ++i) resize_px_taps(src, rs, tx[i], ty[i], rgb[i]);
+        } else {
+#pragma unroll
+            for (int i = 0; i < ST_PI; ++i) {
+                const int p = min(tid + i * 256, ST_WH * ST_WW - 1), wy = p / ST_WW, wx = p - wy * ST_WW;
+                resize_px_strided(src, rs, a.sh, a.sw, a.dh, a.dw, min(max(iy0 + wy, 0), a.dh - 1), min(max(ix0 + wx, 0), a.dw - 1), rgb[i]);
+            }
+        }
+#pragma unroll
+        for (int i = 0; i < ST_PI; ++i) {
+            const int p = tid + i * 256, wy = p / ST_WW, wx = p - wy * ST_WW;
+            const int iy = iy0 + wy, ix = ix0 + wx;
+            float v[3];
+            kp_normalize(rgb[i], v);
+            half4 hi, lo;
+            stem_split4(v[0], v[1], v[2], 0.0f, hi, lo);
+            const u32x2 h2 = __builtin_bit_cast(u32x2, hi), l2 = __builtin_bit_cast(u32x2, lo);
+            const bool in_map = iy >= 0 && iy < a.dh && ix >= 0 && ix < a.dw;
+            const u32x4 rec = in_map ? u32x4{h2[0], h2[1], l2[0], l2[1]} : u32x4{0u, 0u, 0u, 0u};
+            if (p < ST_WH * ST_WW) *(u32x4*)(win + stem_rec(wy, wx)) = rec;
+        }
+    }
+    __syncthreads();
+    int roff[2][2];
+#pragma unroll
+    for (int s = 0; s < 2; ++s)
+#pragma unroll
+        for (int i = 0; i < 2; ++i) {
+            const int tap = 2 * (2 * s + kh) + i, ky = tap / 3, kx = tap - ky * 3;
+            roff[s][i] = stem_rec(ky, kx);
+        }
+    const rsrc_t yrs = __builtin_amdgcn_make_buffer_rsrc(a.y, 0, (int)a.ybytes, 0x00020000);
+    const float ds = a.descale;
+    float vmax = 0.0f;
+    f32x16 accs[2][2];
+#pragma unroll
+    for (int j = 0; j < 2; ++j) {
+        const int r = wave * 2 + j;
+        const char* const rb = win + stem_rec(2 * r, 2 * lx);
+        f32x16 (&acc)[2] = accs[j];
+#pragma unroll
+        for (int m = 0; m < 2; ++m)
+#pragma unroll
+            for (int k = 0; k < 16; ++k) acc[m][k] = 0.0f;
+        const u32x4 r8 = *(const u32x4*)(rb + stem_rec(2, 2));
+#pragma unroll
+        for (int s = 0; s < 2; ++s) {
+            const u32x4 r0 = *(const u32x4*)(rb + roff[s][0]), r1 = *(const u32x4*)(rb + roff[s][1]);
+            const int g = 2 * s + kh;
+            const unsigned xh0 = g == 0 ? r8[0] << 16 : g == 1 ? r8[1] << 16 : 0u, xh1 = g == 0 ? r8[0] & 0xFFFF0000u : 0u;
+            const unsigned xl0 = g == 0 ? r8[2] << 16 : g == 1 ? r8[3] << 16 : 0u, xl1 = g == 0 ? r8[2] & 0xFFFF0000u : 0u;
+            const u32x4 bh = {r0[0], r0[1] | xh0, r1[0], r1[1] | xh1}, bl = {r0[2], r0[3] | xl0, r1[2], r1[3] | xl1};
+            const half8 Bh = __builtin_bit_cast(half8, bh), Bl = __builtin_bit_cast(half8, bl);
+#pragma unroll
+            for (int m = 0; m < 2; ++m) {
+                acc[m] = __builtin_amdgcn_mfma_f32_32x32x16_f16(__builtin_bit_cast(half8, A[s][0][m]), Bh, acc[m], 0, 0, 0);
+                acc[m] = __builtin_amdgcn_mfma_f32_32x32x16_f16(__builtin_bit_cast(half8, A[s][0][m]), Bl, acc[m], 0, 0, 0);
+                acc[m] = __builtin_amdgcn_mfma_f32_32x32x16_f16(__builtin_bit_cast(half8, A[s][1][m]), Bh, acc[m], 0, 0, 0);
+            }
+        }
+    }
+    __syncthreads();
+#pragma unroll
+    for (int j = 0; j < 2; ++j) {
+        const int r = wave * 2 + j;
+        f32x16 (&acc)[2] = accs[j];
+        const int oy = oy0 + r;
+        const bool inside = oy < a.ho && ox0 + lx < a.wo;
+        char* const rec = strip + lx * ST_TPS + kh * 8;
+#pragma unroll
+        for (int m = 0; m < 2; ++m)
+#pragma unroll
+            for (int jj = 0; jj < 4; ++jj) {
+                const float4 bv = *(const float4*)(a.bias + m * 32 + jj * 8 + kh * 4);
+                float v0 = acc[m][jj * 4 + 0] * ds + bv.x, v1 = acc[m][jj * 4 + 1] * ds + bv.y, v2 = acc[m][jj * 4 + 2] * ds + bv.z, v3 = acc[m][jj * 4 + 3] * ds + bv.w;
+                v0 = v0 > 0.f ? v0 : 0.f; v1 = v1 > 0.f ? v1 : 0.f; v2 = v2 > 0.f ? v2 : 0.f; v3 = v3 > 0.f ? v3 : 0.f;
+                half4 hi, lo; stem_split4(v0, v1, v2, v3, hi, lo);
+                const float mm = split_absmax4(vmax, v0, v1, v2, v3);
+                vmax = inside ? mm : vmax;
+                char* const d = rec + (m * 4 + jj) * 32;
+                *(half4*)d = hi; *(half4*)(d + 16) = lo;
+            }
+        u32x4 sd[8];
+#pragma unroll
+        for (int i = 0; i < 8; ++i) { const int e = i * 64 + lane; sd[i] = *(const u32x4*)(strip + (e >> 4) * ST_TPS + (e & 15) * 16); }
+        __builtin_amdgcn_sched_barrier(0);
+#pragma unroll
+        for (int i = 0; i < 8; ++i) {
+            const int e = i * 64 + lane, ox = ox0 + (e >> 4);
+            const unsigned off = (oy < a.ho && ox < a.wo) ? (unsigned)((((n * a.ho + oy) * a.wo + ox) * a.ycs + a.yoff) * 2 + (e & 15) * 16) : OOB_OFF;
+            __builtin_amdgcn_raw_buffer_store_b128(sd[i], yrs, off, 0, EAGLE_STORE_NT * 2);
+        }
+        __builtin_amdgcn_sched_barrier(0);
+        asm volatile("s_nop 2" ::: "memory");
+        __builtin_amdgcn_sched_barrier(0);
+    }
+    split_report(a.sat, n, vmax);
+}
+
+void stem_tile_weights(const float* w, std::vector<_Float16>& out, float* descale)
+{
+    float amax = 0.f;
+    for (int k = 0; k < 27 * 64; ++k) amax = std::max(amax, std::fabs(w[k]));
+    int e = 0;
+    if (amax > 0.f) (void)std::frexp(amax, &e);
+    const int sw = 15 - e;
+    const float scale = std::ldexp(1.0f, sw);
+    *descale = std::ldexp(1.0f, -(sw + 4));
+    out.resize((size_t)2 * 2 * 2 * 64 * 8);
+    _Float16* d = out.data();
+    for (int s = 0; s < 2; ++s)
+        for (int part = 0; part < 2; ++part)
+            for (int mb = 0; mb < 2; ++mb)
+                for (int l = 0; l < 64; ++l)
+                    for (int j = 0; j < 8; ++j) {
+                        const int g = 2 * s + (l >> 5);
+                        int tap = -1, c = 0;
+                        if (j < 3) { tap = 2 * g; c = j; }
+                        else if (j >= 4 && j < 7) { tap = 2 * g + 1; c = j - 4; }
+                        else if (g == 0) { tap = 8; c = j == 3 ? 0 : 1; }
+                        else if (g == 1 && j == 3) { tap = 8; c = 2; }
+                        const float v = tap < 0 ? 0.f : w[(size_t)(tap * 3 + c) * 64 + mb * 32 + (l & 31)] * scale;
+                        const _Float16 hi = (_Float16)v;
+                        *d++ = part == 0 ? hi : (_Float16)(v - (float)hi);
+                    }
+}
+
+bool stem_supported(int precision, int ks, int stride, int cin, int cout)
+{
+    return precision == EAGLE_PREC_F32S && ks == 3 && stride == 2 && cin == 3 && cout == 64;
+}
+
+void stem_launch(const StemLaunch& L, hipStream_t s)
+{
+    const TView& y = L.y;
+    const int ho = (L.dh - 1) / 2 + 1, wo = (L.dw - 1) / 2 + 1;
+    if (y.f32 != 2 || y.c != 64 || y.h != ho || y.w != wo || L.n < 0 || L.n > y.n || L.sh < 1 || L.sw < 1 || L.dh < 1 || L.dw < 1 || !L.bgr)
+        fail(EAGLE_E_INVALID, "fused stem: a %d x %d x 64-channel split-format output of at least %d frames required", ho, wo, L.n);
+    const size_t ybytes = (size_t)y.n * y.h * y.w * y.cs * 4;
+    if (ybytes >= ((size_t)1 << 31)) fail(EAGLE_E_INVALID, "fused stem: the output of %d frames reaches 2 GiB (32-bit tensor offsets); use a smaller device batch", y.n);
+    if (L.n == 0) return;
+    StemArgs a;
+    a.bgr = L.bgr; a.n = L.n; a.sh = L.sh; a.sw = L.sw; a.dh = L.dh; a.dw = L.dw;
+    a.w = L.w; a.bias = L.bias; a.descale = L.descale;
+    a.y = y.p; a.ycs = y.cs * 2; a.yoff = y.off * 2; a.ybytes = (unsigned)ybytes; a.ho = ho; a.wo = wo;
+    a.tiles_x = (wo + ST_TW - 1) / ST_TW; a.tiles_y = (ho + ST_TH - 1) / ST_TH;
+    a.sat = L.sat_slot ? *L.sat_slot : nullptr;
+    ensure_max_dynamic_lds((const void*)stem_split_kernel, ST_LDS);
+    hipLaunchKernelGGL(stem_split_kernel, dim3((unsigned)(a.tiles_x * a.tiles_y * L.n)), dim3(256), ST_LDS, s, a);
+    HIP_CHECK(hipGetLastError());
+}
+
+}
diff --git a/eagle_amd/csrc/step.hip b/eagle_amd/csrc/step.hip
--- a/eagle_amd/csrc/step.hip
+++ b/eagle_amd/csrc/step.hip
@@ -65,11 +65,12 @@
     size_t ev_i = 0;
     HIP_CHECK(hipMemsetAsync(sb.d_sat, 0, sat_pad_bytes(B) + sizeof(EagleFrameResult) * B, h->s_main));
     h->cur_sat = sb.d_sat;
-    const double esz = h->prec == EAGLE_PREC_F16 ? 2 : 4;
+    h->cur_src = d_src; h->cur_n = n_active;
+    const double esz = h->prec == EAGLE_PREC_F16 ? 2 : 4, det_esz = h->det_prec == EAGLE_PREC_F16 ? 2 : 4;
     if (!(g_dbg_skip & 16))
-        timed(h, "preprocess", (double)n_active * ((double)c.frame_h * c.frame_w * 3 + (540.0 * 960 + (double)h->lb.out_h * h->lb.out_w) * h->kp_in.c * esz), h->s_main,
+        timed(h, "preprocess", (double)n_active * ((double)c.frame_h * c.frame_w * 3 + (h->stem_on ? 0.0 : 540.0 * 960 * h->kp_in.c * esz) + (double)h->lb.out_h * h->lb.out_w * h->det_in.c * det_esz), h->s_main,
               [&] {
-                  preprocess_launch(h->prec, d_src, n_active, c.frame_h, c.frame_w, h->kp_in, h->det_in, h->lb, h->s_main, 3, h->det_prec);
+                  preprocess_launch(h->prec, d_src, n_active, c.frame_h, c.frame_w, h->kp_in, h->det_in, h->lb, h->s_main, h->stem_on ? 2 : 3, h->det_prec);
               });
     const bool two = !h->prof;
     hipStream_t sd = two ? h->s_det : h->s_main;
diff --git a/eagle_amd/lib.py b/eagle_amd/lib.py
--- a/eagle_amd/lib.py
+++ b/eagle_amd/lib.py
@@ -123,6 +123,7 @@
     L.eagle_get_kernel_times.argtypes = [vp, C.POINTER(EagleKernelTime), i32, C.POINTER(i32)]
     L.eagle_op_conv2d.argtypes = [i32, i32, fp, i32, i32, i32, i32, fp, fp, i32, i32, i32, i32, fp, fp, i32, fp]
     L.eagle_op_bottleneck.argtypes = [i32, fp, i32, i32, i32, i32, fp, fp, fp, fp, fp, fp, fp, fp, i32, fp, fp, fp]
+    L.eagle_op_stem.argtypes = [i32, u8p, i32, i32, i32, i32, i32, fp, fp, fp, C.POINTER(C.c_uint32)]
     L.eagle_op_fuse_sum.argtypes = [i32, i32, fp, i32, i32, i32, i32, i32, C.POINTER(fp), C.POINTER(i32), C.POINTER(i32), i32, fp]
     L.eagle_op_preprocess.argtypes = [i32, i32, u8p, i32, i32, i32, i32, fp, fp, C.POINTER(i32)]
     L.eagle_op_preprocess_lb.argtypes = [i32, i32, u8p, i32, i32, i32, i32, i32, fp, fp, C.POINTER(i32)]
@@ -148,7 +149,7 @@
 EXPORTS = ["eagle_abi_sizes", "eagle_default_config", "eagle_create", "eagle_destroy", "eagle_last_error", "eagle_get_config", "eagle_resolve_config", "eagle_load_weights",
            "eagle_finalize_weights", "eagle_process_frames", "eagle_process_device_frames", "eagle_device_alloc",
            "eagle_device_free", "eagle_device_upload", "eagle_host_alloc", "eagle_host_free", "eagle_reproject", "eagle_comm_id", "eagle_comm_init", "eagle_gather",
-           "eagle_set_profiling", "eagle_get_timings", "eagle_get_kernel_times", "eagle_op_conv2d", "eagle_op_bottleneck", "eagle_op_fuse_sum", "eagle_op_preprocess", "eagle_op_preprocess_lb",
+           "eagle_set_profiling", "eagle_get_timings", "eagle_get_kernel_times", "eagle_op_conv2d", "eagle_op_bottleneck", "eagle_op_stem", "eagle_op_fuse_sum", "eagle_op_preprocess", "eagle_op_preprocess_lb",
            "eagle_op_find_homography", "eagle_clip_open", "eagle_clip_close", "eagle_clip_detect_objects", "eagle_clip_detect_keypoints", "eagle_clip_get_keypoints",
            "eagle_clip_set_keypoints", "eagle_clip_flow", "eagle_clip_run", "eagle_clip_fetch", "eagle_debug", "eagle_track_open", "eagle_track_frames", "eagle_track_frames_cmc", "eagle_clip_motion_ecc", "eagle_clip_motion", "eagle_team_colors",
            "eagle_reid_features", "eagle_track_frames_reid", "eagle_process_frames_yuv", "eagle_process_device_frames_yuv", "eagle_yuv_to_bgr",
@@ -537,6 +538,21 @@
     return (y, ms.value) if reps > 0 else y
 
 
+def op_stem(frames, w1, b1, out_hw=(540, 960), device=0):
+    L = load()
+    frames = np.ascontiguousarray(frames, np.uint8)
+    n, h, w, _ = frames.shape
+    w1 = np.ascontiguousarray(w1, np.float32); b1 = np.ascontiguousarray(b1, np.float32)
+    assert w1.shape == (3, 3, 3, 64) and b1.shape == (64,), "HWIO weights of HRNet's conv1"
+    dh, dw = out_hw
+    y = np.empty((n, (dh - 1) // 2 + 1, (dw - 1) // 2 + 1, 64), np.float32)
+    sat = np.zeros(n, np.uint32)
+    rc = L.eagle_op_stem(device, frames.ctypes.data_as(C.POINTER(C.c_uint8)), n, h, w, dh, dw, _fp(w1), _fp(b1), _fp(y), sat.ctypes.data_as(C.POINTER(C.c_uint32)))
+    if rc:
+        raise EagleError(f"eagle_op_stem failed ({rc}): {L.eagle_last_error(None).decode()}")
+    return y, sat
+
+
 def op_fuse_sum(base, ups, relu=True, precision=PREC_F32, device=0):
     L = load()
     base = np.ascontiguousarray(base, np.float32)
diff --git a/include/eagle.h b/include/eagle.h
--- a/include/eagle.h
+++ b/include/eagle.h
@@ -195,6 +195,7 @@
 int eagle_op_bottleneck(int device, const float* x, int n, int h, int w, int cin, const float* w1, const float* b1, const float* w2, const float* b2,
                         const float* w3, const float* b3, const float* res, float* y, int reps, float* ms,
                         const float* wd , const float* bd);
+int eagle_op_stem(int device, const uint8_t* bgr, int n, int h, int w, int dh, int dw, const float* w1, const float* b1, float* y, uint32_t* sat);
 int eagle_op_fuse_sum(int device, int precision, const float* base, int n, int H, int W, int c, int n_up,
                       const float* const* ups, const int* up_h, const int* up_w, int relu, float* y);
 int eagle_op_preprocess(int device, int precision, const uint8_t* bgr, int n, int h, int w, int det_imgsz,
```

Measured after the change: 828.7 (median of 6 runs). 1.1% higher.
